# om-ai-lab/OmChat

Measured on AMD Instinct MI355X. Metric: images/sec prefill + decode tokens/sec, OmChat-13B TP=1/8; p50 TTFT, higher is better.
Workload: dtype bf16

## Files before the change

include/omchat_hip.h:

```cpp
#ifndef OMCHAT_HIP_H
#define OMCHAT_HIP_H
#include <stddef.h>
#include <stdint.h>

#ifdef __cplusplus
extern "C" {
#endif

#define OMCHAT_F16 0
#define OMCHAT_BF16 1
#define OMCHAT_F32 2
#define OMCHAT_PAD_ROW INT32_MIN

typedef struct omchat_ctx omchat_ctx;

typedef struct {
  int v_hidden;
  int v_heads;
  int v_qk_channels;
  int v_mlp;
  int v_layers;
  int v_patch;
  int v_image;
  float v_eps;
  int t_hidden;
  int t_layers;
  int t_heads;
  int t_kv_heads;
  int t_mlp;
  int t_vocab;
  int t_vocab_total;
  float t_eps;
  float rope_theta;
  int max_seq;
  int max_batch;
  int max_tiles;
  int max_prefill_rows;
  int dtype;
  int v_head_dim;
  int v_norm_type;
  int v_no_qk_norm;
} omchat_config;

const char* omchat_last_error(void);
const char* omchat_version(void);

int omchat_ctx_create(const omchat_config* cfg, int tp_rank, int tp_size, void* rccl_comm, omchat_ctx** out);
void omchat_ctx_destroy(omchat_ctx* ctx);
int omchat_load_tensor(omchat_ctx* ctx, const char* name, const void* data, const int64_t* shape, int ndim, int src_dtype);
int omchat_fill_synthetic(omchat_ctx* ctx, uint64_t seed);
int omchat_weights_missing(omchat_ctx* ctx);
size_t omchat_device_bytes(omchat_ctx* ctx);

int omchat_vit_forward(omchat_ctx* ctx, const void* pixels, int n_tiles, int select_layer, int keep_cls, void* out, void* stream);
int omchat_projector_forward(omchat_ctx* ctx, const void* in, int rows, void* out, void* stream);
int omchat_encode_images(omchat_ctx* ctx, const void* pixels, int n_tiles, int select_layer, void* out, void* stream);

int omchat_splice_plan(const int64_t* ids, const uint8_t* mask, int b, int T, int n_tok, int n_tiles_avail,
                       int padding_side, int max_length, int32_t* src_index, int32_t* lengths, int* S_out, int vocab);
int omchat_splice_gather(omchat_ctx* ctx, const int32_t* src_index, const void* feats, void* embeds, int rows, void* stream);

int omchat_prefill(omchat_ctx* ctx, const void* embeds, int b, int S, const int32_t* lengths, float* logits_last,
                   void* hidden_out, void* stream);
int omchat_prefill_left(omchat_ctx* ctx, const void* embeds, int b, int S, const int32_t* lengths, float* logits_last,
                        void* hidden_out, void* stream);
int omchat_decode_step(omchat_ctx* ctx, const int32_t* tokens, int b, float* logits, int32_t* next_tokens, void* stream);
int omchat_decode_step_masked(omchat_ctx* ctx, const int32_t* tokens, int b, const int32_t* positions, const uint8_t* key_mask, int mask_ld,
                              float* logits, int32_t* next_tokens, void* stream);
int omchat_masked_decode_begin(omchat_ctx* ctx, int b, const int32_t* positions, const uint8_t* key_mask, int mask_ld, int mask_cols, void* stream);
int omchat_decode_step_masked_next(omchat_ctx* ctx, const int32_t* tokens, int b, float* logits, int32_t* next_tokens, void* stream);
int omchat_fused_status(omchat_ctx* ctx, long* launches, unsigned* timeout_bits);
int omchat_has_experiments(void);
int omchat_lm_head(omchat_ctx* ctx, const void* hidden, int n, float* logits, void* stream);
int omchat_greedy(omchat_ctx* ctx, const float* logits, int b, int32_t* next_tokens, void* stream);
int omchat_set_sampling(omchat_ctx* ctx, int b, uint64_t seed, float temperature, int top_k, double top_p, float rep_penalty,
                        const int32_t* seen_ids, const int32_t* n_seen_per_row, void* stream);
int omchat_set_sampling_filters(omchat_ctx* ctx, double min_p, double typical_p, double epsilon_cutoff, double eta_cutoff, void* stream);
int omchat_sample(omchat_ctx* ctx, const float* logits, int b, int32_t* next_tokens, void* stream);
#define OMCHAT_CON_MAX_NGRAM 64
#define OMCHAT_CON_MAX_EOS 16
#define OMCHAT_CON_MAX_SUPPRESS 1024
#define OMCHAT_CON_MAX_BAD_WORDS 1024
#define OMCHAT_CON_MAX_BAD_WORD_IDS 8192
int omchat_set_constraints(omchat_ctx* ctx, int b, int no_repeat_ngram_size, int min_new_tokens, int min_length, const int32_t* eos_ids, int n_eos,
                           const int32_t* suppress_ids, int n_suppress, const int32_t* begin_suppress_ids, int n_begin_suppress,
                           const int32_t* bad_word_ids, const int32_t* bad_word_offsets, int n_bad_words, const int32_t* prompt_ids,
                           const int32_t* prompt_len, int max_new, void* stream);
int omchat_set_logprobs(omchat_ctx* ctx, int b, int max_new, void* stream);
int omchat_read_logprobs(omchat_ctx* ctx, int b, float* raw, float* processed, int32_t* counts, int max_len);
int omchat_read_sampling_state(omchat_ctx* ctx, int row, int* step, uint32_t* seen_words);
int omchat_kv_lengths(omchat_ctx* ctx, int32_t* out, int b);
int omchat_kv_rewind(omchat_ctx* ctx, int b, int n, void* stream);

int omchat_beam_begin(omchat_ctx* ctx, int b, int num_beams, float length_penalty, int early_stopping, const int32_t* eos_ids, int n_eos,
                      int max_new, int prompt_tok_len, void* stream);
int omchat_beam_step(omchat_ctx* ctx, const float* logits, int rows, int32_t* next_tokens, int32_t* done_word, void* stream);
int omchat_beam_result(omchat_ctx* ctx, int num_return, int32_t* tokens, int32_t* lengths, float* scores, int max_len);

#define OMCHAT_VERIFY_KEEP_ALL 1
#define OMCHAT_VERIFY_SAMPLE 2
int omchat_decode_verify(omchat_ctx* ctx, const int32_t* tokens, int T, float* logits, int32_t* picks,
                         int* n_accept, int flags, void* stream);

int omchat_prefill_extend(omchat_ctx* ctx, const void* embeds, int S_new, int keep, float* logits_last, void* hidden_out, void* stream);
int omchat_extend_attn_form(int S_new, int keep, int Hkv);
int omchat_kv_read(omchat_ctx* ctx, int layer, int which, int pos0, int n, void* out, void* stream);

int omchat_enable_decode_graph(omchat_ctx* ctx, int on);
int omchat_decode_graph_stats(omchat_ctx* ctx, long* steps, long* replays, long* captures);

int omchat_enable_fp8_decode(omchat_ctx* ctx, int on);

int omchat_enable_mxfp4_decode(omchat_ctx* ctx, int mode);

int omchat_enable_fp8_kv(omchat_ctx* ctx, int on);
int omchat_enable_fp8_prefill(omchat_ctx* ctx, int on);

#define OMCHAT_PROF_DECODE_GATEUP 0
#define OMCHAT_PROF_PREFILL_GATEUP 1
#define OMCHAT_PROF_VIT_FC1 2
#define OMCHAT_PROF_CATS 3
int omchat_prof_enable(omchat_ctx* ctx, int on);
int omchat_prof_read(omchat_ctx* ctx, int cat, double* total_ms, long* launches, int reset);

int omchat_mha_fwd(const void* qkv, int B, int S, int H, float softmax_scale, int causal, void* out, int dtype, void* stream);
int omchat_mha_fwd_varlen(const void* qkv, int B, int S, int H, int D, const int32_t* seqlens, float softmax_scale, int causal,
                          void* out, int dtype, void* stream);

int omchat_op_gemm(int dtype, const void* A, int lda, const void* W, int ldw, void* C, int ldc, int M, int N, int K,
                   const void* bias, const void* ls, const void* resid, int ldr, int epi, int force_tile, void* stream);
int omchat_op_gemm_fused(int dtype, const void* A, int lda, const void* W, int ldw, void* C, int ldc, int M, int N, int K,
                         const void* bias, const void* ls, const void* resid, int ldr, int epi, int force_tile, const float* row_scale,
                         const float* rs_stats, int rs_ld, int rs_nslots, int rs_dim, float rs_eps,
                         float* stats, int stats_ld, int* nslots, void* stream);
int omchat_op_stats_finish(const float* stats, int ld, int slot0, int nslots, int ngroups, int rows, int dim, float eps, float* out, void* stream);
int omchat_op_row_sumsq(int dtype, const void* x, int ldx, int rows, int H, float* stats, void* stream);
int omchat_op_fold_cols(int dtype, const void* W, const void* n, void* out, int rows, int cols, void* stream);
int omchat_op_vit_knorm_slots(int dtype, void* k, int ld, const void* wk, int rows, int C, int C_total, float eps, const float* stats, int stats_ld,
                              int nslots, float* sumsq_q, void* stream);
int omchat_op_mha_qnorm(int dtype, const void* qkv, int B, int Sq, int H, const float* sumsq, int stride, int dim, const void* wq,
                        float eps, float q_scale, void* out, void* stream);
int omchat_op_gemv_norm(int dtype, const void* X, const void* W, int ldw, void* Y, int N, int K, const void* norm_w, float eps,
                        const void* bias, int epi, int out_f32, void* stream);
int omchat_op_set_tuning(int key, int value);
int omchat_gemm_tune_load(const char* path);
int omchat_gemm_tune_dump(const char* path);
long omchat_gemm_tune_runs(void);
size_t omchat_op_gemm_sk_ws(void);
int omchat_op_gemm_sk(int dtype, const void* A, int lda, const void* W, int ldw, void* C, int ldc, int M, int N, int K,
                      const void* bias, const void* ls, const void* resid, int ldr, int epi, int force_tile, void* ws,
                      size_t ws_bytes, int stream_k, void* stream);
int omchat_op_gemv(int dtype, const void* X, int ldx, const void* W, int ldw, void* Y, int ldy, int b, int N, int K,
                   const void* bias, const void* resid, int ldr, int epi, int out_f32, void* stream);
int omchat_op_gemv_packed(int dtype, const void* X, int ldx, const void* W, int ldw, void* Y, int ldy, int b, int N, int K,
                          const void* bias, int epi, int out_f32, int ksplit, int w_packed, int y_packed, void* stream);
int omchat_op_pack_x(int dtype, const void* X, int ldx, int b, int K, void* out, void* stream);
int omchat_op_gemm_fp8(int dtype, const void* A8, const float* a_scale, const void* W8, const float* w_scale, void* C, int ldc, int M, int N,
                       int K, const void* bias, const void* resid, int ldr, int epi, void* stream);
int omchat_op_quant_rows_fp8(int dtype, const void* x, const void* norm_w, float eps, void* y8, float* scale, int rows, int H, void* stream);
int omchat_op_quant_fp8(int dtype, const void* W, int N, int K, void* W8, float* scale, void* stream);
int omchat_op_gemv_fp8(int dtype, const void* X, const void* W8, const float* scale, void* Y, int N, int K, const void* bias,
                       const void* resid, int epi, int out_f32, int ksplit, void* stream);
int omchat_op_quant_mxfp4(int dtype, const void* W, int N, int K, void* W4, void* S, void* stream);
int omchat_op_gemv_mxfp4(int dtype, const void* X, const void* W4, const void* S, void* Y, int N, int K, const void* bias,
                         const void* resid, int epi, int out_f32, int ksplit, void* stream);
int omchat_op_gemv_mxfp4_norm(int dtype, const void* X, const void* W4, const void* S, void* Y, int N, int K, const void* norm_w, float eps,
                              const void* bias, int epi, int out_f32, void* stream);
int omchat_op_gemv_mxfp4_rows(int dtype, const void* X, int ldx, const void* W4, const void* S, void* Y, int ldy, int b, int N, int K,
                              const void* bias, int epi, int out_f32, int ksplit, void* stream);
int omchat_op_gemv_mxfp4_packed(int dtype, const void* X, int ldx, const void* W4, const void* S, void* Y, int ldy, int b, int N, int K,
                                const void* bias, int epi, int out_f32, int ksplit, int y_packed, void* stream);
int omchat_op_pack_w(int dtype, const void* W, int ldw, int N, int K, void* out, void* stream);
int omchat_op_pack_w4(const void* W4, const void* S, int N, int K, void* W4P, void* SP, void* stream);
int omchat_op_gemv_prepacked(int dtype, const void* XP, const void* WP, const void* SP, void* Y, int ldy, int b, int N, int K, const void* bias,
                             int epi, int out_f32, int ksplit, int y_packed, void* stream);
int omchat_op_rmsnorm(int dtype, const void* x, const void* w, void* y, int rows, int H, float eps, void* stream);
int omchat_op_resid_rmsnorm(int dtype, void* x, int ldx, const float* part, int ks, const void* w, void* xn, int ldn, int rows, int H,
                            float eps, int pack_nb, void* stream);
int omchat_op_vit_qknorm(int dtype, void* qkv, int ld, const void* wq, const void* wk, int rows, int C, int C_total,
                         float eps, float q_scale, void* stream);
int omchat_op_attn_prefill(int dtype, const void* q, const void* k, const void* v, void* out, int b, int Sq, int Skv,
                           int Hq, int Hkv, const int32_t* kv_len, int causal, int q_pos0, float scale, void* stream);
int omchat_op_attn_prefill_d(int dtype, const void* q, const void* k, const void* v, void* out, int b, int Sq, int Skv,
                             int Hq, int Hkv, int D, const int32_t* kv_len, int causal, int q_pos0, float scale, void* stream);
int omchat_op_layernorm(int dtype, const void* x, const void* w, const void* b, void* y, int rows, int H, float eps, void* stream);
size_t omchat_op_attn_decode_ws(int b, int Hq, int L);
int omchat_op_attn_decode(int dtype, const void* q, const void* k, const void* v, void* out, int b, int Hq, int Hkv,
                          int cap, int L, const int32_t* kv_len, float scale, void* ws, size_t ws_bytes, void* stream);
int omchat_op_attn_verify(int dtype, const void* q, void* k, void* v, void* out, int T, int Hq, int Hkv, int cap, int L, float scale,
                          void* ws, size_t ws_bytes, void* stream);
int omchat_op_attn_verify_tpw(int keys, int Hkv);
size_t omchat_op_attn_extend_ws(int Sq, int Hq, int Hkv, int L);
int omchat_op_attn_extend(int dtype, const void* q, const void* k, const void* v, void* out, int Sq, int Hq, int Hkv, int cap, int L,
                          float scale, void* ws, size_t ws_bytes, void* stream);
int omchat_op_attn_verify_append(int dtype, const void* qkv, float theta, void* k, void* v, void* out, int T, int Hq, int Hkv, int cap,
                                 int L, float scale, void* ws, size_t ws_bytes, void* stream);
// ... 95 lines not shown
```

omchat_amd/_lib.py:

```python
import ctypes as C
import os

HERE = os.path.dirname(os.path.abspath(__file__))
LIB_PATH = os.environ.get("OMCHAT_LIB") or os.path.join(HERE, "lib", "libomchat_hip.so")
_lib = None

F16, BF16, F32 = 0, 1, 2
EPI_NONE, EPI_GELU, EPI_LS_RESID, EPI_RESID, EPI_SWIGLU = 0, 1, 2, 3, 4
EPI_F32OUT = 6
EPI_LS_RESID_STATS, EPI_NONE_STATS = 7, 8
PAD_ROW = -(2 ** 31)
PROF_DECODE_GATEUP, PROF_PREFILL_GATEUP, PROF_VIT_FC1 = 0, 1, 2


class OmchatConfig(C.Structure):
    _fields_ = [
        ("v_hidden", C.c_int), ("v_heads", C.c_int), ("v_qk_channels", C.c_int), ("v_mlp", C.c_int), ("v_layers", C.c_int),
        ("v_patch", C.c_int), ("v_image", C.c_int), ("v_eps", C.c_float),
        ("t_hidden", C.c_int), ("t_layers", C.c_int), ("t_heads", C.c_int), ("t_kv_heads", C.c_int), ("t_mlp", C.c_int),
        ("t_vocab", C.c_int), ("t_vocab_total", C.c_int), ("t_eps", C.c_float), ("rope_theta", C.c_float),
        ("max_seq", C.c_int), ("max_batch", C.c_int), ("max_tiles", C.c_int), ("max_prefill_rows", C.c_int), ("dtype", C.c_int),
        ("v_head_dim", C.c_int), ("v_norm_type", C.c_int), ("v_no_qk_norm", C.c_int),
    ]

# ... 52 lines not shown
    "omchat_op_row_sumsq": (_i, [_i, _vp, _i, _i, _i, _vp, _vp]),
    "omchat_op_fold_cols": (_i, [_i, _vp, _vp, _vp, _i, _i, _vp]),
    "omchat_op_vit_knorm_slots": (_i, [_i, _vp, _i, _vp, _i, _i, _i, _f, _vp, _i, _i, _vp, _vp]),
    "omchat_op_mha_qnorm": (_i, [_i, _vp, _i, _i, _i, _vp, _i, _i, _vp, _f, _f, _vp, _vp]),
    "omchat_ctx_sp_stats": (_i, [_vp, C.POINTER(C.c_long), C.POINTER(C.c_long)]),
    "omchat_op_set_tuning": (_i, [_i, _i]),
    "omchat_gemm_tune_load": (_i, [C.c_char_p]),
    "omchat_gemm_tune_dump": (_i, [C.c_char_p]),
    "omchat_gemm_tune_runs": (C.c_long, []),
    "omchat_op_gemm_sk_ws": (_sz, []),
    "omchat_op_gemm_sk": (_i, [_i, _vp, _i, _vp, _i, _vp, _i, _i, _i, _i, _vp, _vp, _vp, _i, _i, _i, _vp, _sz, _i, _vp]),
    "omchat_op_gemv": (_i, [_i, _vp, _i, _vp, _i, _vp, _i, _i, _i, _i, _vp, _vp, _i, _i, _i, _vp]),
    "omchat_op_gemv_packed": (_i, [_i, _vp, _i, _vp, _i, _vp, _i, _i, _i, _i, _vp, _i, _i, _i, _i, _i, _vp]),
    "omchat_op_pack_x": (_i, [_i, _vp, _i, _i, _i, _vp, _vp]),
    "omchat_op_gemm_fp8": (_i, [_i, _vp, _vp, _vp, _vp, _vp, _i, _i, _i, _i, _vp, _vp, _i, _i, _vp]),
    "omchat_op_quant_rows_fp8": (_i, [_i, _vp, _vp, _f, _vp, _vp, _i, _i, _vp]),
    "omchat_enable_fp8_decode": (_i, [_vp, _i]),
    "omchat_enable_fp8_kv": (_i, [_vp, _i]),
    "omchat_enable_fp8_prefill": (_i, [_vp, _i]),
    "omchat_enable_decode_graph": (_i, [_vp, _i]),
    "omchat_decode_graph_stats": (_i, [_vp, C.POINTER(C.c_long), C.POINTER(C.c_long), C.POINTER(C.c_long)]),
    "omchat_op_quant_fp8": (_i, [_i, _vp, _i, _i, _vp, _vp, _vp]),
    "omchat_op_gemv_fp8": (_i, [_i, _vp, _vp, _vp, _vp, _i, _i, _vp, _vp, _i, _i, _i, _vp]),
    "omchat_enable_mxfp4_decode": (_i, [_vp, _i]),
    "omchat_op_quant_mxfp4": (_i, [_i, _vp, _i, _i, _vp, _vp, _vp]),
    "omchat_op_gemv_mxfp4": (_i, [_i, _vp, _vp, _vp, _vp, _i, _i, _vp, _vp, _i, _i, _i, _vp]),
    "omchat_op_gemv_mxfp4_rows": (_i, [_i, _vp, _i, _vp, _vp, _vp, _i, _i, _i, _i, _vp, _i, _i, _i, _vp]),
    "omchat_op_gemv_mxfp4_packed": (_i, [_i, _vp, _i, _vp, _vp, _vp, _i, _i, _i, _i, _vp, _i, _i, _i, _i, _vp]),
    "omchat_op_pack_w": (_i, [_i, _vp, _i, _i, _i, _vp, _vp]),
    "omchat_op_pack_w4": (_i, [_vp, _vp, _i, _i, _vp, _vp, _vp]),
    "omchat_op_gemv_prepacked": (_i, [_i, _vp, _vp, _vp, _vp, _i, _i, _i, _i, _vp, _i, _i, _i, _i, _vp]),
    "omchat_op_gemv_mxfp4_norm": (_i, [_i, _vp, _vp, _vp, _vp, _i, _i, _vp, _f, _vp, _i, _i, _vp]),
    "omchat_op_rmsnorm": (_i, [_i, _vp, _vp, _vp, _i, _i, _f, _vp]),
    "omchat_op_resid_rmsnorm": (_i, [_i, _vp, _i, _vp, _i, _vp, _vp, _i, _i, _i, _f, _i, _vp]),
    "omchat_op_vit_qknorm": (_i, [_i, _vp, _i, _vp, _vp, _i, _i, _i, _f, _f, _vp]),
    "omchat_op_attn_prefill": (_i, [_i, _vp, _vp, _vp, _vp, _i, _i, _i, _i, _i, _vp, _i, _i, _f, _vp]),
    "omchat_op_attn_prefill_d": (_i, [_i, _vp, _vp, _vp, _vp, _i, _i, _i, _i, _i, _i, _vp, _i, _i, _f, _vp]),
    "omchat_op_layernorm": (_i, [_i, _vp, _vp, _vp, _vp, _i, _i, _f, _vp]),
    "omchat_op_attn_decode_ws": (_sz, [_i, _i, _i]),
    "omchat_op_attn_decode": (_i, [_i, _vp, _vp, _vp, _vp, _i, _i, _i, _i, _i, _vp, _f, _vp, _sz, _vp]),
    "omchat_op_attn_verify_tpw": (_i, [_i, _i]),
    "omchat_op_attn_verify": (_i, [_i, _vp, _vp, _vp, _vp, _i, _i, _i, _i, _i, _f, _vp, _sz, _vp]),
    "omchat_op_attn_extend_ws": (_sz, [_i, _i, _i, _i]),
    "omchat_op_attn_extend": (_i, [_i, _vp, _vp, _vp, _vp, _i, _i, _i, _i, _i, _f, _vp, _sz, _vp]),
    "omchat_prefill_extend": (_i, [_vp, _vp, _i, _i, _vp, _vp, _vp]),
    "omchat_extend_attn_form": (_i, [_i, _i, _i]),
    "omchat_kv_read": (_i, [_vp, _i, _i, _i, _i, _vp, _vp]),
    "omchat_op_attn_verify_append": (_i, [_i, _vp, _f, _vp, _vp, _vp, _i, _i, _i, _i, _i, _f, _vp, _sz, _vp]),
    "omchat_op_attn_decode_kv8": (_i, [_i, _vp, _vp, _vp, _vp, _vp, _vp, _i, _i, _i, _i, _i, _vp, _f, _vp, _sz, _vp]),
    "omchat_op_attn_decode_kv8_append": (_i, [_i, _vp, _f, _vp, _vp, _vp, _vp, _vp, _vp, _vp, _i, _i, _i, _i, _i, _vp, _vp, _f, _vp, _sz, _vp]),
    "omchat_op_rope_kv": (_i, [_i, _vp, _i, _i, _i, _i, _i, _f, _vp, _vp, _i, _vp]),
    "omchat_op_rope_kv_q8": (_i, [_i, _vp, _i, _i, _i, _i, _i, _f, _vp, _vp, _i, _vp, _vp, _vp, _vp, _vp]),
    "omchat_op_argmax": (_i, [_vp, _i, _i, _vp, _vp]),
    "omchat_op_attn_prefill_left": (_i, [_i, _vp, _vp, _vp, _vp, _i, _i, _i, _i, _i, _vp, _vp, _i, _i, _f, _i, _vp]),
    "omchat_op_rope_kv_pos": (_i, [_i, _vp, _i, _i, _i, _i, _vp, _i, _i, _i, _f, _vp, _vp, _i, _vp]),
    "omchat_op_argmax_ld": (_i, [_vp, _i, _i, _i, _vp, _vp, _vp, _vp]),
    "omchat_op_im2col": (_i, [_i, _vp, _vp, _i, _i, _i, _i, _vp]),
    "omchat_op_vit_assemble": (_i, [_i, _vp, _vp, _vp, _vp, _i, _i, _i, _vp]),
    "omchat_op_gather_rows": (_i, [_i, _vp, _vp, _vp, _vp, _i, _i, _vp]),
    "omchat_op_copy_rows": (_i, [_i, _vp, _i64, _vp, _i64, _i, _i, _i, _i, _vp]),
    "omchat_op_tp_finish": (_i, [_i, _vp, _vp, _vp, _vp, _vp, _i, _i, _i, _vp]),
    "omchat_op_resid16_norm": (_i, [_i, _vp, _i, _vp, _i, _vp, _vp, _vp, _i, _i, _i, _f, _vp]),
    "omchat_op_cast_f32": (_i, [_i, _vp, _vp, _i64, _vp]),
    "omchat_op_rmsnorm_ld": (_i, [_i, _vp, _i, _vp, _vp, _i, _i, _i, _f, _i, _vp]),
    "omchat_op_layernorm_ld": (_i, [_i, _vp, _i, _vp, _vp, _vp, _i, _i, _i, _f, _vp]),
    "omchat_op_sample": (_i, [_vp, _i, _i, _u64, _f, _i, C.c_double, _f, _vp, _vp, _i, _vp, _vp, _vp]),
    "omchat_op_token_logprob": (_i, [_vp, _i, _i, _i, _vp, _vp, _f, _f, _vp, _vp, _vp, _vp, _vp, _vp, _vp]),
    "omchat_op_sample_filtered": (_i, [_vp, _i, _i, _u64, _f, _i, C.c_double, _f, C.c_double, C.c_double, C.c_double, C.c_double, _vp, _vp, _i,
                                       _vp, _vp, _vp, _vp]),
    "omchat_op_sample_verify": (_i, [_vp, _i, _i, _i, _vp, _u64, _i, _f, _i, C.c_double, _f, C.c_double, C.c_double, C.c_double, C.c_double, _vp,
                                     _i, _i, _i, _vp, _vp, _vp, _vp]),
    "omchat_read_sampling_state": (_i, [_vp, _i, _vp, _vp]),
    "omchat_op_token_logprob_interval": (_i, [_vp, _i, _i, _i, _vp, _vp, _f, _f, _vp, _vp, _vp, _vp, _vp, _vp, _vp, _vp]),
    "omchat_op_constrain": (_i, [_vp, _vp, _vp, _i, _i, _i, _i, _i, _i, _i, _i, _vp, _i, _vp, _i, _vp, _i, _vp, _vp, _i, _vp, _vp]),
    "omchat_beam_state_words": (_sz, [_i, _i, _i]),
    "omchat_op_beam_select": (_i, [_vp, _i, _i, _i, _i, _i, _i, _f, _i, _vp, _i, _vp, _vp, _vp, _vp, _vp]),
    "omchat_op_kv_gather": (_i, [_i, _vp, _vp, _vp, _vp, _vp, _vp, _i, _i, _i, _i, _vp, _i, _i, _i, _i, _i, _vp]),
    "omchat_op_fill_uniform": (_i, [_i, _vp, _i64, _u64, _f, _f, _vp]),
    "omchat_preproc_plan": (_i, [_i, _i, _vp, _i, _i, C.POINTER(_i), C.POINTER(_i), C.POINTER(_i)]),
    "omchat_preproc_anyres": (_i, [_i, _vp, _i, _i, _i, _i, _i, _i, _vp, _vp, _vp, _vp]),
    "omchat_preproc_dynamic": (_i, [_i, _vp, _i, _i, _i, _i, _i, _i, _i, _vp, _vp, _vp, _vp]),
    "omchat_resample_coeffs": (_i, [_i, _i, C.POINTER(_i), _vp, _vp, _i]),
    "omchat_normalize_lut": (_i, [_vp, _vp, _vp]),
    "omchat_comm_unique_id": (_i, [C.c_char_p]),
    "omchat_comm_init": (_i, [C.c_char_p, _i, _i, C.POINTER(_vp)]),
    "omchat_comm_allreduce": (_i, [_vp, _vp, _sz, _i, _vp]),
    "omchat_comm_destroy": (None, [_vp]),
    "omchat_comm_count": (_i, [_vp, C.POINTER(_i)]),
    "omchat_peer_create": (_i, [_i, _i, _sz, C.POINTER(_vp), C.c_char_p]),
    "omchat_peer_connect": (_i, [_vp, C.c_char_p]),
    "omchat_peer_base": (_vp, [_vp]),
    "omchat_peer_connect_local": (_i, [_vp, C.POINTER(_vp)]),
    "omchat_peer_set_mode": (_i, [_vp, _i, _sz, _i]),
    "omchat_peer_capacity": (_sz, [_vp]),
    "omchat_peer_allreduce": (_i, [_vp, _vp, _sz, _i, _vp]),
    "omchat_peer_reduce_scatter": (_i, [_vp, _vp, _sz, _i, _vp]),
    "omchat_peer_all_gather": (_i, [_vp, _vp, _sz, _i, _vp]),
    "omchat_peer_resid_rmsnorm": (_i, [_vp, _i, _vp, _i, _vp, _i, _vp, _vp, _i, _i, _i, _f, _i, _vp]),
    "omchat_peer_error": (_i, [_vp, C.POINTER(_i)]),
    "omchat_peer_destroy": (None, [_vp]),
    "omchat_ctx_set_peer": (_i, [_vp, _vp, _sz, _i]),
    "omchat_ctx_allreduce": (_i, [_vp, _vp, _sz, _i, _vp]),
    "omchat_ctx_comm_stats": (_i, [_vp, C.POINTER(C.c_long), C.POINTER(C.c_long)]),
}
EXPORTS = sorted(_SIGS)

# ... 50 lines not shown
```

omchat_amd/csrc/capi.hip:

```cpp
#include "kernels.h"
#include <stdlib.h>
#include "../../include/omchat_hip.h"
#include <math.h>
#include <vector>

#define S(x) ((hipStream_t)(x))
#if OMCHAT_EXPERIMENTS
int g_launch_any_order = 0;
#endif

extern "C" int omchat_op_gemm(int dtype, const void* A, int lda, const void* W, int ldw, void* C, int ldc, int M, int N, int K,
                              const void* bias, const void* ls, const void* resid, int ldr, int epi, int force_tile, void* stream) {
  GemmArgs g{A, lda, W, ldw, C, ldc, M, N, K, bias, ls, resid, ldr, epi, force_tile, nullptr, 0, -1};
  return launch_gemm(dtype, g, S(stream));
}

extern "C" int omchat_op_gemm_fused(int dtype, const void* A, int lda, const void* W, int ldw, void* C, int ldc, int M, int N, int K,
                                    const void* bias, const void* ls, const void* resid, int ldr, int epi, int force_tile, const float* row_scale,
                                    const float* rs_stats, int rs_ld, int rs_nslots, int rs_dim, float rs_eps,
                                    float* stats, int stats_ld, int* nslots, void* stream) {
  GemmArgs g{A, lda, W, ldw, C, ldc, M, N, K, bias, ls, resid, ldr, epi, force_tile, nullptr, 0, -1};
  g.row_scale = row_scale; g.stats = stats; g.stats_ld = stats_ld; g.stats_nslots = nslots;
  g.rs_stats = rs_stats; g.rs_ld = rs_ld; g.rs_nslots = rs_nslots; g.rs_dim = rs_dim; g.rs_eps = rs_eps;
  return launch_gemm(dtype, g, S(stream));
// ... 22 lines not shown
  a.O = out; a.o_sb = (int64_t)Sq * H * 128; a.o_sh = 128; a.o_sr = (int64_t)H * 128;
  a.batch = B; a.q_heads = H; a.kv_heads = H; a.Sq = Sq; a.Skv = Sq; a.kv_len = nullptr; a.causal = 0; a.q_pos0 = 0;
  a.scale = 1.0f;
  a.qn_sumsq = sumsq; a.qn_stride = stride; a.qn_dim = dim; a.qn_w = wq; a.qn_eps = eps; a.qn_scale = q_scale;
  return launch_attn_prefill(dtype, a, S(stream));
}

extern "C" int omchat_op_set_tuning(int key, int value) {
  const char* allow = getenv("OMCHAT_ALLOW_TUNING");
  if (!allow || allow[0] != '1') {
    omchat_set_error("omchat_op_set_tuning: process-global test / measurement hook; set OMCHAT_ALLOW_TUNING=1 to use it (see include/omchat_hip.h)");
    return 1;
  }
  if (key == 0) { gemm_set_skew(value); return 0; }
  if (key == 1) { gemv_set_force_mfma(value); return 0; }
  if (key == 5) { gemm_set_autotune(value); return 0; }
  if (key == 4) { model_set_ar_min_rows(value); return 0; }
  if (key == 6) { model_set_pack_replica(value); return 0; }
  if (key == 8) { attn_set_v2(value); return 0; }
  if (key == 9) { model_set_fuse_peer_norm(value); return 0; }
  if (key == 10) { attn_set_tpw(value); return 0; }
  if (key == 11) { gemv_set_no_xs(value); return 0; }
  if (key == 12) { attn_set_klds(value); return 0; }
  if (key == 25) { attn_set_dma(value); return 0; }
  if (key == 26) { attn_set_dma_slots(value); return 0; }
  if (key == 27) { attn_set_dma_rot(value); return 0; }
  if (key == 28) { gemv_set_skew(value); return 0; }
  if (key == 29) { model_set_tp_f32(value); return 0; }
  if (key == 30) { attn_set_hsplit(value); return 0; }
  if (key == 33) { attn_set_mha_xcd(value); return 0; }
  if (key == 16) { gemv_set_norm_loop(value); return 0; }
  if (key == 17) { gemv_set_rows_balance(value); return 0; }
  if (key == 19) { attn_set_merge_mid_min(value); return 0; }
  if (key == 21) { attn_set_merge_dg(value); return 0; }
  if (key == 13) { gemm_set_persist(value); return 0; }
  if (key == 14) { model_set_norm_in_gemv(value); return 0; }
  if (key == 22) { model_set_fuse_attn_oproj(value); return 0; }
  if (key == 23) { model_set_decode_layer(value); return 0; }
  if (key == 24) { gemv_set_dyn(value); return 0; }
  if (key == 34) { gemv_set_shard_shapes(value); return 0; }
  if (key == 35) { model_set_shard_as_tp1(value); return 0; }
  if (key == 36) { attn_set_kg(value); return 0; }
  if (key == 37) { gemm_set_wide_store(value); return 0; }
  if (key == 43) { gemm_set_skip_dead(value); return 0; }
  if (key == 44) { model_set_vit_fused(value); return 0; }
  if (key == 45) { model_set_tp_sp(value); return 0; }
  if (key == 46) { attn_set_peel(value); return 0; }
  if (key == 47) { attn_set_kv8_tpw(value); return 0; }
  if (key == 48) { attn_set_kv8_fuse(value); return 0; }
  if (key == 49) { model_set_extend_attn(value); return 0; }
  if (key == 38) { gemv_set_gu_rr(value); return 0; }
  if (key == 39) { gemv_set_longk_direct(value); return 0; }
  if (key == 40) { norm_set_wave(value); return 0; }
#if OMCHAT_EXPERIMENTS
  if (key == 41) { g_launch_any_order = value; return 0; }
  if (key == 42) { model_set_ao_oproj(value); return 0; }
#endif
  omchat_set_error("omchat_op_set_tuning: unknown key");
  return 1;
}

extern "C" int omchat_allreduce_noop(void*, void*, size_t, int, void*) { return 0; }

extern "C" int omchat_gemm_tune_load(const char* path) { OM_CHECK(path, "null path"); return gemm_tune_load(path); }
extern "C" int omchat_gemm_tune_dump(const char* path) { OM_CHECK(path, "null path"); return gemm_tune_dump(path); }
extern "C" long omchat_gemm_tune_runs(void) { return gemm_tune_runs(); }

extern "C" size_t omchat_op_gemm_sk_ws(void) { return gemm_sk_ws_bytes(); }

extern "C" int omchat_op_gemm_sk(int dtype, const void* A, int lda, const void* W, int ldw, void* C, int ldc, int M, int N, int K,
                                 const void* bias, const void* ls, const void* resid, int ldr, int epi, int force_tile, void* ws,
                                 size_t ws_bytes, int stream_k, void* stream) {
  GemmArgs g{A, lda, W, ldw, C, ldc, M, N, K, bias, ls, resid, ldr, epi, force_tile, ws, ws_bytes, stream_k};
  return launch_gemm(dtype, g, S(stream));
}

extern "C" int omchat_op_gemv(int dtype, const void* X, int ldx, const void* W, int ldw, void* Y, int ldy, int b, int N, int K,
                              const void* bias, const void* resid, int ldr, int epi, int out_f32, void* stream) {
  GemvArgs g{X, ldx, W, ldw, Y, ldy, b, N, K, bias, resid, ldr, epi, out_f32};
  return launch_gemv(dtype, g, S(stream));
}

extern "C" int omchat_op_gemv_norm(int dtype, const void* X, const void* W, int ldw, void* Y, int N, int K, const void* norm_w, float eps,
                                   const void* bias, int epi, int out_f32, void* stream) {
  OM_CHECK(X && W && Y && norm_w, "null argument");
  GemvArgs g{X, K, W, ldw, Y, N, 1, N, K, bias, nullptr, 0, epi, out_f32};
  g.norm_w = norm_w; g.norm_eps = eps;
  return launch_gemv(dtype, g, S(stream));
}

extern "C" int omchat_op_gemv_packed(int dtype, const void* X, int ldx, const void* W, int ldw, void* Y, int ldy, int b, int N, int K,
                                     const void* bias, int epi, int out_f32, int ksplit, int w_packed, int y_packed, void* stream) {
  OM_CHECK(b >= 1 && b <= 32 && K % 64 == 0, "1 <= b <= 32, K % 64 == 0");
  const int NB = b > 16 ? 2 : 1;
  void *xp = nullptr, *wp = nullptr;
  OM_HIP(hipMalloc(&xp, (size_t)NB * 16 * K * 2));
  int rc = launch_pack_x(dtype, X, ldx, b, K, xp, S(stream));
  if (rc == 0 && w_packed) {
    if (hipMalloc(&wp, (size_t)N * K * 2) != hipSuccess) { hipFree(xp); omchat_set_error("hipMalloc failed"); return 2; }
    rc = launch_pack_w(dtype, W, ldw, N, K, wp, S(stream));
  }
  if (rc == 0) {
    GemvArgs g{xp, K, w_packed ? wp : W, ldw, Y, ldy, b, N, K, bias, nullptr, 0, epi, out_f32, ksplit, 0, nullptr, 1, w_packed, y_packed};
    rc = launch_gemv(dtype, g, S(stream));
  }
  hipStreamSynchronize(S(stream));
  hipFree(xp); if (wp) hipFree(wp);
  return rc;
}
extern "C" int omchat_op_pack_x(int dtype, const void* X, int ldx, int b, int K, void* out, void* stream) { return launch_pack_x(dtype, X, ldx, b, K, out, S(stream)); }

extern "C" int omchat_op_gemm_fp8(int dtype, const void* A8, const float* a_scale, const void* W8, const float* w_scale, void* C, int ldc, int M,
                                  int N, int K, const void* bias, const void* resid, int ldr, int epi, void* stream) {
  GemmArgs g{A8, K, W8, K, C, ldc, M, N, K, bias, nullptr, resid, ldr, epi, 0, nullptr, 0, -1, 1, a_scale, w_scale};
  return launch_gemm(dtype, g, S(stream));
}
extern "C" int omchat_op_quant_rows_fp8(int dtype, const void* x, const void* norm_w, float eps, void* y8, float* scale, int rows, int H, void* stream) {
  if (norm_w) return launch_rmsnorm_q8(dtype, x, H, norm_w, y8, H, scale, rows, H, eps, S(stream));
  return launch_quant_rows_q8(dtype, x, H, y8, H, scale, rows, H, S(stream));
}

extern "C" int omchat_op_resid_rmsnorm(int dtype, void* x, int ldx, const float* part, int ks, const void* w, void* xn, int ldn, int rows, int H,
                                       float eps, int pack_nb, void* stream) {
  OM_CHECK(x && part, "null argument");
  return launch_resid_rmsnorm(dtype, x, ldx, part, ks, w, xn, ldn, rows, H, eps, S(stream), pack_nb);
}
extern "C" int omchat_op_rmsnorm(int dtype, const void* x, const void* w, void* y, int rows, int H, float eps, void* stream) {
  return launch_rmsnorm(dtype, x, H, w, y, H, rows, H, eps, S(stream));
}

extern "C" int omchat_op_vit_qknorm(int dtype, void* qkv, int ld, const void* wq, const void* wk, int rows, int C, int C_total, float eps,
                                    float q_scale, void* stream) {
  return launch_vit_qknorm(dtype, qkv, ld, wq, wk, rows, C, C_total, eps, q_scale, nullptr, S(stream));
}

extern "C" int omchat_op_attn_prefill(int dtype, const void* q, const void* k, const void* v, void* out, int b, int Sq, int Skv, int Hq,
                                      int Hkv, const int32_t* kv_len, int causal, int q_pos0, float scale, void* stream) {
  AttnArgs a{};
  a.Q = q; a.q_sb = (int64_t)Sq * Hq * 128; a.q_sh = 128; a.q_sr = (int64_t)Hq * 128;
  a.K = k; a.k_sb = (int64_t)Hkv * Skv * 128; a.k_sh = (int64_t)Skv * 128; a.k_sr = 128;
// ... 673 lines not shown
```

omchat_amd/csrc/ctx.h:

```cpp
#pragma once
#include "kernels.h"
#include "../../include/omchat_hip.h"
#include <rccl/rccl.h>
#include <string>
#include <unordered_map>
#include <vector>

#define TRY(x) do { int rc_ = (x); if (rc_) return rc_; } while (0)

extern int g_fuse_peer_norm;

enum RouteKind { R_PLAIN = 0, R_GATE = 1, R_UP = 2, R_PATCH = 3 };
struct Route {
  void* dst = nullptr;
  int64_t rows = 0, cols = 0;
  int64_t dst_ld = 0;
  int kind = R_PLAIN;
  bool loaded = false;
  float synth_std = 0.02f, synth_off = 0.f;
};

struct Grown {
  void* p = nullptr; size_t cap = 0;
  void release() { if (p) (void)hipFree(p); p = nullptr; cap = 0; }
};

struct PickState {
  void* arg_scratch = nullptr;
  float* tp_table = nullptr;
  struct Sampling { bool on = false; uint64_t seed = 0; float temperature = 1.f; int top_k = 0; double top_p = 1.0; float penalty = 1.f; };
  Sampling smp;
  SampleFilters smp_f, smp_f_graph;
  void* smp_ws = nullptr;
  uint32_t* smp_bm = nullptr; int smp_bmw = 0;
  int *smp_last = nullptr, *smp_step = nullptr;
  uint32_t* smp_vseen = nullptr;
  int* smp_vlast = nullptr;
  int smp_vcommit = 0;
  struct Constraints {
    bool on = false; int b = 0, ngram = 0, min_new = 0, min_len = 0, n_eos = 0, n_sup = 0, n_bsup = 0, n_bw = 0;
    bool operator==(const Constraints& o) const {
      return on == o.on && b == o.b && ngram == o.ngram && min_new == o.min_new && min_len == o.min_len && n_eos == o.n_eos && n_sup == o.n_sup &&
             n_bsup == o.n_bsup && n_bw == o.n_bw;
    }
  };
  Constraints con;
  int con_ld = 0, con_fed = 0, con_room = 0;
  int *con_len = nullptr, *con_plen = nullptr;
  int32_t* con_lists = nullptr;
  uint32_t* con_ban = nullptr; int con_bmw = 0;
  float* con_logits = nullptr;
  struct Logprobs { bool on = false; int b = 0, max_new = 0; };
  Logprobs lp;
  int lp_picks = 0;
  int lp_cap = 0;
  int* lp_cnt = nullptr;
  void* lp_ws = nullptr;
  float* lp_table = nullptr;
  Grown con_hist;
  Grown lp_rec;
  bool sampling_on() const { return smp.on; }
  bool constraints_on() const { return con.on; }
  bool logprobs_on() const { return lp.on; }
  void release() { con_hist.release(); lp_rec.release(); }
};

struct BeamState {
  struct Search { bool on = false; int b = 0, N = 0, KB = 0, max_new = 0, P = 0, es = 0, ns = 1, t = 0; float lp = 1.f; std::vector<int> eos; };
  Search cur;
  Grown state, table, dn, parents, stash;
  bool stash8 = false;
  std::vector<int> hpos, hlen;
  bool on() const { return cur.on; }
  void end() { cur.on = false; }
  void release() { for (Grown* g : {&state, &table, &dn, &parents, &stash}) g->release(); }
};

struct omchat_ctx {
  omchat_config c;
  int dt = OMCHAT_BF16;
  int tp_rank = 0, tp_size = 1;
// ... 14 lines not shown
  void* t_lmP = nullptr;
  bool pk_ready = false, pk_unavailable = false;
  void* t_lm8 = nullptr; float* t_lm8_s = nullptr;
  bool fp8_decode = false, fp8_stale = false;
  struct DecLayer4 { void *wqkv = nullptr, *wo = nullptr, *wgu = nullptr, *wd = nullptr; unsigned char *sqkv = nullptr, *so = nullptr, *sgu = nullptr, *sd = nullptr; };
  std::vector<DecLayer4> dl4;
  void* t_lm4 = nullptr; unsigned char* t_lm4_s = nullptr;
  bool mxfp4_decode = false, mxfp4_stale = false;
  std::vector<DecLayer4> dl4p;
  void* t_lm4P = nullptr; unsigned char* t_lm4P_s = nullptr;
  bool mxfp4_batched = false, mxfp4p_stale = false;
  bool mx4_rows_ok(int b) const { return !(mxfp4_decode && mxfp4_batched && b > 32); }
  bool mx4_step(int b) const { return mxfp4_decode && (b == 1 || (mxfp4_batched && b >= 2 && b <= 32)); }
  void *k8cache = nullptr, *v8cache = nullptr;
  float *ks8 = nullptr, *vs8 = nullptr;
  bool fp8_kv = false, kv8_valid = false, fp8_prefill = false;
  void* tw_q8 = nullptr; float* tw_q8s = nullptr;
  int64_t scale_layer_stride() const { return (int64_t)c.max_batch * c.t_kv_heads * c.max_seq; }
  struct DecodeGraph { hipGraph_t graph = nullptr; hipGraphExec_t exec = nullptr; int cap_len = 0; };
  std::unordered_map<int, DecodeGraph> graphs;
  bool graph_on = false;
  hipStream_t graph_stream = nullptr;
  hipEvent_t graph_ev_in = nullptr, graph_ev_out = nullptr;
  int32_t *d_tok_in = nullptr, *d_tok_out = nullptr;
  long graph_steps = 0, graph_replays = 0, graph_captures = 0;
  void *v_cls = nullptr, *v_pos = nullptr, *v_wpatch = nullptr, *v_bpatch = nullptr;
  std::vector<VitLayer> vl;
  void *p_w0 = nullptr, *p_b0 = nullptr, *p_w2 = nullptr, *p_b2 = nullptr;
  void *t_embed = nullptr, *t_norm = nullptr, *t_lm = nullptr;
  std::vector<DecLayer> dl;
  float* rope = nullptr;

  void *vw_cols = nullptr, *vw_pe = nullptr, *vw_x = nullptr, *vw_x2 = nullptr, *vw_xn = nullptr, *vw_qkv = nullptr, *vw_ao = nullptr,
       *vw_h = nullptr, *vw_feat = nullptr, *vw_proj = nullptr;
  float* vw_sumsq = nullptr;
  float *vw_stats_x = nullptr, *vw_stats_qk = nullptr, *vw_rstd = nullptr;
  int vw_stats_x_ld = 0, vw_stats_qk_ld = 0, vw_stats_x_ld_used = 1;
  struct VitFold { void *wqkv = nullptr, *w1 = nullptr; };
  std::vector<VitFold> vfold;
  bool vfold_stale = true;
  void *tw_x = nullptr, *tw_x2 = nullptr, *tw_xn = nullptr, *tw_qkv = nullptr, *tw_ao = nullptr, *tw_act = nullptr, *tw_last = nullptr;
  float* tw_logits = nullptr;
  void* sk_ws = nullptr; size_t sk_ws_bytes = 0;
  float* tp_f32_ws = nullptr; size_t tp_f32_bytes = 0;
  float* tw_part = nullptr;
  float* tw_attn_ws = nullptr;
  size_t tw_attn_ws_bytes = 0;
  void* fd_ws = nullptr;
  unsigned* fd_err = nullptr;
  unsigned fd_epoch = 0;
  long n_fused_launches = 0;
  void* dl_ws = nullptr;
  long n_layer_launches = 0;
  unsigned long long* dbg_stamps = nullptr;
  unsigned* dyn_ctr = nullptr;
  int *d_pos = nullptr, *d_len = nullptr, *d_idx = nullptr, *d_start = nullptr;
  int* d_verify_n = nullptr;
  PickState pick;
  BeamState beam;
  Grown ext_ws;
  int grow(Grown& g, size_t n) {
    if (n <= g.cap) return 0;
    if (g.p) { hipFree(g.p); bytes -= g.cap; g.p = nullptr; g.cap = 0; }
    hipError_t e = hipMalloc(&g.p, n);
    if (e != hipSuccess) { omchat_set_error(std::string("hipMalloc failed: ") + hipGetErrorString(e)); return 2; }
    g.cap = n; bytes += n;
    return 0;
  }
  bool left_padded = false;
  int pre_S = 0, pre_b = 0, masked_steps = 0, dec_mode = 0;
  unsigned char* d_mask = nullptr; int64_t mask_sb = 0;
  bool mask_on_device = false;
  void *kcache = nullptr, *vcache = nullptr;
  std::vector<int> h_len;
  struct Prof { std::vector<hipEvent_t> ev; size_t used = 0; double ms = 0; long count = 0; };
  bool prof_on = false;
  Prof prof[OMCHAT_PROF_CATS];
  void prof_mark(int cat, hipStream_t s) {
    if (!prof_on) return;
    Prof& p = prof[cat];
    if (p.used == p.ev.size()) { hipEvent_t e; hipEventCreate(&e); p.ev.push_back(e); }
    hipEventRecord(p.ev[p.used++], s);
  }
  void* stage_f32 = nullptr; size_t stage_f32_bytes = 0;
  void* stage_t = nullptr; size_t stage_t_bytes = 0;

  int alloc(void** p, size_t n) {
    if (n == 0) n = 16;
    hipError_t e = hipMalloc(p, n);
    if (e != hipSuccess) { omchat_set_error(std::string("hipMalloc failed: ") + hipGetErrorString(e)); return 2; }
    allocs.push_back(*p);
    bytes += n;
    return 0;
  }
  int alloc_group(const std::vector<void**>& slots, const std::vector<size_t>& sizes) {
    std::vector<void*> got;
    size_t total = 0;
    for (size_t i = 0; i < slots.size(); ++i) {
      const size_t n = sizes[i] ? sizes[i] : 16;
      const hipError_t e = hipMalloc(slots[i], n);
      if (e != hipSuccess) {
        (void)hipGetLastError();
        for (void* p : got) (void)hipFree(p);
        for (void** s : slots) *s = nullptr;
        omchat_set_error(std::string("hipMalloc failed: ") + hipGetErrorString(e));
        return 2;
// ... 104 lines not shown
```

omchat_amd/csrc/elementwise.hip:

```cpp
#include "kernels.h"
#include <limits.h>

namespace {

constexpr int NORM_THREADS = 256;
constexpr int NORM_MAXC = 8;

__device__ __forceinline__ float block_sum(float v, float* red) {
  v = wave_sum(v);
  const int lane = threadIdx.x & 63, wave = threadIdx.x >> 6;
  if (lane == 0) red[wave] = v;
  __syncthreads();
  float t = 0.f;
#pragma unroll
  for (int w = 0; w < NORM_THREADS / 64; ++w) t += red[w];
  __syncthreads();
  return t;
}

template <typename T>
__global__ __launch_bounds__(NORM_THREADS) void rmsnorm_kernel(const T* x, int ldx, const T* w, T* y, int ldy, int H, float eps, int pack_nb) {
  typedef typename V8<T>::type v8;
  __shared__ float red[NORM_THREADS / 64];
  const int row = blockIdx.x;
// ... 602 lines not shown
__global__ void vit_assemble_kernel(const T* pe, const T* cls, const T* pos, T* x, int B, int np, int C) {
  typedef typename V8<T>::type v8;
  const int cc = C >> 3;
  const long n = (long)B * (np + 1) * cc;
  for (long i = (long)blockIdx.x * blockDim.x + threadIdx.x; i < n; i += (long)gridDim.x * blockDim.x) {
    const int c = (int)(i % cc);
    const long rt = i / cc;
    const int t = (int)(rt % (np + 1)), b = (int)(rt / (np + 1));
    const v8 a = t == 0 ? ld8<T>(cls + c * 8) : ld8<T>(pe + ((size_t)b * np + (t - 1)) * C + c * 8);
    const v8 p = ld8<T>(pos + (size_t)t * C + c * 8);
    v8 o;
#pragma unroll
    for (int j = 0; j < 8; ++j) o[j] = fromf<T>(tof(a[j]) + tof(p[j]));
    st8<T>(x + ((size_t)b * (np + 1) + t) * C + c * 8, o);
  }
}

template <typename T>
__global__ void gather_rows_kernel(const int* idx, const T* table, const T* feats, T* out, int rows, int H) {
  typedef typename V8<T>::type v8;
  const int cc = H >> 3;
  const long n = (long)rows * cc;
  for (long i = (long)blockIdx.x * blockDim.x + threadIdx.x; i < n; i += (long)gridDim.x * blockDim.x) {
    const int c = (int)(i % cc);
    const int r = (int)(i / cc);
    const int id = idx[r];
    v8 v;
    if (id == INT_MIN) {
#pragma unroll
      for (int j = 0; j < 8; ++j) v[j] = (T)0.f;
    } else if (id >= 0) {
      v = ld8<T>(table + (size_t)id * H + c * 8);
    } else {
      v = ld8<T>(feats + (size_t)(-1 - id) * H + c * 8);
    }
    st8<T>(out + (size_t)r * H + c * 8, v);
  }
}

template <typename T>
__global__ void copy_rows_kernel(const T* src, int64_t src_ld, T* dst, int64_t dst_ld, int rows, int H, int group, int skip) {
  typedef typename V8<T>::type v8;
  const int cc = H >> 3;
  const long n = (long)rows * cc;
  for (long i = (long)blockIdx.x * blockDim.x + threadIdx.x; i < n; i += (long)gridDim.x * blockDim.x) {
    const int c = (int)(i % cc);
    const long r = i / cc;
    const long sr = (r / group) * (group + skip) + skip + r % group;
    st8<T>(dst + r * dst_ld + c * 8, ld8<T>(src + sr * src_ld + c * 8));
  }
}

constexpr int ARG_CHUNKS = 64;
__device__ __forceinline__ void arg_better(float& best, int& besti, float v, int i) {
  if (v > best || (v == best && i < besti)) { best = v; besti = i; }
}
__global__ __launch_bounds__(256) void argmax_stage1_kernel(const float* logits, int ld, int V, float* pv, int* pi) {
  __shared__ float bv[4];
  __shared__ int bi[4];
  const float* row = logits + (size_t)blockIdx.y * ld;
  const int per = (V + ARG_CHUNKS - 1) / ARG_CHUNKS;
  const int lo = blockIdx.x * per, hi = lo + per < V ? lo + per : V;
  float best = -INFINITY;
  int besti = INT_MAX;
  for (int i = lo + threadIdx.x; i < hi; i += 256) arg_better(best, besti, row[i], i);
#pragma unroll
  for (int o = 32; o > 0; o >>= 1) arg_better(best, besti, __shfl_xor(best, o, 64), __shfl_xor(besti, o, 64));
  if ((threadIdx.x & 63) == 0) { bv[threadIdx.x >> 6] = best; bi[threadIdx.x >> 6] = besti; }
  __syncthreads();
  if (threadIdx.x == 0) {
    for (int w = 1; w < 4; ++w) arg_better(best, besti, bv[w], bi[w]);
    pv[blockIdx.y * ARG_CHUNKS + blockIdx.x] = best;
    pi[blockIdx.y * ARG_CHUNKS + blockIdx.x] = besti;
  }
}
__global__ __launch_bounds__(64) void argmax_stage2_kernel(const float* pv, const int* pi, int* out, int* adv_pos, int* adv_len) {
  if (threadIdx.x == 0) {
    if (adv_pos) adv_pos[blockIdx.x] += 1;
    if (adv_len) adv_len[blockIdx.x] += 1;
  }
  float best = pv[blockIdx.x * ARG_CHUNKS + threadIdx.x];
  int besti = pi[blockIdx.x * ARG_CHUNKS + threadIdx.x];
#pragma unroll
  for (int o = 32; o > 0; o >>= 1) arg_better(best, besti, __shfl_xor(best, o, 64), __shfl_xor(besti, o, 64));
  if (threadIdx.x == 0) out[blockIdx.x] = besti == INT_MAX ? 0 : besti;
}

__device__ __forceinline__ uint64_t splitmix64(uint64_t x) {
  x += 0x9E3779B97F4A7C15ull;
  x = (x ^ (x >> 30)) * 0xBF58476D1CE4E5B9ull;
  x = (x ^ (x >> 27)) * 0x94D049BB133111EBull;
  return x ^ (x >> 31);
}
template <typename T>
__global__ void fill_uniform_kernel(T* dst, int64_t n, uint64_t key, float mul, float offset) {
  for (int64_t i = (int64_t)blockIdx.x * blockDim.x + threadIdx.x; i < n; i += (int64_t)gridDim.x * blockDim.x) {
    const uint64_t h = splitmix64(key + (uint64_t)i * 0x9E3779B97F4A7C15ull);
    const int iv = (int)(h >> 40) - (1 << 23);
    float v = __fmul_rn((float)iv, mul);
    if (offset != 0.f) v = __fadd_rn(v, offset);
    uint32_t u = __float_as_uint(v);
    u = ((u + 0x7FFFu + ((u >> 16) & 1u)) >> 16) << 16;
    float f = __uint_as_float(u);
    if ((float)((f16)f) != f) f = 0.f;
    dst[i] = (T)f;
  }
}

template <typename T>
__global__ void cast_f32_kernel(const T* src, float* dst, int64_t n) {
  for (int64_t i = (int64_t)blockIdx.x * blockDim.x + threadIdx.x; i < n; i += (int64_t)gridDim.x * blockDim.x) dst[i] = tof(src[i]);
}

inline int grid_for(long n, int threads) {
  long g = (n + threads - 1) / threads;
  return (int)(g < 1 ? 1 : (g > 8192 ? 8192 : g));
}

}

#define DISPATCH(dtype, CALL)                                        \
  if ((dtype) == OMCHAT_F16) { typedef f16 T; CALL; }                \
  else if ((dtype) == OMCHAT_BF16) { typedef bf16 T; CALL; }         \
  else { omchat_set_error("bad dtype"); return 1; }

static int g_norm_wave = 0;
[[maybe_unused]] constexpr int NORM_WAVE_ROWS = 256;
void norm_set_wave(int v) { g_norm_wave = v; }

int launch_layernorm(int dtype, const void* x, int ldx, const void* w, const void* b, void* y, int ldy, int rows, int H, float eps, hipStream_t s) {
  OM_CHECK(H % 8 == 0 && H <= NORM_THREADS * NORM_MAXC * 8 && ldx % 8 == 0 && ldy % 8 == 0, "H must be a multiple of 8 and <= 16384");
  OM_CHECK(w && b, "LayerNorm needs weight and bias");
  if (rows == 0) return 0;
  DISPATCH(dtype, hipLaunchKernelGGL(layernorm_kernel<T>, dim3(rows), dim3(NORM_THREADS), 0, s, (const T*)x, ldx, (const T*)w, (const T*)b, (T*)y, ldy, H, eps));
  OM_LAUNCH_CHECK();
  return 0;
}

// ... 137 lines not shown
template <typename T>
__global__ __launch_bounds__(256) void tp_finish_kernel(const float* __restrict__ sum, const T* __restrict__ bias, const T* __restrict__ ls,
                                                        const T* resid, T* out, long total4, int N, int epi) {
#pragma clang fp contract(off)
  for (long i = (long)blockIdx.x * 256 + threadIdx.x; i < total4; i += (long)gridDim.x * 256) {
    const long e = i * 4;
    const int col = (int)(e % N);
    const f32x4 a = *reinterpret_cast<const f32x4*>(sum + e);
    typename V8<T>::half_type o;
#pragma unroll
    for (int j = 0; j < 4; ++j) {
      float v = a[j] + (bias ? tof(bias[col + j]) : 0.f);
      if (epi != EPI_NONE) v = rnd<T>(v);
      if (epi == EPI_LS_RESID) v = tof(resid[e + j]) + rnd<T>(v * tof(ls[col + j]));
      if (epi == EPI_RESID) v = tof(resid[e + j]) + v;
      o[j] = fromf<T>(v);
    }
    *reinterpret_cast<typename V8<T>::half_type*>(out + e) = o;
  }
}

int launch_tp_finish(int dtype, const float* sum, const void* bias, const void* ls, const void* resid, void* out, int M, int N, int epi, hipStream_t s) {
  OM_CHECK(sum && out && M > 0 && N > 0 && N % 4 == 0, "tp_finish: null argument or N % 4 != 0");
  OM_CHECK(epi == EPI_NONE || ((epi == EPI_RESID || epi == EPI_LS_RESID) && resid && (epi != EPI_LS_RESID || ls)), "tp_finish: epilogue NONE / RESID / LS_RESID with its operands");
  const long total4 = (long)M * N / 4;
  const int grid = (int)std::min<long>((total4 + 255) / 256, 4096);
  if (dtype == OMCHAT_F16) hipLaunchKernelGGL(tp_finish_kernel<f16>, dim3(grid), dim3(256), 0, s, sum, (const f16*)bias, (const f16*)ls, (const f16*)resid, (f16*)out, total4, N, epi);
  else if (dtype == OMCHAT_BF16) hipLaunchKernelGGL(tp_finish_kernel<bf16>, dim3(grid), dim3(256), 0, s, sum, (const bf16*)bias, (const bf16*)ls, (const bf16*)resid, (bf16*)out, total4, N, epi);
  else { omchat_set_error("tp_finish: bad dtype"); return 1; }
  OM_LAUNCH_CHECK();
  return 0;
}

int launch_gather_rows(int dtype, const int* idx, const void* table, const void* feats, void* out, int rows, int H, hipStream_t s) {
  OM_CHECK(H % 8 == 0, "H % 8");
  const long n = (long)rows * (H / 8);
  if (n == 0) return 0;
  DISPATCH(dtype, hipLaunchKernelGGL(gather_rows_kernel<T>, dim3(grid_for(n, 256)), dim3(256), 0, s, idx, (const T*)table, (const T*)feats, (T*)out, rows, H));
  OM_LAUNCH_CHECK();
  return 0;
}

int launch_copy_rows(int dtype, const void* src, int64_t src_ld, void* dst, int64_t dst_ld, int rows, int H, int group, int skip, hipStream_t s) {
  OM_CHECK(H % 8 == 0 && src_ld % 8 == 0 && dst_ld % 8 == 0 && group > 0, "H/ld % 8, group > 0");
  const long n = (long)rows * (H / 8);
  if (n == 0) return 0;
  DISPATCH(dtype, hipLaunchKernelGGL(copy_rows_kernel<T>, dim3(grid_for(n, 256)), dim3(256), 0, s, (const T*)src, src_ld, (T*)dst, dst_ld, rows, H, group, skip));
  OM_LAUNCH_CHECK();
  return 0;
}

size_t argmax_scratch_bytes(int b) { return (size_t)b * ARG_CHUNKS * 8; }

int launch_argmax(const float* logits, int ld, int b, int V, int* out, void* scratch, hipStream_t s, int* adv_pos, int* adv_len) {
  if (b == 0) return 0;
  OM_CHECK(scratch, "argmax scratch missing");
  float* pv = (float*)scratch;
  int* pi = (int*)((char*)scratch + (size_t)b * ARG_CHUNKS * 4);
  hipLaunchKernelGGL(argmax_stage1_kernel, dim3(ARG_CHUNKS, b), dim3(256), 0, s, logits, ld, V, pv, pi);
  hipLaunchKernelGGL(argmax_stage2_kernel, dim3(b), dim3(64), 0, s, pv, pi, out, adv_pos, adv_len);
  OM_LAUNCH_CHECK();
  return 0;
}

int launch_resid_rmsnorm(int dtype, void* x, int ldx, const float* part, int ks, const void* w, void* xn, int ldn, int rows, int H, float eps,
                         hipStream_t s, int pack_nb) {
  OM_CHECK(H % 8 == 0 && H <= NORM_THREADS * NORM_MAXC * 8 && ldx % 8 == 0 && ldn % 8 == 0 && ks >= 1, "H % 8, H <= 16384, ld % 8");
  OM_CHECK(pack_nb == 0 || (rows <= 16 * pack_nb && H % 64 == 0), "packed output: rows <= 16 * NB, H % 64 == 0");
  if (rows == 0) return 0;
  OM_CHECK(ks <= 8, "at most 8 K slices");
#define RR(KS_) case KS_: DISPATCH(dtype, hipLaunchKernelGGL((resid_rmsnorm_kernel<T, KS_>), dim3(rows), dim3(NORM_THREADS), 0, s, (T*)x, ldx, part, rows, (const T*)w, (T*)xn, ldn, H, eps, pack_nb)); break;
  switch (ks) { RR(1) RR(2) RR(3) RR(4) RR(5) RR(6) RR(7) RR(8) }
#undef RR
  OM_LAUNCH_CHECK();
  return 0;
}

int launch_fill_uniform(int dtype, void* dst, int64_t n, uint64_t key, float scale, float offset, hipStream_t s) {
  if (n == 0) return 0;
  const float mul = scale / 8388608.0f;
  DISPATCH(dtype, hipLaunchKernelGGL(fill_uniform_kernel<T>, dim3(grid_for(n, 256)), dim3(256), 0, s, (T*)dst, n, key, mul, offset));
  OM_LAUNCH_CHECK();
  return 0;
}

int launch_cast_f32(int dtype, const void* src, float* dst, int64_t n, hipStream_t s) {
  if (n == 0) return 0;
  DISPATCH(dtype, hipLaunchKernelGGL(cast_f32_kernel<T>, dim3(grid_for(n, 256)), dim3(256), 0, s, (const T*)src, dst, n));
  OM_LAUNCH_CHECK();
  return 0;
}
```

omchat_amd/csrc/gemv.hip:

```cpp
#include "kernels.h"
#include "rowdot.h"
#include <type_traits>

namespace {

struct GemvP {
  const void* X; const void* W; void* Y; const void* bias; const void* resid;
  int ldx, ldw, ldy, ldr, b, N, K, out_f32, ksplit;
  const float* w_scale;
  int y_packed;
  const void* norm_w; float norm_eps;
  unsigned* dyn;
  void* y_pack;
  unsigned long long* dbg;
  const unsigned char* mx_s;
#if OMCHAT_EXPERIMENTS
  int xskew;
#endif
};
constexpr int WF_16 = 0, WF_E4M3 = 1, WF_MX4 = 2;
#if OMCHAT_EXPERIMENTS
#define OM_DBG_MIN(slot, cond) do { if (p.dbg && (cond) && threadIdx.x == 0) atomicMax(p.dbg + (slot), ~wall_clock64()); } while (0)
#define OM_DBG_MAX(slot, cond) do { if (p.dbg && (cond) && threadIdx.x == 0) atomicMax(p.dbg + (slot), wall_clock64()); } while (0)
#else
#define OM_DBG_MIN(slot, cond) do { } while (0)
#define OM_DBG_MAX(slot, cond) do { } while (0)
#endif

template <typename T, int NTILE, int N, int WAVES, bool NTL, int NB>
__device__ __forceinline__ void gemv_group(f32x4 (&acc)[NTILE][NB], const T* const (&wrow)[NTILE], const T* const (&xrow)[NB], int k0,
                                           const bool (&xvalid)[NB]) {
  typedef typename V8<T>::type frag_t;
  frag_t wf[N][NTILE][2], xf[N][NB][2];
#pragma unroll
  for (int u = 0; u < N; ++u) {
    const int k = k0 + u * WAVES * 64;
#pragma unroll
    for (int t = 0; t < NTILE; ++t) {
      if constexpr (NTL) {
        wf[u][t][0] = __builtin_nontemporal_load(reinterpret_cast<const frag_t*>(wrow[t] + k));
        wf[u][t][1] = __builtin_nontemporal_load(reinterpret_cast<const frag_t*>(wrow[t] + k + 32));
      } else {
        wf[u][t][0] = ld8<T>(wrow[t] + k);
        wf[u][t][1] = ld8<T>(wrow[t] + k + 32);
      }
    }
#pragma unroll
    for (int nb = 0; nb < NB; ++nb) {
      xf[u][nb][0] = ld8<T>(xrow[nb] + k);
      xf[u][nb][1] = ld8<T>(xrow[nb] + k + 32);
    }
  }
  frag_t zero;
#pragma unroll
  for (int j = 0; j < 8; ++j) zero[j] = (T)0.f;
#pragma unroll
  for (int u = 0; u < N; ++u) {
#pragma unroll
    for (int nb = 0; nb < NB; ++nb) {
      if (!xvalid[nb]) { xf[u][nb][0] = zero; xf[u][nb][1] = zero; }
#pragma unroll
      for (int t = 0; t < NTILE; ++t) {
        acc[t][nb] = mfma16(wf[u][t][0], xf[u][nb][0], acc[t][nb]);
        acc[t][nb] = mfma16(wf[u][t][1], xf[u][nb][1], acc[t][nb]);
      }
    }
  }
}

template <typename T, int NTILE, int N, int WAVES, bool NTL, int NB>
__device__ __forceinline__ void gemv_tail(int rem, f32x4 (&acc)[NTILE][NB], const T* const (&wrow)[NTILE], const T* const (&xrow)[NB], int k0,
                                          const bool (&xvalid)[NB]) {
// ... 643 lines not shown

template <typename T, int R, int NCH>
__device__ __forceinline__ void rw_rows(const T* W, int ldw, const int (&rows)[R], int k0, int K, int lane, const rw_u32x4 (&xr)[RW_MAXC],
                                        float (&acc)[R], RwTail<T, R>& tail) {
  rw_u32x4 w[R][NCH];
#pragma unroll
  for (int r = 0; r < R; ++r)
#pragma unroll
    for (int c = 0; c < NCH; ++c) {
      int k = k0 + c * 512 + lane * 8;
      k = k < K ? k : k0;
      w[r][c] = __builtin_nontemporal_load(reinterpret_cast<const rw_u32x4*>(W + (size_t)rows[r] * ldw + k));
    }
  rw_tail_load<T, R>(tail);
#pragma unroll
  for (int r = 0; r < R; ++r) {
    float a = 0.f;
#pragma unroll
    for (int c = 0; c < NCH; ++c) a = rw_dot8<T>(w[r][c], xr[c], a);
#pragma unroll
    for (int o = 32; o > 0; o >>= 1) a += __shfl_xor(a, o, 64);
    acc[r] = a;
  }
}

template <typename T, int R, int N>
__device__ __forceinline__ void rw_dispatch(int nch, const T* W, int ldw, const int (&rows)[R], int k0, int K, int lane,
                                            const rw_u32x4 (&xr)[RW_MAXC], float (&acc)[R], RwTail<T, R>& tail) {
  if constexpr (N > 0) {
    if (nch == N) rw_rows<T, R, N>(W, ldw, rows, k0, K, lane, xr, acc, tail);
    else rw_dispatch<T, R, N - 1>(nch, W, ldw, rows, k0, K, lane, xr, acc, tail);
  }
}

template <typename T, int EPI, int RR, int WAVES, int F8>
__device__ __forceinline__ void gemv_rows_body(const GemvP& p) {
  constexpr int R = EPI == EPI_SWIGLU ? 2 * RR : RR;
  constexpr int OUT = RR;
  const int lane = threadIdx.x & 63, wave = threadIdx.x >> 6;
  const T* W = (const T*)p.W;
  if constexpr (EPI == EPI_RESID && WAVES == 7) OM_DBG_MIN(1, blockIdx.x < 8);
  const int nch_all = (p.K + 511) / 512;
  const int c_lo = (int)(((long)nch_all * blockIdx.y) / p.ksplit), c_hi = (int)(((long)nch_all * (blockIdx.y + 1)) / p.ksplit);
  const int nch = c_hi - c_lo, k0 = c_lo * 512;
  rw_u32x4 xr[RW_MAXC];
#pragma unroll
  for (int c = 0; c < RW_MAXC; ++c) {
    const int k = k0 + c * 512 + lane * 8;
    rw_u32x4 z = {0u, 0u, 0u, 0u};
    xr[c] = (c < nch && k < p.K) ? *reinterpret_cast<const rw_u32x4*>((const T*)p.X + k) : z;
  }
  const int n_out = EPI == EPI_SWIGLU ? p.N / 2 : p.N;
  const int ngroups = (n_out + OUT - 1) / OUT;
  for (int g = blockIdx.x * WAVES + wave; g < ngroups; g += gridDim.x * WAVES) {
    int rows[R];
#pragma unroll
    for (int r = 0; r < R; ++r) {
      if constexpr (EPI == EPI_SWIGLU) {
        int n = g * RR + (r % RR); n = n < n_out ? n : n_out - 1;
        rows[r] = 32 * (n >> 4) + (n & 15) + (r / RR) * 16;
      } else {
        const int n = g * R + r;
        rows[r] = n < p.N ? n : p.N - 1;
      }
    }
    float acc[R];
    RwTail<T, R> tail;
    {
      constexpr bool plain = EPI != EPI_SWIGLU && EPI != EPI_PARTIAL;
      const bool hb = plain && p.bias, hr = EPI == EPI_RESID && !p.out_f32;
      tail.p0 = hb ? (const T*)p.bias : (const T*)p.X;
      tail.p1 = hr ? (const T*)p.resid : (const T*)p.X;
#pragma unroll
      for (int r = 0; r < R; ++r) {
        const int n = g * OUT + r;
        tail.idx[r] = (hb || hr) ? (n < n_out ? n : n_out - 1) : 0;
      }
      if (!hb) tail.p0 = tail.p1;
      if (!hr) tail.p1 = tail.p0;
    }
    if constexpr (F8 != WF_16) rw_dispatch_q<T, R, RW_MAXC, F8>(nch, p, rows, k0, lane, xr, acc, tail);
    else rw_dispatch<T, R, RW_MAXC>(nch, W, p.ldw, rows, k0, p.K, lane, xr, acc, tail);
    if (lane == 0) {
#pragma unroll
      for (int r = 0; r < OUT; ++r) {
        const int n = g * OUT + r;
        if (n >= n_out) continue;
        if constexpr (EPI == EPI_SWIGLU) {
          const float gt = rnd<T>(acc[r]), up = rnd<T>(acc[r + RR]);
          ((T*)p.Y)[n] = fromf<T>(rnd<T>(silu(gt)) * up);
        } else if constexpr (EPI == EPI_PARTIAL) {
          ((float*)p.Y)[(size_t)blockIdx.y * p.ldy + n] = acc[r];
        } else {
          float y = acc[r] + (p.bias ? tail.v0[r] : 0.f);
          if (p.out_f32) ((float*)p.Y)[n] = y;
          else {
            y = rnd<T>(y);
            if constexpr (EPI == EPI_RESID) y = tail.v1[r] + y;
            ((T*)p.Y)[n] = fromf<T>(y);
          }
        }
      }
    }
  }
  if constexpr (EPI == EPI_RESID && WAVES == 7) OM_DBG_MAX(3, (blockIdx.x & 7) == 0);
}

template <typename T, int EPI, int RR = 4, int WAVES = 4, bool F8 = false>
__global__ __launch_bounds__(WAVES * 64) void gemv_rows_kernel(GemvP p) { gemv_rows_body<T, EPI, RR, WAVES, F8 ? WF_E4M3 : WF_16>(p); }
template <typename T, int EPI, int RR, int WAVES>
__global__ __launch_bounds__(WAVES * 64) void gemv_rows_mx4_kernel(GemvP p) { gemv_rows_body<T, EPI, RR, WAVES, WF_MX4>(p); }

template <typename T, int EPI, int RR, int NCH, int F8, int WAVES>
__device__ __forceinline__ void gemv_rows_norm_body(const GemvP& p) {
  typedef typename V8<T>::type v8;
  constexpr int R = EPI == EPI_SWIGLU ? 2 * RR : RR;
  __shared__ __attribute__((aligned(16))) T xs[NCH * 512];
  __shared__ float red[WAVES];
  const int lane = threadIdx.x & 63, wave = __builtin_amdgcn_readfirstlane(threadIdx.x >> 6);
  const int n_out = EPI == EPI_SWIGLU ? p.N / 2 : p.N;
  int g = blockIdx.x * WAVES + wave;
#if OMCHAT_EXPERIMENTS
  if constexpr (EPI == EPI_SWIGLU && RR == 1 && WAVES == 4) {
    if (p.xskew) {
      const int x = blockIdx.x & 7, j = blockIdx.x >> 3;
      const int base = ((n_out + 3) / 4) / 8;
      const int n_x = base + ((x & 1) ? -p.xskew : p.xskew);
      if (j >= n_x) return;
      g = (x * base + ((x & 1) ? p.xskew : 0) + j) * 4 + wave;
    }
  }
#endif
  if constexpr (EPI == EPI_SWIGLU) OM_DBG_MIN(4, blockIdx.x < 8);
  if constexpr (EPI == EPI_NONE) OM_DBG_MIN(8, blockIdx.x < 8);
  static_assert(WAVES >= 4 && NCH <= 8, "sum-of-squares order: four owner waves, up to two chunks each");
  constexpr int MC = (NCH + WAVES - 1) / WAVES;
  constexpr int SC = (NCH + 3) / 4;
  rw_u32x4 xq[MC], nq[MC], sq[SC];
#pragma unroll
  for (int i = 0; i < MC; ++i) {
    const int c = wave + WAVES * i, k = c * 512 + lane * 8;
    const rw_u32x4 z = {0u, 0u, 0u, 0u};
    const bool ok = c < NCH && k < p.K;
    xq[i] = ok ? *reinterpret_cast<const rw_u32x4*>((const T*)p.X + k) : z;
    nq[i] = ok ? *reinterpret_cast<const rw_u32x4*>((const T*)p.norm_w + k) : z;
  }
#pragma unroll
  for (int i = 0; i < SC; ++i) {
    if constexpr (WAVES == 4) {
      sq[i] = xq[i];
    } else {
      const int c = wave + 4 * i, k = c * 512 + lane * 8;
      const rw_u32x4 z = {0u, 0u, 0u, 0u};
      sq[i] = (wave < 4 && c < NCH && k < p.K) ? *reinterpret_cast<const rw_u32x4*>((const T*)p.X + k) : z;
    }
  }
  int rows[R];
#pragma unroll
  for (int r = 0; r < R; ++r) {
    if constexpr (EPI == EPI_SWIGLU) {
      int n = g * RR + (r % RR); n = n < n_out ? n : n_out - 1;
      rows[r] = 32 * (n >> 4) + (n & 15) + (r / RR) * 16;
    } else {
      const int n = g * R + r;
      rows[r] = n < p.N ? n : p.N - 1;
    }
  }
  typedef typename RwW<F8>::type wreg_t;
  wreg_t w[R][NCH];
#pragma unroll
  for (int r = 0; r < R; ++r)
#pragma unroll
    for (int c = 0; c < NCH; ++c) {
      int k = c * 512 + lane * 8;
      k = k < p.K ? k : 0;
      w[r][c] = rw_ldw<T, F8>(p, (size_t)rows[r], k);
    }
  float e_bias[RR], e_scale[R];
  {
    const T* bp = (EPI != EPI_SWIGLU && p.bias) ? (const T*)p.bias : (const T*)p.norm_w;
    const int nmax = (EPI != EPI_SWIGLU && p.bias) ? n_out - 1 : 0;
#pragma unroll
    for (int r = 0; r < RR; ++r) {
      const int n = g * RR + r;
      e_bias[r] = tof(bp[n < nmax ? n : nmax]);
    }
    if (!(EPI != EPI_SWIGLU && p.bias)) {
#pragma unroll
      for (int r = 0; r < RR; ++r) e_bias[r] = 0.f;
    }
#pragma unroll
    for (int r = 0; r < R; ++r) e_scale[r] = 1.f;
    if constexpr (F8 == WF_E4M3) {
#pragma unroll
      for (int r = 0; r < R; ++r) e_scale[r] = p.w_scale[rows[r]];
    }
  }
  __builtin_amdgcn_sched_barrier(0);
  float ss = 0.f;
#pragma unroll
  for (int i = 0; i < SC; ++i) {
    const v8 xv = __builtin_bit_cast(v8, sq[i]);
#pragma unroll
    for (int j = 0; j < 8; ++j) { const float v = tof(xv[j]); ss += v * v; }
  }
#pragma unroll
  for (int o = 32; o > 0; o >>= 1) ss += __shfl_xor(ss, o, 64);
  if (lane == 0 && wave < 4) red[wave] = ss;
  asm volatile("s_waitcnt lgkmcnt(0)" ::: "memory");
  __builtin_amdgcn_s_barrier();
  float tot = red[0];
#pragma unroll
  for (int w = 1; w < 4; ++w) tot += red[w];
  const float inv = rsqrtf(tot / (float)p.K + p.norm_eps);
#pragma unroll
  for (int i = 0; i < MC; ++i) {
    const int c = wave + WAVES * i;
    if (c < NCH) {
      const v8 xv = __builtin_bit_cast(v8, xq[i]), wv = __builtin_bit_cast(v8, nq[i]);
      v8 o;
#pragma unroll
      for (int j = 0; j < 8; ++j) o[j] = fromf<T>(tof(wv[j]) * rnd<T>(tof(xv[j]) * inv));
      *reinterpret_cast<v8*>(xs + c * 512 + lane * 8) = o;
    }
  }
  asm volatile("s_waitcnt lgkmcnt(0)" ::: "memory");
  __builtin_amdgcn_s_barrier();
  rw_u32x4 xr[NCH];
#pragma unroll
  for (int c = 0; c < NCH; ++c) xr[c] = *reinterpret_cast<const rw_u32x4*>(xs + c * 512 + lane * 8);
  __builtin_amdgcn_sched_barrier(0);
  float acc[R];
#pragma unroll
  for (int r = 0; r < R; ++r) {
    float a = 0.f;
#pragma unroll
    for (int c = 0; c < NCH; ++c) {
      a = rw_dotw<T, F8>(w[r][c], xr[c], a);
    }
#pragma unroll
    for (int o = 32; o > 0; o >>= 1) a += __shfl_xor(a, o, 64);
    if constexpr (F8 == WF_E4M3) a *= e_scale[r];
    acc[r] = a;
  }
  if (lane == 0) {
#pragma unroll
    for (int r = 0; r < RR; ++r) {
      const int n = g * RR + r;
      if (n >= n_out) continue;
      if constexpr (EPI == EPI_SWIGLU) {
        const float gt = rnd<T>(acc[r]), up = rnd<T>(acc[r + RR]);
        ((T*)p.Y)[n] = fromf<T>(rnd<T>(silu(gt)) * up);
      } else {
        const float y = acc[r] + e_bias[r];
        if (p.out_f32) ((float*)p.Y)[n] = y;
        else ((T*)p.Y)[n] = fromf<T>(y);
      }
    }
  }
  if constexpr (EPI == EPI_SWIGLU) { OM_DBG_MAX(5, blockIdx.x + 64 >= gridDim.x); OM_DBG_MAX(16 + (blockIdx.x & 7), blockIdx.x + 512 >= gridDim.x); }
  if constexpr (EPI == EPI_NONE) OM_DBG_MAX(9, (blockIdx.x & 7) == 0);
}

template <typename T, int EPI, int RR, int NCH, bool F8, int WAVES = 4>
__global__ __launch_bounds__(WAVES * 64) void gemv_rows_norm_kernel(GemvP p) { gemv_rows_norm_body<T, EPI, RR, NCH, F8 ? WF_E4M3 : WF_16, WAVES>(p); }
template <typename T, int EPI, int RR, int NCH, int WAVES = 4>
__global__ __launch_bounds__(WAVES * 64) void gemv_rows_norm_mx4_kernel(GemvP p) { gemv_rows_norm_body<T, EPI, RR, NCH, WF_MX4, WAVES>(p); }

template <typename T, int EPI, int NCH, int F8>
__device__ __forceinline__ void gemv_rows_norm_loop_body(const GemvP& p, int per_wg, unsigned skew) {
  typedef typename V8<T>::type v8;
  constexpr int R = EPI == EPI_SWIGLU ? 2 : 1;
  __shared__ __attribute__((aligned(16))) T xs[NCH * 512];
  __shared__ float red[4];
  const int lane = threadIdx.x & 63, wave = __builtin_amdgcn_readfirstlane(threadIdx.x >> 6);
  const int n_out = EPI == EPI_SWIGLU ? p.N / 2 : p.N;
  int o0 = blockIdx.x * per_wg, o1 = o0 + per_wg < n_out ? o0 + per_wg : n_out;
  if constexpr (EPI == EPI_SWIGLU) OM_DBG_MIN(4, blockIdx.x < 8);
  if (skew) {
    const int l = blockIdx.x & 7;
    int pre = 0;
    for (int i = 0; i < l; ++i) pre += per_wg + (int)((skew >> (4 * i)) & 15u) - 8;
    o0 = (blockIdx.x >> 3) * 8 * per_wg + pre;
    o1 = o0 + per_wg + (int)((skew >> (4 * l)) & 15u) - 8;
    o1 = o1 < n_out ? o1 : n_out;
  }
  typedef typename RwW<F8>::type wreg_t;
  auto row_of = [&](int n, int r) { return EPI == EPI_SWIGLU ? 32 * (n >> 4) + (n & 15) + r * 16 : n; };
  auto load_w = [&](wreg_t (&w)[R][NCH], int n) {
#pragma unroll
    for (int r = 0; r < R; ++r) {
      const size_t row = (size_t)row_of(n, r);
#pragma unroll
      for (int c = 0; c < NCH; ++c) {
        int k = c * 512 + lane * 8;
        k = k < p.K ? k : 0;
        w[r][c] = rw_ldw<T, F8>(p, row, k);
      }
    }
  };
  wreg_t wa[R][NCH], wb[R][NCH], wc[R][NCH];
  const int u0 = o0 + wave;
  if (u0 < o1) load_w(wa, u0);
  if (u0 + 4 < o1) load_w(wb, u0 + 4);
  if (u0 + 8 < o1) load_w(wc, u0 + 8);
  constexpr int MC = (NCH + 3) / 4;
  rw_u32x4 xq[MC], nq[MC];
#pragma unroll
  for (int i = 0; i < MC; ++i) {
// ... 326 lines not shown
    }
  };
  auto load_x = [&](rw_u32x4 (&x)[8], int pass) {
#pragma unroll
    for (int c = 0; c < 8; ++c) {
      const int k = (pass * 8 + c) * 512 + lane * 8;
      const rw_u32x4 z = {0u, 0u, 0u, 0u};
      x[c] = k < p.K ? *reinterpret_cast<const rw_u32x4*>((const T*)p.X + k) : z;
    }
  };
  float acc = 0.f;
  auto dots = [&](wreg_t (&w)[8], rw_u32x4 (&x)[8]) {
#pragma unroll
    for (int c = 0; c < 8; ++c) {
      acc = rw_dotw<T, F8>(w[c], x[c], acc);
    }
  };
  wreg_t wa[8], wb[8];
  rw_u32x4 xa[8], xb[8];
  load_w(wa, 0);
  load_x(xa, 0);
  if (npass > 1) { load_w(wb, 1); load_x(xb, 1); }
  const float e_bias_raw = tof(((const T*)(p.bias ? p.bias : p.X))[p.bias ? row : 0]);
  const float e_res_raw = tof(((const T*)(p.resid ? p.resid : p.X))[p.resid ? row : 0]);
  const float e_bias = p.bias ? e_bias_raw : 0.f, e_res = p.resid ? e_res_raw : 0.f;
  float e_scale = 1.f;
  if constexpr (F8 == WF_E4M3) e_scale = p.w_scale[row];
  for (int ps = 0; ps < npass; ps += 2) {
    dots(wa, xa);
    if (ps + 2 < npass) { load_w(wa, ps + 2); load_x(xa, ps + 2); }
    if (ps + 1 < npass) {
      dots(wb, xb);
      if (ps + 3 < npass) { load_w(wb, ps + 3); load_x(xb, ps + 3); }
    }
  }
  float a = acc;
#pragma unroll
  for (int o = 32; o > 0; o >>= 1) a += __shfl_xor(a, o, 64);
  if constexpr (F8 == WF_E4M3) a *= e_scale;
  if (lane == 0) {
    const float y = rnd<T>(a + e_bias);
    ((T*)p.Y)[n] = fromf<T>(e_res + y);
  }
}

template <typename T, bool F8>
__global__ __launch_bounds__(256) void gemv_rows_longk_direct_kernel(GemvP p) { gemv_rows_longk_direct_body<T, F8 ? WF_E4M3 : WF_16>(p); }
template <typename T>
__global__ __launch_bounds__(256) void gemv_rows_longk_direct_mx4_kernel(GemvP p) { gemv_rows_longk_direct_body<T, WF_MX4>(p); }

#endif
int g_gemv_longk_direct = 0;

template <typename T>
int launch_rows_longk(const GemvP& p, hipStream_t s) {
#if OMCHAT_EXPERIMENTS
  if (g_gemv_longk_direct > 0) {
    const int wpw = g_gemv_longk_direct > 4 ? 4 : g_gemv_longk_direct;
    if (p.mx_s) hipLaunchKernelGGL((gemv_rows_longk_direct_mx4_kernel<T>), dim3(cdiv(p.N, wpw)), dim3(64 * wpw), 0, s, p);
    else if (p.w_scale) hipLaunchKernelGGL((gemv_rows_longk_direct_kernel<T, true>), dim3(cdiv(p.N, wpw)), dim3(64 * wpw), 0, s, p);
    else hipLaunchKernelGGL((gemv_rows_longk_direct_kernel<T, false>), dim3(cdiv(p.N, wpw)), dim3(64 * wpw), 0, s, p);
    return 0;
  }
#endif
  const int n_cu = device_cus();
  int rpw = cdiv(p.N, 2 * n_cu);
  rpw = rpw < 1 ? 1 : (rpw > 8 ? 8 : rpw);
  const int grid = cdiv(p.N, rpw);
  const int npass = (cdiv(p.K, 512) + 7) / 8;
  const size_t lds = (size_t)npass * 8 * 512 * 2;
  if (p.mx_s) {
    static PerDeviceOnce set;
    auto k = gemv_rows_longk_mx4_kernel<T>;
    if (set.first()) OM_HIP(hipFuncSetAttribute((const void*)k, hipFuncAttributeMaxDynamicSharedMemorySize, 64 * 1024));
    hipLaunchKernelGGL(k, dim3(grid), dim3(64 * rpw), lds, s, p, rpw);
  } else if (p.w_scale) {
    auto k = gemv_rows_longk_kernel<T, true>;
    static PerDeviceOnce set;
    if (set.first()) OM_HIP(hipFuncSetAttribute((const void*)k, hipFuncAttributeMaxDynamicSharedMemorySize, 64 * 1024));
    hipLaunchKernelGGL(k, dim3(grid), dim3(64 * rpw), lds, s, p, rpw);
  } else {
    auto k = gemv_rows_longk_kernel<T, false>;
    static PerDeviceOnce set;
    if (set.first()) OM_HIP(hipFuncSetAttribute((const void*)k, hipFuncAttributeMaxDynamicSharedMemorySize, 64 * 1024));
    hipLaunchKernelGGL(k, dim3(grid), dim3(64 * rpw), lds, s, p, rpw);
  }
  return 0;
}

int g_gemv_rows_balance = 1;
unsigned g_gemv_skew = 0;
int g_gemv_dyn = 0;
int g_gemv_gu_rr = 1;
int g_gemv_gu_rr8 = 1;
int g_gemv_norm_loop = 0;

template <typename T, int EPI, int RR, int F8, int NCH>
void launch_rows_norm_n(const GemvP& p, hipStream_t s) {
  const int n_out = EPI == EPI_SWIGLU ? p.N / 2 : p.N;
  if constexpr (NCH >= 4) {
    const bool want = EPI == EPI_SWIGLU ? (g_gemv_norm_loop & (F8 != WF_16 ? 4 : 1)) : (p.N < 32768 ? (g_gemv_norm_loop & 2) : (g_gemv_norm_loop & 8));
    const int n_cu = device_cus();
#if OMCHAT_EXPERIMENTS
    if (want && p.dyn && g_gemv_dyn && n_out >= 8 * n_cu) {
      if constexpr (F8 == WF_MX4) hipLaunchKernelGGL((gemv_rows_norm_dyn_mx4_kernel<T, EPI, NCH>), dim3(2 * n_cu), dim3(256), 0, s, p);
      else hipLaunchKernelGGL((gemv_rows_norm_dyn_kernel<T, EPI, NCH, F8 == WF_E4M3>), dim3(2 * n_cu), dim3(256), 0, s, p);
      return;
    }
#endif
    if (want && n_out >= 8 * n_cu) {
      const int per = cdiv(n_out, 2 * n_cu);
      const unsigned skew = (g_gemv_skew >= 256u && n_out == per * 2 * n_cu && (2 * n_cu) % 8 == 0) ? g_gemv_skew : 0u;
      if constexpr (F8 == WF_MX4) hipLaunchKernelGGL((gemv_rows_norm_loop_mx4_kernel<T, EPI, NCH>), dim3(cdiv(n_out, per)), dim3(256), 0, s, p, per, skew);
      else hipLaunchKernelGGL((gemv_rows_norm_loop_kernel<T, EPI, NCH, F8 == WF_E4M3>), dim3(cdiv(n_out, per)), dim3(256), 0, s, p, per, skew);
      return;
    }
  }
  if constexpr (NCH >= 4 && EPI == EPI_NONE && RR <= 2) {
    const int n_cu = device_cus();
    if (g_gemv_rows_balance && n_out == 9 * 2 * n_cu) {
      if constexpr (F8 == WF_MX4) hipLaunchKernelGGL((gemv_rows_norm_mx4_kernel<T, EPI, 1, NCH, 9>), dim3(2 * n_cu), dim3(576), 0, s, p);
      else hipLaunchKernelGGL((gemv_rows_norm_kernel<T, EPI, 1, NCH, F8 == WF_E4M3, 9>), dim3(2 * n_cu), dim3(576), 0, s, p);
      return;
    }
  }
#if OMCHAT_EXPERIMENTS
  if constexpr (EPI == EPI_SWIGLU && RR == 1) {
    const int nwg = cdiv(n_out, 4), xs = (int)(g_gemv_skew < 256u ? g_gemv_skew : 0u);
    if (xs > 0 && nwg % 8 == 0 && n_out % 4 == 0 && xs < nwg / 8) {
      GemvP q = p; q.xskew = xs;
      if constexpr (F8 == WF_MX4) hipLaunchKernelGGL((gemv_rows_norm_mx4_kernel<T, EPI, RR, NCH>), dim3(8 * (nwg / 8 + xs)), dim3(256), 0, s, q);
      else hipLaunchKernelGGL((gemv_rows_norm_kernel<T, EPI, RR, NCH, F8 == WF_E4M3>), dim3(8 * (nwg / 8 + xs)), dim3(256), 0, s, q);
      return;
    }
  }
#endif
  if constexpr (F8 == WF_MX4) hipLaunchKernelGGL((gemv_rows_norm_mx4_kernel<T, EPI, RR, NCH>), dim3(cdiv(cdiv(n_out, RR), 4)), dim3(256), 0, s, p);
  else hipLaunchKernelGGL((gemv_rows_norm_kernel<T, EPI, RR, NCH, F8 == WF_E4M3>), dim3(cdiv(cdiv(n_out, RR), 4)), dim3(256), 0, s, p);
}
template <typename T, int EPI, int RR, int F8>
void launch_rows_norm(const GemvP& p, hipStream_t s) {
  switch (cdiv(p.K, 512)) {
    case 1: launch_rows_norm_n<T, EPI, RR, F8, 1>(p, s); break;
    case 2: launch_rows_norm_n<T, EPI, RR, F8, 2>(p, s); break;
    case 3: launch_rows_norm_n<T, EPI, RR, F8, 3>(p, s); break;
    case 4: launch_rows_norm_n<T, EPI, RR, F8, 4>(p, s); break;
    case 5: launch_rows_norm_n<T, EPI, RR, F8, 5>(p, s); break;
    case 6: launch_rows_norm_n<T, EPI, RR, F8, 6>(p, s); break;
    case 7: launch_rows_norm_n<T, EPI, RR, F8, 7>(p, s); break;
    default: launch_rows_norm_n<T, EPI, RR, F8, 8>(p, s); break;
  }
}

template <typename T, int EPI, int RR, int F8>
void launch_rows_r(const GemvP& p, hipStream_t s) {
  const int n_out = EPI == EPI_SWIGLU ? p.N / 2 : p.N;
  if constexpr (RR == 1 && EPI == EPI_RESID) {
    const int n_cu = device_cus();
    if (g_gemv_rows_balance && p.ksplit == 1 && n_out == 7 * 2 * n_cu) {
      if constexpr (F8 == WF_MX4) hipLaunchKernelGGL((gemv_rows_mx4_kernel<T, EPI, 1, 7>), dim3(2 * n_cu, 1), dim3(448), 0, s, p);
      else hipLaunchKernelGGL((gemv_rows_kernel<T, EPI, 1, 7, F8 == WF_E4M3>), dim3(2 * n_cu, 1), dim3(448), 0, s, p);
      return;
    }
  }
  int grid = cdiv(cdiv(n_out, RR), 4);
  grid = grid > 2048 ? 2048 : grid;
  if constexpr (F8 == WF_MX4) hipLaunchKernelGGL((gemv_rows_mx4_kernel<T, EPI, RR, 4>), dim3(grid, p.ksplit), dim3(256), 0, s, p);
  else hipLaunchKernelGGL((gemv_rows_kernel<T, EPI, RR, 4, F8 == WF_E4M3>), dim3(grid, p.ksplit), dim3(256), 0, s, p);
}
template <typename T, int EPI, int WF>
void launch_rows_q(const GemvP& p, hipStream_t s) {
  if constexpr (EPI == EPI_SWIGLU || EPI == EPI_NONE) {
    if (p.norm_w) {
      if (EPI == EPI_NONE && p.N < 32768) launch_rows_norm<T, EPI, 2, WF>(p, s);
      else if (EPI == EPI_SWIGLU && g_gemv_gu_rr8 == 2) launch_rows_norm<T, EPI, 2, WF>(p, s);
      else if (EPI == EPI_SWIGLU && g_gemv_gu_rr8 == 1) launch_rows_norm<T, EPI, 1, WF>(p, s);
      else launch_rows_norm<T, EPI, 4, WF>(p, s);
      return;
    }
  }
  if ((EPI == EPI_NONE || EPI == EPI_RESID) && p.N < 32768) launch_rows_r<T, EPI, 1, WF>(p, s);
  else if (EPI == EPI_NONE) launch_rows_r<T, EPI, 8, WF>(p, s);
  else launch_rows_r<T, EPI, 4, WF>(p, s);
}
template <typename T, int EPI>
void launch_rows(const GemvP& p, hipStream_t s) {
  if (p.mx_s) { launch_rows_q<T, EPI, WF_MX4>(p, s); return; }
  if (p.w_scale) { launch_rows_q<T, EPI, WF_E4M3>(p, s); return; }
  if constexpr (EPI == EPI_SWIGLU || EPI == EPI_NONE) {
    if (p.norm_w) {
      if (EPI == EPI_NONE && p.N < 32768) launch_rows_norm<T, EPI, 2, WF_16>(p, s);
      else if (EPI == EPI_SWIGLU && g_gemv_gu_rr == 2) launch_rows_norm<T, EPI, 2, WF_16>(p, s);
      else if (EPI == EPI_SWIGLU && g_gemv_gu_rr == 3) launch_rows_norm<T, EPI, 3, WF_16>(p, s);
      else if (EPI == EPI_SWIGLU) launch_rows_norm<T, EPI, 1, WF_16>(p, s);
      else launch_rows_norm<T, EPI, 4, WF_16>(p, s);
      return;
    }
  }
  if ((EPI == EPI_NONE || EPI == EPI_RESID) && p.N < 32768) launch_rows_r<T, EPI, 1, WF_16>(p, s);
  else if (EPI == EPI_SWIGLU && (g_gemv_shard & 4) && p.N / 2 < 16 * device_cus()) launch_rows_r<T, EPI, 1, WF_16>(p, s);
  else launch_rows_r<T, EPI, 4, WF_16>(p, s);
}

template <typename T>
int launch_t(const GemvArgs& a, hipStream_t s) {
  const int ks = a.ksplit > 1 ? a.ksplit : 1;
  GemvP p{a.X, a.W, a.Y, a.bias, a.resid, a.ldx, a.ldw, a.ldy, a.ldr, a.b, a.N, a.K, a.out_f32, ks, a.w_scale, a.y_packed, a.norm_w, a.norm_eps,
          (unsigned*)a.dyn_ctr, a.y_pack, a.dbg, a.mx_scale};
  if (a.norm_w && a.x_packed && !(a.w_packed && ks == 1 && (a.K >> 6) == 56 && a.epi == EPI_SWIGLU && a.N % 32 == 0 && !g_gemv_no_xs)) {
    omchat_set_error("launch_gemv: the in-register RMSNorm on packed x exists for the x-stationary gate|up form only (packed W, K = 3584, no split-K)");
    return 1;
  }
  if (a.epi == EPI_RESID && a.x_packed && !(a.w_packed && ks == 1 && (a.K >> 6) == 56 && a.N % 16 == 0 && a.N / 16 <= device_cus() && !g_gemv_no_xs)) {
    omchat_set_error("launch_gemv: the batched residual epilogue exists for the x-stationary form only (packed W, K = 3584, N / 16 <= CUs, no split-K)");
    return 1;
  }
  if (a.x_packed) {
#define OM_PK(NT_, EPI_, WV_, UN_)                                                                                                  \
  do {                                                                                                                              \
    const dim3 grid(cdiv(cdiv(a.N, 16), NT_), ks);                                                                                  \
    if (a.mx_scale) { if (a.b > 16) hipLaunchKernelGGL((gemv_pk_mx4_kernel<T, NT_, EPI_, WV_, UN_, 2>), grid, dim3(WV_ * 64), 0, s, p);     \
                      else hipLaunchKernelGGL((gemv_pk_mx4_kernel<T, NT_, EPI_, WV_, UN_, 1>), grid, dim3(WV_ * 64), 0, s, p); }             \
    else if (a.b > 16) { if (a.w_packed) hipLaunchKernelGGL((gemv_pk_kernel<T, NT_, EPI_, WV_, UN_, 2, true>), grid, dim3(WV_ * 64), 0, s, p);   \
                    else hipLaunchKernelGGL((gemv_pk_kernel<T, NT_, EPI_, WV_, UN_, 2, false>), grid, dim3(WV_ * 64), 0, s, p); }            \
    else { if (a.w_packed) hipLaunchKernelGGL((gemv_pk_kernel<T, NT_, EPI_, WV_, UN_, 1, true>), grid, dim3(WV_ * 64), 0, s, p);            \
           else hipLaunchKernelGGL((gemv_pk_kernel<T, NT_, EPI_, WV_, UN_, 1, false>), grid, dim3(WV_ * 64), 0, s, p); }                     \
  } while (0)
    const int n_cu = device_cus();
    if (a.mx_scale && (a.norm_w || a.epi == EPI_RESID)) {
      omchat_set_error("launch_gemv: the batched norm-in-GEMV / residual forms read 16-bit weights only (no MXFP4 instantiation)");
      return 1;
    }
#if !OMCHAT_EXPERIMENTS
    if (a.norm_w || a.epi == EPI_RESID) { omchat_set_error("launch_gemv: the batched norm-in-GEMV / residual forms need a -DOMCHAT_EXPERIMENTS=1 build"); return 1; }
#else
    if (a.w_packed && ks == 1 && !g_gemv_no_xs && (a.K >> 6) == 56 && a.epi == EPI_RESID) {
      const dim3 grid(a.N / 16);
      if (a.b > 16) hipLaunchKernelGGL((gemv_xs_kernel<T, EPI_RESID, 2, 7>), grid, dim3(512), 0, s, p);
      else hipLaunchKernelGGL((gemv_xs_kernel<T, EPI_RESID, 1, 7>), grid, dim3(512), 0, s, p);
      OM_LAUNCH_CHECK();
      return 0;
    }
#endif
    if (a.w_packed && ks == 1 && !g_gemv_no_xs && (a.K >> 6) == 56 && a.N % 32 == 0 && (a.epi == EPI_SWIGLU || a.epi == EPI_NONE) &&
        ((a.epi == EPI_SWIGLU ? a.N / 32 : a.N / 16) >= 4 * n_cu || (a.epi == EPI_NONE && a.N / 16 >= n_cu && a.N / 16 <= 2 * n_cu) ||
         ((g_gemv_shard & 1) && a.epi == EPI_NONE && a.N / 16 < n_cu) || ((g_gemv_shard & 8) && a.epi == EPI_SWIGLU && a.N / 32 <= n_cu))) {
      const dim3 grid((a.epi == EPI_SWIGLU ? a.N / 32 : a.N / 16) >= 4 * n_cu ? n_cu : (a.epi == EPI_SWIGLU ? a.N / 32 : a.N / 16 < n_cu ? a.N / 16 : a.N / 32));
#if OMCHAT_EXPERIMENTS
      if (a.epi == EPI_SWIGLU && a.norm_w) {
        if (a.b > 16) hipLaunchKernelGGL((gemv_xs_kernel<T, EPI_SWIGLU, 2, 7, true>), grid, dim3(512), 0, s, p);
        else hipLaunchKernelGGL((gemv_xs_kernel<T, EPI_SWIGLU, 1, 7, true>), grid, dim3(512), 0, s, p);
      } else
#endif
      if (a.mx_scale) {
        if (a.epi == EPI_SWIGLU) {
          if (a.b > 16) hipLaunchKernelGGL((gemv_xs_mx4_kernel<T, EPI_SWIGLU, 2, 7>), grid, dim3(512), 0, s, p);
          else hipLaunchKernelGGL((gemv_xs_mx4_kernel<T, EPI_SWIGLU, 1, 7>), grid, dim3(512), 0, s, p);
        } else {
          if (a.b > 16) hipLaunchKernelGGL((gemv_xs_mx4_kernel<T, EPI_NONE, 2, 7>), grid, dim3(512), 0, s, p);
          else hipLaunchKernelGGL((gemv_xs_mx4_kernel<T, EPI_NONE, 1, 7>), grid, dim3(512), 0, s, p);
        }
// ... 320 lines not shown
```

omchat_amd/csrc/kernels.h:

```cpp
#pragma once
#ifndef OMCHAT_EXPERIMENTS
#define OMCHAT_EXPERIMENTS 0
#endif
#include "common.h"
#if OMCHAT_EXPERIMENTS
#include <hip/hip_ext.h>
extern int g_launch_any_order;
#undef hipLaunchKernelGGL
#define hipLaunchKernelGGL(kernelName, numBlocks, numThreads, memPerBlock, streamId, ...)                                                      \
  do {                                                                                                                                         \
    if (g_launch_any_order)                                                                                                                    \
      hipExtLaunchKernelGGL((kernelName), dim3(numBlocks), dim3(numThreads), (memPerBlock), (streamId), nullptr, nullptr, hipExtAnyOrderLaunch, \
                            __VA_ARGS__);                                                                                                      \
    else                                                                                                                                       \
      hipLaunchKernelGGLInternal((kernelName), numBlocks, numThreads, memPerBlock, streamId, __VA_ARGS__);                                     \
  } while (0)
#endif

enum {
  EPI_NONE = 0,
  EPI_GELU = 1,
  EPI_LS_RESID = 2,
  EPI_RESID = 3,
  EPI_SWIGLU = 4,
  EPI_PARTIAL = 5,
  EPI_F32OUT = 6,
  EPI_LS_RESID_STATS = 7,
  EPI_NONE_STATS = 8,
};
struct GemmArgs {
  const void* A; int lda;
  const void* W; int ldw;
  void* C; int ldc;
  int M, N, K;
  const void* bias;
  const void* ls;
  const void* resid;
  int ldr;
  int epi;
  int force_tile;
  void* sk_ws; size_t sk_ws_bytes;
  int stream_k;
  int f8;
  const float* a_scale; const float* w_scale;
  const float* row_scale = nullptr;
  const float* rs_stats = nullptr; int rs_ld = 0, rs_nslots = 0, rs_dim = 0; float rs_eps = 0.f;
  float* stats = nullptr; int stats_ld = 0; int* stats_nslots = nullptr;
};
int launch_gemm(int dtype, const GemmArgs& a, hipStream_t stream);
int launch_stats_finish(const float* stats, int ld, int slot0, int nslots, int ngroups, int rows, int dim, float eps, float* out, hipStream_t s);
int launch_row_sumsq(int dtype, const void* x, int ldx, int rows, int H, float* stats, hipStream_t s);
size_t gemm_sk_ws_bytes();
void gemm_set_skew(int v);
void gemm_set_persist(int v);
void gemm_set_wide_store(int v);
void gemm_set_skip_dead(int v);

struct GemvArgs {
  const void* X; int ldx;
  const void* W; int ldw;
  void* Y; int ldy;
  int b, N, K;
  const void* bias;
  const void* resid; int ldr;
  int epi;
  int out_f32;
  int ksplit;
  int force_mfma;
  const float* w_scale;
  int x_packed;
  int w_packed;
  int y_packed;
  const void* norm_w; float norm_eps;
  void* dyn_ctr = nullptr;
  void* y_pack = nullptr;
  unsigned long long* dbg = nullptr;
  const unsigned char* mx_scale = nullptr;
};
int launch_pack_x(int dtype, const void* X, int ldx, int b, int K, void* out, hipStream_t s);
int launch_pack_w(int dtype, const void* W, int ldw, int N, int K, void* out, hipStream_t s);
int launch_pack_w4(const void* W4, const unsigned char* S, int N, int K, void* W4P, unsigned char* SP, hipStream_t s);
int launch_gemv(int dtype, const GemvArgs& a, hipStream_t stream);
int launch_gemv_wait(int dtype, const GemvArgs& a, const unsigned* flags, unsigned epoch, int nflags, unsigned* err, int mode, hipStream_t s);
int launch_quant_fp8_rows(int dtype, const void* W, int ldw, int N, int K, void* W8, int ld8, float* scale, hipStream_t stream);
int launch_quant_mxfp4_rows(int dtype, const void* W, int ldw, int N, int K, void* W4, int ld4, unsigned char* S, hipStream_t stream);
void gemv_set_force_mfma(int v);
int gemv_get_force_mfma();
void gemm_set_autotune(int v);
int gemm_tune_load(const char* path);
int gemm_tune_dump(const char* path);
long gemm_tune_runs();
void model_set_ar_min_rows(int v);
void model_set_tp_f32(int v);
void model_set_pack_replica(int v);
void model_set_norm_in_gemv(int v);
void model_set_vit_fused(int v);
void model_set_tp_sp(int v);
int launch_fold_cols(int dtype, const void* W, const void* n, void* out, int rows, int cols, hipStream_t s);

int launch_layernorm(int dtype, const void* x, int ldx, const void* w, const void* b, void* y, int ldy, int rows, int H, float eps, hipStream_t stream);
int launch_rmsnorm(int dtype, const void* x, int ldx, const void* w, void* y, int ldy, int rows, int H, float eps, hipStream_t s, int pack_nb = 0);
int launch_rmsnorm_q8(int dtype, const void* x, int ldx, const void* w, void* y8, int ldy, float* scale, int rows, int H, float eps, hipStream_t s);
int launch_quant_rows_q8(int dtype, const void* x, int ldx, void* y8, int ldy, float* scale, int rows, int H, hipStream_t s);
int launch_resid_rmsnorm(int dtype, void* x, int ldx, const float* part, int ks, const void* w, void* xn, int ldn, int rows, int H, float eps,
                         hipStream_t s, int pack_nb = 0);
int launch_resid16_norm(int dtype, void* x, int ldx, const void* y, int ldy, const void* w, const void* b, void* xn, int ldn, int rows, int H, float eps,
                        hipStream_t s);
int launch_vit_qknorm(int dtype, void* qkv, int ld, const void* wq, const void* wk, int rows, int C, int C_total,
                      float eps, float q_scale, const float* sumsq_in, hipStream_t s, int only_k = 0);
int launch_vit_qk_sumsq(int dtype, const void* qkv, int ld, int rows, int C, float* sumsq_out, hipStream_t s);
int launch_vit_knorm_slots(int dtype, void* k, int ld, const void* wk, int rows, int C, int C_total, float eps, const float* stats, int stats_ld, int nslots,
                           float* sumsq_q, hipStream_t s);
struct AttnArgs {
  const void* Q; int64_t q_sb, q_sh, q_sr;
  const void* K; int64_t k_sb, k_sh, k_sr;
  const void* V; int64_t v_sb, v_sh, v_sr;
  void* O; int64_t o_sb, o_sh, o_sr;
  int batch, q_heads, kv_heads;
  int Sq, Skv;
  const int* kv_len;
  const int* kv_start;
  int causal;
  int q_pos0;
  float scale;
  int head_dim;
  const float* qn_sumsq = nullptr; int qn_stride = 0, qn_dim = 0; const void* qn_w = nullptr; float qn_eps = 0.f, qn_scale = 1.f;
};
int launch_attn_prefill(int dtype, const AttnArgs& a, hipStream_t s);
int launch_attn_uniform_rows(int dtype, const AttnArgs& a, hipStream_t s);
void attn_set_v2(int v);
// ... 40 lines not shown
  const void* k_new; const void* v_new; int64_t new_sb;
  int o_pack_nb;
  const float* k_scale; const float* v_scale; int64_t scale_sb, scale_sh;
  void* k16_w = nullptr; void* v16_w = nullptr;
  const unsigned char* key_mask; int64_t mask_sb;
  unsigned* done_flags = nullptr; unsigned done_epoch = 0; int done_mode = 0;
  unsigned long long* done_dbg = nullptr;
};
int launch_kv_quant(int dtype, const void* kc, const void* vc, void* k8, void* v8, float* ks, float* vs, int b, int kv_heads, int64_t c_sb, int64_t c_sh,
                    int64_t s_sb, int64_t s_sh, const int* pos_lo, int pos0, const int* len, int max_rows, hipStream_t s);
size_t attn_decode_ws_bytes(int batch, int q_heads, int max_len);
int launch_attn_decode(int dtype, const AttnDecodeArgs& a, hipStream_t s);

struct AttnVerifyArgs {
  const void* Q; int64_t q_sb, q_sh;
  void* K; int64_t k_sh, k_sr;
  void* V; int64_t v_sh, v_sr;
  void* O; int64_t o_sb, o_sh;
  int T, q_heads, kv_heads, L;
  float scale;
  float* ws; size_t ws_bytes;
  const float* rope; int rope_max;
  const void* k_new; const void* v_new; int64_t new_sb;
  int o_pack_nb;
};
constexpr int VERIFY_MAX_T = 16;
int launch_attn_verify(int dtype, const AttnVerifyArgs& a, hipStream_t s);
int attn_verify_tpw(int keys, int kv_heads);

struct AttnExtendArgs {
  const void* Q; int64_t q_sb, q_sh;
  const void* K; int64_t k_sh, k_sr;
  const void* V; int64_t v_sh, v_sr;
  void* O; int64_t o_sb, o_sh;
  int Sq, q_heads, kv_heads, L;
  float scale;
  float* ws; size_t ws_bytes;
};
size_t attn_extend_ws_bytes(int Sq, int q_heads, int kv_heads, int L);
int launch_attn_extend(int dtype, const AttnExtendArgs& a, hipStream_t s);

struct FusedDecodeArgs {
  const void* Wo; int ldw;
  void* x; int H, qd;
  void* ws; unsigned epoch;
  unsigned* err; int timeout_ms;
  void* dbg = nullptr;
};
size_t fused_decode_ws_bytes(int q_heads);
bool attn_oproj_fused_ok(const AttnDecodeArgs& a, int H, int qd);
int launch_attn_oproj_fused(int dtype, const AttnDecodeArgs& a, const FusedDecodeArgs& f, hipStream_t s);
void model_set_fuse_attn_oproj(int v);
void model_set_decode_layer(int v);
void model_set_shard_as_tp1(int v);

struct DecodeLayerArgs {
  const void *ln1, *ln2, *wqkv, *bqkv, *wo, *wgu, *wd;
  void *kc, *vc; int64_t k_sh;
  void* x;
  int H, qd, kvd, It, q_heads, kv_heads, kv_len;
  const float* rope; int rope_max;
  float eps, scale;
  void* ws; unsigned epoch;
  unsigned* err; int timeout_ms;
  void* dbg = nullptr;
};
size_t decode_layer_ws_bytes(int q_heads, int H, int qd, int kvd, int It);
bool decode_layer_ok(const DecodeLayerArgs& a);
int launch_decode_layer(int dtype, const DecodeLayerArgs& a, hipStream_t s);

struct RopeArgs {
  void* qkv; int ld;
  int rows, S;
  int nq, nkv;
  const int* pos;
  int pos0;
  const float* cos_sin;
  int max_pos;
  void* kcache; void* vcache;
  int64_t c_sb, c_sh;
  void* k8 = nullptr; void* v8 = nullptr; float* ks = nullptr; float* vs = nullptr; int64_t s_sb = 0, s_sh = 0;
  int slot0 = -1;
};
int launch_rope_kv(int dtype, const RopeArgs& a, hipStream_t s);

int launch_im2col(int dtype, const void* pixels, void* cols, int B, int HW, int patch, int Kpad, hipStream_t s);
int launch_vit_assemble(int dtype, const void* pe, const void* cls, const void* pos, void* x, int B, int np, int C, hipStream_t s);
int launch_tp_finish(int dtype, const float* sum, const void* bias, const void* ls, const void* resid, void* out, int M, int N, int epi, hipStream_t s);
int launch_gather_rows(int dtype, const int* idx, const void* table, const void* feats, void* out, int rows, int H, hipStream_t s);
int launch_copy_rows(int dtype, const void* src, int64_t src_ld, void* dst, int64_t dst_ld, int rows, int H,
                     int group, int skip, hipStream_t s);
size_t argmax_scratch_bytes(int b);
int launch_argmax(const float* logits, int ld, int b, int V, int* out, void* scratch, hipStream_t s, int* adv_pos = nullptr, int* adv_len = nullptr);
struct SampleFilters {
  double min_p = -1.0, typical_p = 1.0, epsilon = 1.0, eta = 1.0;
  bool min_p_on() const { return min_p >= 0.0; }
  bool typical_on() const { return typical_p < 1.0; }
  bool epsilon_on() const { return epsilon < 1.0; }
  bool eta_on() const { return eta < 1.0; }
  bool any() const { return min_p_on() || typical_on() || epsilon_on() || eta_on(); }
  bool operator==(const SampleFilters& o) const { return min_p == o.min_p && typical_p == o.typical_p && epsilon == o.epsilon && eta == o.eta; }
};
struct SampleArgs {
  const float* logits = nullptr; int ld = 0, b = 0, V = 0, V_total = 0;
  int rank = 0, tp = 1;
  uint64_t seed = 0; float temperature = 1.f; int top_k = 0; double top_p = 1.0; float penalty = 1.f;
  SampleFilters f;
  uint32_t* bitmap = nullptr; int bm_words = 0;
  int* last_set = nullptr;
  int* step = nullptr;
  int* adv_pos = nullptr; int* adv_len = nullptr;
  int* out = nullptr; uint32_t* thr_out = nullptr;
  uint32_t* hi_out = nullptr;
  void* ws = nullptr;
  float* table = nullptr;
  const int32_t* vtokens = nullptr;
  uint32_t* vseen = nullptr;
  int (*xchg)(void* user, float* buf, size_t count, hipStream_t s) = nullptr;
  void* xchg_user = nullptr;
};
constexpr int SMP_VERIFY_ROWS = VERIFY_MAX_T;
size_t sample_ws_bytes(int b);
int launch_sample(const SampleArgs& a, hipStream_t s);
int launch_sample_rewind(uint32_t* bitmap, int bm_words, int* last_set, int* step, int b, int n, hipStream_t s);
int launch_sample_rewind_verify(uint32_t* bitmap, int* vlast, int* step, int cnt, int r, hipStream_t s);
const uint32_t* sample_thr_words(const void* ws, int b, int V_total, int top_k, double top_p, const SampleFilters& f, int* stride,
                                 const uint32_t** hi);
struct LogprobArgs {
  const float* raw = nullptr; int raw_ld = 0;
  const float* proc = nullptr; int proc_ld = 0;
  int b = 0, V = 0, rank = 0, tp = 1;
  const int* ids = nullptr;
  const uint32_t* ban = nullptr;
  const uint32_t* seen = nullptr; int bm_words = 0; const int* last_set = nullptr;
  float temperature = 1.f, penalty = 1.f;
  const uint32_t* thr = nullptr; const uint32_t* thr_hi = nullptr; int thr_stride = 1; int top1 = 0;
  void* ws = nullptr;
  float* table = nullptr;
  int (*xchg)(void* user, float* buf, size_t count, hipStream_t s) = nullptr;
  void* xchg_user = nullptr;
  float* rec = nullptr; int* cnt = nullptr; int max_new = 0, rec_ld = 0;
};
size_t logprob_ws_bytes(int b);
size_t logprob_table_bytes(int b, int tp);
int launch_logprob(const LogprobArgs& a, hipStream_t s);
// ... 51 lines not shown
```

omchat_amd/csrc/model.hip:

```cpp
#include "ctx.h"
#include <limits.h>
#include <math.h>
#include <string.h>
#include <algorithm>
#include <functional>
#include <string>
#include <unordered_map>
#include <vector>

static thread_local std::string g_err;
void omchat_set_error(const std::string& s) { g_err = s; }
extern "C" const char* omchat_last_error(void) { return g_err.c_str(); }
extern "C" const char* omchat_version(void) { return "omchat_hip 0.1 (gfx950)"; }

namespace {

__global__ void cast_from_f32_f16(const float* s, f16* d, int64_t n) {
  for (int64_t i = (int64_t)blockIdx.x * blockDim.x + threadIdx.x; i < n; i += (int64_t)gridDim.x * blockDim.x) d[i] = (f16)s[i];
}
__global__ void cast_from_f32_bf16(const float* s, bf16* d, int64_t n) {
  for (int64_t i = (int64_t)blockIdx.x * blockDim.x + threadIdx.x; i < n; i += (int64_t)gridDim.x * blockDim.x) d[i] = (bf16)s[i];
}
__global__ void add_positions_kernel(int* pos, int b, int d) {
  const int i = threadIdx.x;
// ... 9 lines not shown
  while (n < T - 1 && tokens[n + 1] == picks[n]) ++n;
  const int kept = keep_all ? T : n + 1;
  pos[0] = L + kept; len[0] = L + kept + 1;
  n_out[0] = n;
}
__global__ void verify_accept_sample_kernel(const int32_t* tokens, const int32_t* picks, int T, int L, int* pos, int* len, int* n_out,
                                            uint32_t* bm, int gbase, int V, int* vlast, int* last, int* step) {
  if (threadIdx.x != 0) return;
  int n = 0;
  while (n < T - 1 && tokens[n + 1] == picks[n]) ++n;
  for (int i = 0; i < VERIFY_MAX_T; ++i) {
    int set = -1;
    if (bm && i <= n) {
      const int id = picks[i];
      const int li = id >= gbase ? id - gbase : -1;
      if (id >= 0 && li >= 0 && li < V) {
        const uint32_t bit = 1u << (li & 31);
        if (!(bm[li >> 5] & bit)) { bm[li >> 5] |= bit; set = li; }
      }
    }
    vlast[i] = set;
  }
  last[0] = -1;
  step[0] += n + 1;
  pos[0] = L + n + 1; len[0] = L + n + 2;
  n_out[0] = n;
}
__global__ void last_row_index_kernel(const int* len, int S, int b, int* idx, int keep) {
  const int i = threadIdx.x;
  if (i < b) idx[i] = i * S + len[i] - keep - 1;
}

constexpr int DEC_KS_MAX = 8;

}

#if !OMCHAT_EXPERIMENTS
size_t fused_decode_ws_bytes(int) { return 0; }
bool attn_oproj_fused_ok(const AttnDecodeArgs&, int, int) { return false; }
int launch_attn_oproj_fused(int, const AttnDecodeArgs&, const FusedDecodeArgs&, hipStream_t) { omchat_set_error("fused decode launch: build with -DOMCHAT_EXPERIMENTS=1"); return 1; }
size_t decode_layer_ws_bytes(int, int, int, int, int) { return 0; }
bool decode_layer_ok(const DecodeLayerArgs&) { return false; }
int launch_decode_layer(int, const DecodeLayerArgs&, hipStream_t) { omchat_set_error("one-launch decode layer: build with -DOMCHAT_EXPERIMENTS=1"); return 1; }
#endif
extern "C" int omchat_has_experiments(void) { return OMCHAT_EXPERIMENTS; }
int g_shard_as_tp1 = 0;
void model_set_shard_as_tp1(int v) { g_shard_as_tp1 = v; }
int g_decode_layer = 0;
void model_set_decode_layer(int v) { g_decode_layer = v; }
int g_fuse_attn_oproj = 0;
void model_set_fuse_attn_oproj(int v) { g_fuse_attn_oproj = v; }
int g_ao_oproj = 0;
void model_set_ao_oproj(int v) { g_ao_oproj = v; }
int g_fuse_peer_norm = 1;
void model_set_fuse_peer_norm(int v) { g_fuse_peer_norm = v; }

namespace {

int add_route(omchat_ctx* ctx, const std::string& name, void** slot, int64_t rows, int64_t cols, float std_, float off,
              int kind = R_PLAIN, void* dst_override = nullptr, int64_t dst_ld = -1) {
  Route r;
  r.rows = rows; r.cols = cols; r.kind = kind; r.synth_std = std_; r.synth_off = off;
  if (dst_override) {
    r.dst = dst_override;
  } else {
    TRY(ctx->alloc(&r.dst, (size_t)rows * cols * 2));
    if (slot) *slot = r.dst;
  }
  r.dst_ld = dst_ld < 0 ? cols : dst_ld;
  ctx->routes[name] = r;
  return 0;
}

int build(omchat_ctx* ctx) {
  const omchat_config& c = ctx->c;
  const int C = c.v_hidden, I = c.v_mlp;
  ctx->v_np = (c.v_image / c.v_patch) * (c.v_image / c.v_patch);
  ctx->v_ntok = ctx->v_np + 1;
  ctx->v_hd = c.v_head_dim ? c.v_head_dim : 128;
  ctx->v_Cq = c.v_heads * ctx->v_hd;
  const int K = 3 * c.v_patch * c.v_patch;
  ctx->v_kpad = cdiv(K, 64) * 64;
  const std::string TW = "model.vision_tower.vision_tower.";

  if (c.v_layers > 0) {
    TRY(add_route(ctx, TW + "embeddings.class_embedding", &ctx->v_cls, 1, C, 0.02f, 0.f));
    TRY(add_route(ctx, TW + "embeddings.position_embedding", &ctx->v_pos, ctx->v_ntok, C, 0.02f, 0.f));
    TRY(ctx->alloc(&ctx->v_wpatch, (size_t)C * ctx->v_kpad * 2));
    OM_HIP(hipMemset(ctx->v_wpatch, 0, (size_t)C * ctx->v_kpad * 2));
    TRY(add_route(ctx, TW + "embeddings.patch_embedding.weight", nullptr, C, K, 0.02f, 0.f, R_PATCH, ctx->v_wpatch, ctx->v_kpad));
    TRY(add_route(ctx, TW + "embeddings.patch_embedding.bias", &ctx->v_bpatch, 1, C, 0.02f, 0.f));
    ctx->vl.resize(c.v_layers);
    for (int j = 0; j < c.v_layers; ++j) {
      const std::string P = TW + "encoder.layers." + std::to_string(j) + ".";
      auto& L = ctx->vl[j];
      TRY(add_route(ctx, P + "ls1", &L.ls1, 1, C, 0.02f, 0.1f));
      TRY(add_route(ctx, P + "ls2", &L.ls2, 1, C, 0.02f, 0.1f));
      TRY(add_route(ctx, P + "norm1.weight", &L.n1, 1, C, 0.05f, 1.f));
      TRY(add_route(ctx, P + "norm2.weight", &L.n2, 1, C, 0.05f, 1.f));
      L.n1b = L.n2b = L.qn = L.kn = nullptr;
      if (c.v_norm_type == 1) {
        TRY(add_route(ctx, P + "norm1.bias", &L.n1b, 1, C, 0.02f, 0.f));
        TRY(add_route(ctx, P + "norm2.bias", &L.n2b, 1, C, 0.02f, 0.f));
      }
      TRY(add_route(ctx, P + "attn.qkv.weight", &L.wqkv, 3 * ctx->v_Cq, C, 0.02f, 0.f));
      if (!c.v_no_qk_norm) {
// ... 1049 lines not shown
static int ensure_packed(omchat_ctx* ctx) {
  if (!g_pack_replica || ctx->pk_ready || ctx->pk_unavailable) return 0;
  const omchat_config& c = ctx->c;
  const int H = c.t_hidden, It = c.t_mlp, qkvd = ctx->t_qkvdim, qd = ctx->t_qdim;
  if (qkvd % 16 || H % 16 || c.t_vocab % 16) return 0;
  if (ctx->dlp.empty()) {
    std::vector<omchat_ctx::DecLayerP> fresh(c.t_layers);
    std::vector<void*> got;
    void* lmP = nullptr;
    auto grab = [&](void** p, size_t n) -> bool {
      if (hipMalloc(p, n) != hipSuccess) { (void)hipGetLastError(); *p = nullptr; return false; }
      got.push_back(*p);
      return true;
    };
    bool ok = true;
    for (auto& P : fresh) {
      ok = ok && grab(&P.wqkv, (size_t)qkvd * H * 2) && grab(&P.wo, (size_t)H * qd * 2) && grab(&P.wgu, (size_t)2 * It * H * 2) &&
           grab(&P.wd, (size_t)H * It * 2);
      if (!ok) break;
    }
    ok = ok && grab(&lmP, (size_t)c.t_vocab * H * 2);
    if (!ok) {
      for (void* p : got) (void)hipFree(p);
      ctx->pk_unavailable = true;
      return 0;
    }
    for (void* p : got) ctx->allocs.push_back(p);
    ctx->bytes += (size_t)c.t_layers * ((size_t)qkvd * H + (size_t)H * qd + (size_t)2 * It * H + (size_t)H * It) * 2 + (size_t)c.t_vocab * H * 2;
    ctx->dlp.swap(fresh);
    ctx->t_lmP = lmP;
  }
  for (int i = 0; i < c.t_layers; ++i) {
    auto& L = ctx->dl[i]; auto& P = ctx->dlp[i];
    TRY(launch_pack_w(ctx->dt, L.wqkv, H, qkvd, H, P.wqkv, nullptr));
    TRY(launch_pack_w(ctx->dt, L.wo, qd, H, qd, P.wo, nullptr));
    TRY(launch_pack_w(ctx->dt, L.wgu, H, 2 * It, H, P.wgu, nullptr));
    TRY(launch_pack_w(ctx->dt, L.wd, It, H, It, P.wd, nullptr));
  }
  TRY(launch_pack_w(ctx->dt, ctx->t_lm, H, c.t_vocab, H, ctx->t_lmP, nullptr));
  OM_HIP(hipDeviceSynchronize());
  ctx->pk_ready = true;
  return 0;
}

static const char* const MX4_ROWS_MSG = "MXFP4 decode mode 2 streams steps of at most 32 rows (omchat_enable_mxfp4_decode(ctx, 0 or 1) first)";

static int decode_body(omchat_ctx* ctx, const int32_t* tokens, int b, int Lmax, float* logits, int32_t* next_tokens, hipStream_t s, bool allow_prof,
                       bool exact_len = false, bool masked = false, int vL = -1, bool vsample = false) {
  const omchat_config& c = ctx->c;
  const int H = c.t_hidden, It = c.t_mlp, qkvd = ctx->t_qkvdim, qd = ctx->t_qdim;
  const bool lead = ctx->tp_rank == 0;
  void* x = ctx->tw_x;
  void* y = ctx->tw_x2;
  TRY(launch_gather_rows(ctx->dt, tokens, ctx->t_embed, nullptr, x, b, H, s));
  const bool f8 = ctx->fp8_decode && b == 1;
  const bool mx4 = ctx->mx4_step(b);
  const bool wq = f8 || mx4;
  const int pk = (b > 1 && b <= 32 && H % 64 == 0 && qd % 64 == 0 && It % 64 == 0) ? (b > 16 ? 2 : 1) : 0;
  const bool wpk = pk && ctx->pk_ready;
  const bool mpk = pk && mx4;
  OM_CHECK(!mx4 || b == 1 || mpk, "MXFP4 decode mode 2: geometry outside the packed path");
  static const omchat_ctx::DecLayerP noneP{};
  auto gemv_args = [&](const void* X, int ldx, const void* W, int K, void* Y, int ldy, int R, int N, const void* bias, const void* resid, int epi,
                       int ks, const void* W8, const float* sc, const void* WP, bool ypk, const void* W4 = nullptr, const unsigned char* s4 = nullptr) {
    GemvArgs g{X, ldx, W, K, Y, ldy, R, N, K, bias, resid, H, epi, 0, ks};
    if (f8 && W8) { g.W = W8; g.w_scale = sc; }
    if (mx4 && W4) { g.W = W4; g.ldw = K / 2; g.mx_scale = s4; }
    if (pk) {
      g.x_packed = 1; g.y_packed = ypk && epi == EPI_SWIGLU;
      if (mpk) g.w_packed = 1;
      else if (wpk && WP) { g.W = WP; g.w_packed = 1; }
    }
    return g;
  };
  auto gemv = [&](const void* X, int ldx, const void* W, int K, void* Y, int ldy, int N, const void* bias, const void* resid, int epi,
                  const void* W8 = nullptr, const float* sc = nullptr, const void* WP = nullptr, bool ypk = false, const void* W4 = nullptr,
                  const unsigned char* s4 = nullptr) -> int {
    for (int r0 = 0; r0 < b; r0 += 32) {
      const int R = std::min(32, b - r0);
      const GemvArgs g = gemv_args((const char*)X + (size_t)r0 * ldx * 2, ldx, W, K, (char*)Y + (size_t)r0 * ldy * 2, ldy, R, N, bias,
                                   resid ? (const char*)resid + (size_t)r0 * H * 2 : nullptr, epi, 0, W8, sc, WP, ypk, W4, s4);
      TRY(launch_gemv(ctx->dt, g, s));
    }
    return 0;
  };
  auto gemv_partial = [&](const void* X, int ldx, const void* W, int K, int ks, const void* W8 = nullptr, const float* sc = nullptr,
                          const void* WP = nullptr, const void* W4 = nullptr, const unsigned char* s4 = nullptr) -> int {
    OM_CHECK(b <= 32, "split-K decode path handles b <= 32");
    const GemvArgs g = gemv_args(X, ldx, W, K, ctx->tw_part, H, b, H, nullptr, nullptr, EPI_PARTIAL, ks, W8, sc, WP, false, W4, s4);
    TRY(launch_gemv(ctx->dt, g, s));
    return 0;
  };
  const bool fused = b <= 32;
  auto ks_rows = [&](int K) { const int nch = cdiv(K, 512); return nch >= 16 ? std::min(DEC_KS_MAX, nch) : std::max(1, std::min(3, nch)); };
  auto ks_short = [&](int K) { return std::max(1, std::min(DEC_KS_MAX, (K / 64) / 16)); };
  const bool shard_ks = (gemv_get_shard_shapes() & 2) != 0;
  const int ks_o = b == 1 ? ks_rows(qd) : ((wpk || mpk) && qd == 3584 ? 2 : (shard_ks && qd / 64 <= 64) ? ks_short(qd) :
                                           std::max(1, std::min(DEC_KS_MAX, std::min(qd / 64, cdiv(512, cdiv(H, 16))))));
  const int ks_d = b == 1 ? ks_rows(It) : (shard_ks && It / 64 <= 64) ? ks_short(It) :
                                          std::max(1, std::min(DEC_KS_MAX, std::min(It / 64, 3 * cdiv(512, cdiv(H, 16)))));
  const bool tp1_like = ctx->tp_size == 1 || (OMCHAT_EXPERIMENTS && g_shard_as_tp1 && ctx->hook == omchat_allreduce_noop);
  const bool n2 = (g_norm_in_gemv & 1) && fused && b == 1 && tp1_like && qd <= 4096 && H <= 4096 && !gemv_get_force_mfma();
  const bool n1 = n2 && (g_norm_in_gemv & 2) && It <= 32768 && It % 8 == 0;
  const bool nb2 = OMCHAT_EXPERIMENTS && (g_norm_in_gemv & 4) && fused && wpk && ctx->tp_size == 1 && !wq && (qd >> 6) == 56 && (H >> 6) == 56 && qd % 64 == 0 &&
                   H / 16 <= device_cus() && (2 * It) / 32 >= 4 * device_cus();
  if (fused && !n1) TRY(launch_rmsnorm(ctx->dt, x, H, ctx->dl[0].ln1, ctx->tw_xn, H, b, H, c.t_eps, s, pk));
#if OMCHAT_EXPERIMENTS
  if ((g_ao_oproj & 16) && ctx->dbg_stamps) OM_HIP(hipMemsetAsync(ctx->dbg_stamps, 0, (size_t)c.t_layers * 256, s));
#endif
  for (int i = 0; i < c.t_layers; ++i) {
    auto& L = ctx->dl[i];
    static const omchat_ctx::DecLayer8 none8{};
    const omchat_ctx::DecLayer8& Q = f8 ? ctx->dl8[i] : none8;
    static const omchat_ctx::DecLayer4 none4{};
    const omchat_ctx::DecLayer4& M = mx4 ? (mpk ? ctx->dl4p[i] : ctx->dl4[i]) : none4;
    const omchat_ctx::DecLayerP& P = wpk ? ctx->dlp[i] : noneP;
    char* kc = (char*)ctx->kcache + (size_t)i * ctx->cache_layer_stride() * 2;
    char* vc = (char*)ctx->vcache + (size_t)i * ctx->cache_layer_stride() * 2;
    if (!fused) TRY(launch_rmsnorm(ctx->dt, x, H, L.ln1, ctx->tw_xn, H, b, H, c.t_eps, s));
    if (g_decode_layer && n1 && exact_len && !masked && !wq && !(ctx->fp8_kv && ctx->kv8_valid) && ctx->dl_ws) {
      DecodeLayerArgs d{L.ln1, L.ln2, L.wqkv, L.bqkv, L.wo, L.wgu, L.wd, kc, vc, ctx->cache_sh(), x, H, qd, ctx->t_kvdim, It, c.t_heads, c.t_kv_heads, Lmax,
                        ctx->rope, c.max_seq, c.t_eps, 0.08838834764831845f, ctx->dl_ws, ++ctx->fd_epoch, ctx->fd_err, 2000};
      if (decode_layer_ok(d)) {
        const bool mark_l = allow_prof && i == c.t_layers / 2;
        if (mark_l) ctx->prof_mark(OMCHAT_PROF_DECODE_GATEUP, s);
        TRY(launch_decode_layer(ctx->dt, d, s));
        if (mark_l) ctx->prof_mark(OMCHAT_PROF_DECODE_GATEUP, s);
        ++ctx->n_layer_launches;
        continue;
      }
      --ctx->fd_epoch;
    }
    if (n1) {
      GemvArgs g = gemv_args(x, H, L.wqkv, H, ctx->tw_qkv, qkvd, 1, qkvd, L.bqkv, nullptr, EPI_NONE, 0, Q.wqkv, Q.sqkv, nullptr, false, M.wqkv, M.sqkv);
      g.norm_w = L.ln1; g.norm_eps = c.t_eps;
      if (OMCHAT_EXPERIMENTS && (g_ao_oproj & 16) && ctx->dbg_stamps) g.dbg = ctx->dbg_stamps + (size_t)i * 32;
      TRY(launch_gemv(ctx->dt, g, s));
    } else {
      TRY(gemv(ctx->tw_xn, H, L.wqkv, H, ctx->tw_qkv, qkvd, qkvd, L.bqkv, nullptr, EPI_NONE, Q.wqkv, Q.sqkv, P.wqkv, false, M.wqkv, M.sqkv));
    }
    AttnDecodeArgs a{};
    a.Q = ctx->tw_qkv; a.q_sb = qkvd; a.q_sh = 128;
    a.K = kc; a.k_sb = ctx->cache_sb(); a.k_sh = ctx->cache_sh(); a.k_sr = 128;
    a.V = vc; a.v_sb = a.k_sb; a.v_sh = a.k_sh; a.v_sr = 128;
    a.O = ctx->tw_ao; a.o_sb = qd; a.o_sh = 128;
    a.batch = b; a.q_heads = c.t_heads; a.kv_heads = c.t_kv_heads; a.L = Lmax; a.kv_len = ctx->d_len; a.scale = 0.08838834764831845f;
    a.ws = ctx->tw_attn_ws; a.ws_bytes = ctx->tw_attn_ws_bytes;
    a.rope = ctx->rope; a.rope_max = c.max_seq; a.pos = ctx->d_pos;
    a.k_new = (const char*)ctx->tw_qkv + (size_t)qd * 2; a.v_new = (const char*)ctx->tw_qkv + (size_t)(qd + ctx->t_kvdim) * 2; a.new_sb = qkvd;
    if (exact_len) a.kv_len = nullptr;
    if (masked) { a.key_mask = ctx->d_mask; a.mask_sb = ctx->mask_sb; }
    if (ctx->fp8_kv && ctx->kv8_valid) {
      const size_t off = (size_t)i * ctx->cache_layer_stride(), so = (size_t)i * ctx->scale_layer_stride();
      RopeArgs r{ctx->tw_qkv, qkvd, b, 1, c.t_heads, c.t_kv_heads, ctx->d_pos, 0, ctx->rope, c.max_seq, kc, vc, ctx->cache_sb(), ctx->cache_sh()};
      r.k8 = (char*)ctx->k8cache + off; r.v8 = (char*)ctx->v8cache + off; r.ks = ctx->ks8 + so; r.vs = ctx->vs8 + so;
      r.s_sb = (int64_t)c.t_kv_heads * c.max_seq; r.s_sh = c.max_seq;
      if (masked) r.slot0 = Lmax - 1;
      else if (exact_len) { r.pos = nullptr; r.pos0 = Lmax - 1; }
      if (attn_decode_kv8_fuses_rope(b, c.t_kv_heads, Lmax, masked)) { a.k16_w = kc; a.v16_w = vc; a.pos = nullptr; }
      else {
        TRY(launch_rope_kv(ctx->dt, r, s));
        a.rope = nullptr; a.pos = nullptr; a.k_new = nullptr; a.v_new = nullptr;
      }
      a.K = (char*)ctx->k8cache + off; a.V = (char*)ctx->v8cache + off;
      a.k_scale = ctx->ks8 + so; a.v_scale = ctx->vs8 + so; a.scale_sb = (int64_t)c.t_kv_heads * c.max_seq; a.scale_sh = c.max_seq;
    }
    a.o_pack_nb = fused ? pk : 0;
    bool ao_oproj = false;
    const bool fuse_ao = g_fuse_attn_oproj && n2 && exact_len && !wq && a.rope && ctx->fd_ws && attn_oproj_fused_ok(a, H, qd);
    if (vL >= 0) {
      AttnVerifyArgs va{};
      va.Q = ctx->tw_qkv; va.q_sb = qkvd; va.q_sh = 128;
      va.K = kc; va.k_sh = ctx->cache_sh(); va.k_sr = 128;
      va.V = vc; va.v_sh = ctx->cache_sh(); va.v_sr = 128;
      va.O = ctx->tw_ao; va.o_sb = qd; va.o_sh = 128;
      va.T = b; va.q_heads = c.t_heads; va.kv_heads = c.t_kv_heads; va.L = vL; va.scale = a.scale;
      va.ws = ctx->tw_attn_ws; va.ws_bytes = ctx->tw_attn_ws_bytes;
      va.rope = ctx->rope; va.rope_max = c.max_seq; va.k_new = a.k_new; va.v_new = a.v_new; va.new_sb = qkvd;
      va.o_pack_nb = a.o_pack_nb;
      TRY(launch_attn_verify(ctx->dt, va, s));
    } else if (fuse_ao) {
      FusedDecodeArgs fa{L.wo, qd, x, H, qd, ctx->fd_ws, ++ctx->fd_epoch, ctx->fd_err, 2000};
      TRY(launch_attn_oproj_fused(ctx->dt, a, fa, s));
      ++ctx->n_fused_launches;
    } else {
#if OMCHAT_EXPERIMENTS
      ao_oproj = (g_ao_oproj & 1) && n2 && !wq && !masked && ctx->fd_ws && Lmax <= 4096 && H == 3584 && qd == 3584 && c.t_heads <= 64 && !ctx->graph_on;
      if (ao_oproj) { a.done_flags = (unsigned*)ctx->fd_ws; a.done_epoch = ++ctx->fd_epoch; a.done_mode = g_ao_oproj; }
      if ((g_ao_oproj & 16) && n2 && ctx->dbg_stamps) a.done_dbg = ctx->dbg_stamps + (size_t)i * 32;
#endif
      TRY(launch_attn_decode(ctx->dt, a, s));
    }
    if (fuse_ao) {
    } else if (ao_oproj) {
      GemvArgs g = gemv_args(ctx->tw_ao, qd, L.wo, qd, x, H, 1, H, nullptr, x, EPI_RESID, 0, nullptr, nullptr, nullptr, false);
      if ((g_ao_oproj & 16) && ctx->dbg_stamps) g.dbg = ctx->dbg_stamps + (size_t)i * 32;
      TRY(launch_gemv_wait(ctx->dt, g, (const unsigned*)ctx->fd_ws, ctx->fd_epoch, c.t_heads, ctx->fd_err, g_ao_oproj, s));
    } else if (n2 && OMCHAT_EXPERIMENTS && (g_ao_oproj & 16) && ctx->dbg_stamps && !wq) {
      GemvArgs g = gemv_args(ctx->tw_ao, qd, L.wo, qd, x, H, 1, H, nullptr, x, EPI_RESID, 0, nullptr, nullptr, nullptr, false);
      g.dbg = ctx->dbg_stamps + (size_t)i * 32;
      TRY(launch_gemv(ctx->dt, g, s));
    } else if (n2) {
      TRY(gemv(ctx->tw_ao, qd, L.wo, qd, x, H, H, nullptr, x, EPI_RESID, Q.wo, Q.so, nullptr, false, M.wo, M.so));
    } else if (nb2) {
      GemvArgs g = gemv_args(ctx->tw_ao, qd, L.wo, qd, x, H, b, H, nullptr, x, EPI_RESID, 0, nullptr, nullptr, P.wo, false);
      g.y_pack = ctx->tw_xn;
      TRY(launch_gemv(ctx->dt, g, s));
    } else if (fused) {
      TRY(gemv_partial(ctx->tw_ao, qd, L.wo, qd, ks_o, Q.wo, Q.so, P.wo, M.wo, M.so));
      TRY(ctx->reduce_resid_rmsnorm(x, H, ctx->tw_part, ks_o, L.ln2, ctx->tw_xn, H, b, H, c.t_eps, pk, s));
    } else if (ctx->tp_size == 1) {
      TRY(gemv(ctx->tw_ao, qd, L.wo, qd, x, H, H, nullptr, x, EPI_RESID));
    } else {
      TRY(gemv(ctx->tw_ao, qd, L.wo, qd, y, H, H, nullptr, lead ? x : nullptr, lead ? EPI_RESID : EPI_NONE));
      TRY(ctx->allreduce(y, (size_t)b * H, s));
      std::swap(x, y);
    }
    if (!fused) TRY(launch_rmsnorm(ctx->dt, x, H, L.ln2, ctx->tw_xn, H, b, H, c.t_eps, s));
    const bool mark = allow_prof && i == c.t_layers / 2;
    if (mark) ctx->prof_mark(OMCHAT_PROF_DECODE_GATEUP, s);
    if (n2) {
      GemvArgs g = gemv_args(x, H, L.wgu, H, ctx->tw_act, It, 1, 2 * It, nullptr, nullptr, EPI_SWIGLU, 0, Q.wgu, Q.sgu, nullptr, false, M.wgu, M.sgu);
      g.norm_w = L.ln2; g.norm_eps = c.t_eps;
      if (ctx->dyn_ctr && !ctx->graph_on) g.dyn_ctr = ctx->dyn_ctr + (size_t)i * 65 * 64;
      if (OMCHAT_EXPERIMENTS && (g_ao_oproj & 16) && ctx->dbg_stamps) g.dbg = ctx->dbg_stamps + (size_t)i * 32;
      TRY(launch_gemv(ctx->dt, g, s));
    } else if (nb2) {
      GemvArgs g = gemv_args(ctx->tw_xn, H, L.wgu, H, ctx->tw_act, It, b, 2 * It, nullptr, nullptr, EPI_SWIGLU, 0, nullptr, nullptr, P.wgu, true);
      g.norm_w = L.ln2; g.norm_eps = c.t_eps;
      TRY(launch_gemv(ctx->dt, g, s));
    } else {
      TRY(gemv(ctx->tw_xn, H, L.wgu, H, ctx->tw_act, It, 2 * It, nullptr, nullptr, EPI_SWIGLU, Q.wgu, Q.sgu, P.wgu, true, M.wgu, M.sgu));
    }
    if (mark) ctx->prof_mark(OMCHAT_PROF_DECODE_GATEUP, s);
    if (n1 && OMCHAT_EXPERIMENTS && (g_ao_oproj & 16) && ctx->dbg_stamps && !wq) {
      GemvArgs g = gemv_args(ctx->tw_act, It, L.wd, It, x, H, 1, H, nullptr, x, EPI_RESID, 0, nullptr, nullptr, nullptr, false);
      g.dbg = ctx->dbg_stamps + (size_t)i * 32;
      TRY(launch_gemv(ctx->dt, g, s));
    } else if (n1) {
      TRY(gemv(ctx->tw_act, It, L.wd, It, x, H, H, nullptr, x, EPI_RESID, Q.wd, Q.sd, nullptr, false, M.wd, M.sd));
    } else if (fused) {
      TRY(gemv_partial(ctx->tw_act, It, L.wd, It, ks_d, Q.wd, Q.sd, P.wd, M.wd, M.sd));
      const void* nw = i + 1 < c.t_layers ? ctx->dl[i + 1].ln1 : ctx->t_norm;
      TRY(ctx->reduce_resid_rmsnorm(x, H, ctx->tw_part, ks_d, nw, ctx->tw_xn, H, b, H, c.t_eps, pk, s));
    } else if (ctx->tp_size == 1) {
      TRY(gemv(ctx->tw_act, It, L.wd, It, x, H, H, nullptr, x, EPI_RESID));
    } else {
      TRY(gemv(ctx->tw_act, It, L.wd, It, y, H, H, nullptr, lead ? x : nullptr, lead ? EPI_RESID : EPI_NONE));
      TRY(ctx->allreduce(y, (size_t)b * H, s));
      std::swap(x, y);
    }
  }
  if (!fused)   TRY(launch_rmsnorm(ctx->dt, x, H, ctx->t_norm, ctx->tw_xn, H, b, H, c.t_eps, s));
  float* lg = logits ? logits : ctx->tw_logits;
  if (n1) {
    GemvArgs g{x, H, ctx->t_lm, H, lg, c.t_vocab, 1, c.t_vocab, H, nullptr, nullptr, 0, EPI_NONE, 1};
    if (f8) { g.W = ctx->t_lm8; g.w_scale = ctx->t_lm8_s; }
    if (mx4) { g.W = ctx->t_lm4; g.ldw = H / 2; g.mx_scale = ctx->t_lm4_s; }
    g.norm_w = ctx->t_norm; g.norm_eps = c.t_eps;
    TRY(launch_gemv(ctx->dt, g, s));
  } else {
    TRY(lm_head_rows(ctx, ctx->tw_xn, b, lg, s, f8, fused && pk, mx4));
  }
  if (vL >= 0) TRY(pick_verify(ctx, lg, b, tokens, next_tokens, s, vsample));
  else if (next_tokens) TRY(pick_run(ctx, lg, b, next_tokens, s, true, tokens));
  else {
    hipLaunchKernelGGL(advance_lens_kernel, dim3(1), dim3(64 > b ? 64 : b), 0, s, ctx->d_pos, ctx->d_len, b);
    TRY(pick_feed(ctx, tokens, b, s));
  }
  OM_LAUNCH_CHECK();
  return 0;
}

static void destroy_graph(omchat_ctx::DecodeGraph& g) {
  if (g.exec) (void)hipGraphExecDestroy(g.exec);
  if (g.graph) (void)hipGraphDestroy(g.graph);
  g = omchat_ctx::DecodeGraph{};
}

void drop_decode_graphs(omchat_ctx* ctx) {
  for (auto& kv : ctx->graphs) destroy_graph(kv.second);
  ctx->graphs.clear();
}


extern "C" int omchat_enable_decode_graph(omchat_ctx* ctx, int on) {
  OM_CHECK(ctx, "null ctx");
  OM_CHECK(ctx->c.t_layers > 0, "context has no decoder");
  if (on && !ctx->graph_stream) {
    OM_HIP(hipStreamCreateWithFlags(&ctx->graph_stream, hipStreamNonBlocking));
    OM_HIP(hipEventCreateWithFlags(&ctx->graph_ev_in, hipEventDisableTiming));
    OM_HIP(hipEventCreateWithFlags(&ctx->graph_ev_out, hipEventDisableTiming));
    TRY(ctx->alloc((void**)&ctx->d_tok_in, (size_t)ctx->c.max_batch * 4));
    TRY(ctx->alloc((void**)&ctx->d_tok_out, (size_t)ctx->c.max_batch * 4));
  }
  ctx->graph_on = on != 0;
  return 0;
}

extern "C" int omchat_decode_graph_stats(omchat_ctx* ctx, long* steps, long* replays, long* captures) {
  OM_CHECK(ctx, "null ctx");
  if (steps) *steps = ctx->graph_steps;
  if (replays) *replays = ctx->graph_replays;
  if (captures) *captures = ctx->graph_captures;
  return 0;
}

extern "C" int omchat_decode_step(omchat_ctx* ctx, const int32_t* tokens, int b, float* logits, int32_t* next_tokens, void* stream) {
  OM_CHECK(ctx && tokens, "null argument");
  const omchat_config& c = ctx->c;
  OM_CHECK(c.t_layers > 0, "context has no decoder");
  OM_CHECK(b >= 1 && b <= c.max_batch, "batch exceeds max_batch");
  OM_CHECK(ctx->mx4_rows_ok(b), MX4_ROWS_MSG);
  int Lmax = 0;
  OM_CHECK(!ctx->left_padded, "per-sequence decode after a left-padded prefill: use omchat_decode_step_masked (the reference positions such a "
                              "batch with sum(mask) - 1 and a per-row key mask, omchat_arch.py:61-70; DESIGN.md section 7)");
  OM_CHECK(ctx->dec_mode != 2, "omchat_decode_step after omchat_decode_step_masked on the same prefill: the two place the cache rows differently");
  bool same_len = true;
  for (int i = 0; i < b; ++i) {
    OM_CHECK(ctx->h_len[i] >= 1, "decode before prefill");
    Lmax = std::max(Lmax, ctx->h_len[i] + 1);
    same_len = same_len && ctx->h_len[i] == ctx->h_len[0];
  }
// ... 317 lines not shown
```

omchat_amd/csrc/pick.hip:

```cpp
#include "ctx.h"
#include <math.h>
#include <algorithm>

namespace {

__global__ void tp_argmax_scatter_kernel(const float* logits, int ld, const int* local_idx, int b, int rank, int v_local, float* table) {
  const int i = threadIdx.x;
  if (i < b) {
    table[((size_t)rank * b + i) * 2] = logits[(size_t)i * ld + local_idx[i]];
    table[((size_t)rank * b + i) * 2 + 1] = (float)(rank * v_local + local_idx[i]);
  }
}
__global__ void tp_argmax_pick_kernel(const float* table, int b, int size, int* out) {
  const int i = threadIdx.x;
  if (i < b) {
    float best = table[(size_t)i * 2]; int bi = (int)table[(size_t)i * 2 + 1];
    for (int r = 1; r < size; ++r) {
      const float v = table[((size_t)r * b + i) * 2];
      if (v > best) { best = v; bi = (int)table[((size_t)r * b + i) * 2 + 1]; }
    }
    out[i] = bi;
  }
}

// ... 8 lines not shown
  a.ngram = P.con.ngram; a.min_new = P.con.min_new; a.min_len = P.con.min_len;
  constrain_bind_lists(P.con_lists, a);
  a.n_eos = P.con.n_eos; a.n_sup = P.con.n_sup; a.n_bsup = P.con.n_bsup; a.n_bw = P.con.n_bw;
  a.ban = P.con_ban; a.bmw = P.con_bmw;
  return a;
}

int ban_stage(omchat_ctx* ctx, const float** lg, int b, const int32_t* fed, hipStream_t s) {
  const PickState& P = ctx->pick;
  if (!P.con.on) return 0;
  OM_CHECK(b <= P.con.b, "constraints are on for fewer rows than this pick has (omchat_set_constraints)");
  const omchat_config& c = ctx->c;
  TRY(launch_constrain_ban(con_args(ctx, b, fed), s));
  TRY(launch_constrain_apply(*lg, c.t_vocab, b, c.t_vocab, P.con_ban, P.con_bmw, P.con_logits, fed ? P.con_len : nullptr, P.con_ld, s));
  *lg = P.con_logits;
  return 0;
}

int logprob_stage(omchat_ctx* ctx, const float* raw, const float* proc, int b, const int32_t* ids, hipStream_t s) {
  const PickState& P = ctx->pick;
  if (!P.lp.on) return 0;
  const omchat_config& c = ctx->c;
  LogprobArgs a;
  a.raw = raw; a.raw_ld = c.t_vocab; a.proc = proc; a.proc_ld = c.t_vocab;
  a.b = std::min(b, P.lp.b); a.V = c.t_vocab; a.rank = ctx->tp_rank; a.tp = ctx->tp_size;
  a.ids = ids;
  if (P.smp.on) {
    a.temperature = P.smp.temperature; a.penalty = P.smp.penalty;
    if (P.smp.penalty != 1.f) { a.seen = P.smp_bm; a.bm_words = P.smp_bmw; a.last_set = P.smp_last; }
    a.top1 = P.smp.top_k == 1;
    a.thr = sample_thr_words(P.smp_ws, b, c.t_vocab_total, P.smp.top_k, P.smp.top_p, P.smp_f, &a.thr_stride, &a.thr_hi);
  }
  a.ws = P.lp_ws; a.table = P.lp_table; a.xchg = smp_xchg; a.xchg_user = ctx;
  a.rec = (float*)P.lp_rec.p; a.cnt = P.lp_cnt; a.max_new = P.lp_cap; a.rec_ld = c.max_batch;
  return launch_logprob(a, s);
}

int lp_room(omchat_ctx* ctx) {
  OM_CHECK(!ctx->pick.lp.on || ctx->pick.lp_picks < ctx->pick.lp.max_new, "logprobs: more picks than the max_new given to omchat_set_logprobs");
  return 0;
}

int con_count_step(omchat_ctx* ctx) {
  if (!ctx->pick.con.on) return 0;
  OM_CHECK(ctx->pick.con_fed + 1 < ctx->pick.con_room, "constraints: more decode steps than the max_new given to omchat_set_constraints");
  ctx->pick.con_fed += 1;
  return 0;
}

}

int pick_alloc(omchat_ctx* ctx, int rows) {
  TRY(ctx->alloc(&ctx->pick.arg_scratch, argmax_scratch_bytes(rows)));
  return ctx->alloc((void**)&ctx->pick.tp_table, (size_t)ctx->tp_size * rows * 2 * 4);
}

int pick_admit(omchat_ctx* ctx, bool picks, bool feeds) {
  if (!(ctx->pick.smp_f == ctx->pick.smp_f_graph)) {
    drop_decode_graphs(ctx);
    ctx->pick.smp_f_graph = ctx->pick.smp_f;
  }
  if (picks) TRY(lp_room(ctx));
  if (feeds) TRY(con_count_step(ctx));
  ctx->pick.smp_vcommit = 0;
  if (ctx->pick.lp.on && picks) ctx->pick.lp_picks += 1;
  return 0;
}

int greedy_pick(omchat_ctx* ctx, const float* lg, int b, int32_t* next_tokens, hipStream_t s, bool advance) {
  const omchat_config& c = ctx->c;
  float* table = ctx->pick.tp_table;
  TRY(launch_argmax(lg, c.t_vocab, b, c.t_vocab, next_tokens, ctx->pick.arg_scratch, s, advance ? ctx->d_pos : nullptr, advance ? ctx->d_len : nullptr));
  if (ctx->tp_size > 1) {
    const size_t n = (size_t)ctx->tp_size * b * 2;
    OM_HIP(hipMemsetAsync(table, 0, n * 4, s));
    hipLaunchKernelGGL(tp_argmax_scatter_kernel, dim3(1), dim3(64 > b ? 64 : b), 0, s, lg, c.t_vocab, next_tokens, b, ctx->tp_rank, c.t_vocab, table);
    TRY(ctx->allreduce_f32(table, n, s));
    hipLaunchKernelGGL(tp_argmax_pick_kernel, dim3(1), dim3(64 > b ? 64 : b), 0, s, table, b, ctx->tp_size, next_tokens);
  }
  return 0;
}

int pick_run(omchat_ctx* ctx, const float* lg, int b, int32_t* next_tokens, hipStream_t s, bool advance, const int32_t* fed, bool force_greedy) {
  const PickState& P = ctx->pick;
  const float* raw = lg;
  TRY(ban_stage(ctx, &lg, b, fed, s));
  if (force_greedy || !P.smp.on) {
    TRY(greedy_pick(ctx, lg, b, next_tokens, s, advance));
    return logprob_stage(ctx, raw, lg, b, next_tokens, s);
  }
  const omchat_config& c = ctx->c;
  SampleArgs a;
  a.logits = lg; a.ld = c.t_vocab; a.b = b; a.V = c.t_vocab; a.V_total = c.t_vocab_total;
  a.rank = ctx->tp_rank; a.tp = ctx->tp_size;
  a.seed = P.smp.seed; a.temperature = P.smp.temperature; a.top_k = P.smp.top_k; a.top_p = P.smp.top_p; a.penalty = P.smp.penalty;
  a.f = P.smp_f;
  if (P.smp.penalty != 1.f) { a.bitmap = P.smp_bm; a.bm_words = P.smp_bmw; }
  a.last_set = P.smp_last; a.step = P.smp_step;
  if (advance) { a.adv_pos = ctx->d_pos; a.adv_len = ctx->d_len; }
  a.out = next_tokens; a.ws = P.smp_ws; a.table = P.tp_table;
  a.xchg = smp_xchg; a.xchg_user = ctx;
  TRY(launch_sample(a, s));
  return logprob_stage(ctx, raw, lg, b, next_tokens, s);
}

const char* pick_verify_refusal(omchat_ctx* ctx, int flags) {
  const PickState& P = ctx->pick;
  if (!(flags & OMCHAT_VERIFY_SAMPLE)) {
    if (P.smp.on) return "sampling is on: prompt-lookup decoding is greedy only";
  } else {
    if (!P.smp.on) return "OMCHAT_VERIFY_SAMPLE: sampling is off (omchat_set_sampling first)";
    if (flags & OMCHAT_VERIFY_KEEP_ALL) return "OMCHAT_VERIFY_SAMPLE with OMCHAT_VERIFY_KEEP_ALL: the slots behind a rejected draw are not the sampled sequence's";
  }
  return nullptr;
}

int pick_verify_prepare(omchat_ctx* ctx) {
  PickState& P = ctx->pick;
  if (P.smp.penalty != 1.f && !P.smp_vseen) TRY(ctx->alloc((void**)&P.smp_vseen, (size_t)SMP_VERIFY_ROWS * P.smp_bmw * 4));
  return 0;
}

int pick_verify(omchat_ctx* ctx, const float* lg, int T, const int32_t* tokens, int32_t* picks, hipStream_t s, bool sample) {
  if (!sample) return greedy_pick(ctx, lg, T, picks, s);
// ... 264 lines not shown
```

omchat_amd/engine.py:

```python
import ctypes as C
import numpy as np

from . import _lib
from ._lib import OmchatConfig, check, ptr, cur_stream
from .config import OmChatConfig


def _torch():
    import torch
    return torch


class Engine:
    def __init__(self, cfg: OmChatConfig, dtype="bf16", max_seq=4096, max_batch=1, max_tiles=4, max_prefill_rows=None,
                 tp_rank=0, tp_size=1, comm=None, device=None, vision=True, text=True):
        torch = _torch()
        if not torch.cuda.is_available():
            raise _lib.OmchatError("omchat_amd.Engine needs a HIP device: the HIP path has no CPU fallback")
        self.lib = _lib.lib()
        self.cfg = cfg
        self.dtype_code = {"f16": _lib.F16, "fp16": _lib.F16, "bf16": _lib.BF16}[dtype] if isinstance(dtype, str) else _lib.dtype_code(dtype)
        self.torch_dtype = _lib.torch_dtype(self.dtype_code)
        self.device = torch.device(device if device is not None else f"cuda:{torch.cuda.current_device()}")
        self.tp_rank, self.tp_size = tp_rank, tp_size
# ... 308 lines not shown
        n = C.c_int(0)
        check(self.lib.omchat_decode_verify(self.h, ptr(tk), T, ptr(logits), ptr(picks), C.byref(n), (1 if keep_all else 0) | (2 if sample else 0),
                                            cur_stream()))
        st = self._lookup_st
        st["verify_steps"] += 1; st["drafted"] += T - 1; st["accepted"] += n.value
        return (picks, n.value, logits) if want_logits else (picks, n.value)

    def lookup_stats(self, reset=False):
        out = dict(self._lookup_st)
        if reset:
            for key in self._lookup_st:
                self._lookup_st[key] = 0
        return out

    def verify_max_tokens(self):
        return min(16, 128 // max(1, self.c.t_heads // max(1, self.c.t_kv_heads)))

    def decode_step_masked(self, tokens, position_ids, attention_mask, want_logits=False):
        torch = _torch()
        tk = tokens.to(device=self.device, dtype=torch.int32).contiguous().view(-1)
        b = tk.shape[0]
        pos = position_ids.detach().to("cpu", torch.int32).contiguous().view(-1)
        m = attention_mask.detach().to("cpu").ne(0).to(torch.uint8).contiguous()
        if pos.shape[0] != b or m.dim() != 2 or m.shape[0] != b:
            raise ValueError("decode_step_masked: position_ids [b], attention_mask [b, slots + 1]")
        logits = torch.empty(b, self.c.t_vocab, dtype=torch.float32, device=self.device) if want_logits else None
        nxt = torch.empty(b, dtype=torch.int32, device=self.device)
        check(self.lib.omchat_decode_step_masked(self.h, ptr(tk), b, ptr(pos), ptr(m), m.shape[1], ptr(logits), ptr(nxt), cur_stream()))
        return nxt, logits

    def masked_decode_begin(self, position_ids, attention_mask):
        torch = _torch()
        pos = position_ids.detach().to("cpu", torch.int32).contiguous().view(-1)
        m = attention_mask.detach().to("cpu").ne(0).to(torch.uint8).contiguous()
        if m.dim() != 2 or pos.shape[0] != m.shape[0]:
            raise ValueError("masked_decode_begin: position_ids [b], attention_mask [b, cols]")
        cols = min(m.shape[1], self.c.max_seq)
        check(self.lib.omchat_masked_decode_begin(self.h, m.shape[0], ptr(pos), ptr(m), m.shape[1], cols, cur_stream()))

    def decode_step_masked_next(self, tokens, want_logits=False):
        torch = _torch()
        tk = tokens.to(device=self.device, dtype=torch.int32).contiguous().view(-1)
        b = tk.shape[0]
        logits = torch.empty(b, self.c.t_vocab, dtype=torch.float32, device=self.device) if want_logits else None
        nxt = torch.empty(b, dtype=torch.int32, device=self.device)
        check(self.lib.omchat_decode_step_masked_next(self.h, ptr(tk), b, ptr(logits), ptr(nxt), cur_stream()))
        return nxt, logits

    def fused_status(self):
        n, bits = C.c_long(0), C.c_uint(0)
        check(self.lib.omchat_fused_status(self.h, C.byref(n), C.byref(bits)))
        return n.value, bits.value

    def lm_head(self, hidden):
        torch = _torch()
        h = hidden.to(device=self.device, dtype=self.torch_dtype).contiguous()
        n = h.numel() // h.shape[-1]
        out = torch.empty(*h.shape[:-1], self.c.t_vocab, dtype=torch.float32, device=self.device)
        check(self.lib.omchat_lm_head(self.h, ptr(h), n, ptr(out), cur_stream()))
        return out

    def full_logits(self, logits):
        if self.tp_size == 1 or logits is None:
            return logits
        torch = _torch()
        import torch.distributed as dist
        if not (dist.is_available() and dist.is_initialized()):
            raise _lib.OmchatError("tensor-parallel logits are vocabulary shards: initialise torch.distributed to gather them, or use Engine.argmax")
        cpu = dist.get_backend() == "gloo"
        mine = logits.float().cpu().contiguous() if cpu else logits.float().contiguous()
        parts = [torch.empty_like(mine) for _ in range(self.tp_size)]
        dist.all_gather(parts, mine)
        return torch.cat(parts, dim=-1).to(self.device)

    def kv_lengths(self, b):
        torch = _torch()
        out = torch.zeros(b, dtype=torch.int32)
        check(self.lib.omchat_kv_lengths(self.h, ptr(out), b))
        return [int(x) for x in out]

    def kv_rewind(self, b, n=1):
        check(self.lib.omchat_kv_rewind(self.h, b, n, cur_stream()))

    def argmax(self, logits):
        torch = _torch()
        out = torch.empty(logits.shape[0], dtype=torch.int32, device=self.device)
        check(self.lib.omchat_greedy(self.h, ptr(logits), logits.shape[0], ptr(out), cur_stream()))
        return out

    def set_sampling(self, b, seed=0, temperature=1.0, top_k=0, top_p=1.0, repetition_penalty=1.0, seen=None, min_p=None, typical_p=None,
                     epsilon_cutoff=None, eta_cutoff=None):
        torch = _torch()
        seen = seen if seen is not None else [[] for _ in range(max(b, 0))]
        n = torch.tensor([len(r) for r in seen] or [0], dtype=torch.int32)
        flat = torch.tensor([int(i) for r in seen for i in r] or [0], dtype=torch.int32)
        check(self.lib.omchat_set_sampling(self.h, int(b), int(seed) & 0xFFFFFFFFFFFFFFFF, float(temperature), int(top_k or 0),
                                           float(1.0 if top_p is None else top_p), float(repetition_penalty), ptr(flat), ptr(n), cur_stream()))
        if int(b) > 0:
            cut = lambda v: float(v) if v is not None and 0.0 < float(v) < 1.0 else 1.0
            check(self.lib.omchat_set_sampling_filters(self.h, -1.0 if min_p is None else float(min_p),
                                                       1.0 if typical_p is None or float(typical_p) >= 1.0 else float(typical_p),
                                                       cut(epsilon_cutoff), cut(eta_cutoff), cur_stream()))

    def sampling_off(self):
        check(self.lib.omchat_set_sampling(self.h, 0, 0, 1.0, 0, 1.0, 1.0, None, None, cur_stream()))

# ... 80 lines not shown
```

Baseline: 342.6.

## Fuse embedding gather into first decode GEMVs and argmax into LM-head GEMV

For batch-1 decode, the first layer's QKV GEMV now reads the token's embedding row directly via a row index, and the o-proj residual does the same, so the separate gather-rows launch is dropped. The LM-head norm GEMV also writes per-block argmax candidates into slots, and a single-block pick kernel reduces them, replacing the two-stage full-vocab argmax. This also turns the SwiGLU XCD-skew launch on by default (skew 24 on 8-XCD parts) outside the experiments build. The changes cut launches and re-reads of the logits in the decode tail, at the cost of extra branches and shared-memory reductions in the GEMV kernels.

```diff
diff --git a/include/omchat_hip.h b/include/omchat_hip.h
--- a/include/omchat_hip.h
+++ b/include/omchat_hip.h
@@ -70,6 +70,7 @@
 int omchat_masked_decode_begin(omchat_ctx* ctx, int b, const int32_t* positions, const uint8_t* key_mask, int mask_ld, int mask_cols, void* stream);
 int omchat_decode_step_masked_next(omchat_ctx* ctx, const int32_t* tokens, int b, float* logits, int32_t* next_tokens, void* stream);
 int omchat_fused_status(omchat_ctx* ctx, long* launches, unsigned* timeout_bits);
+int omchat_decode_tail_stats(omchat_ctx* ctx, long* row_steps, long* slot_picks);
 int omchat_has_experiments(void);
 int omchat_lm_head(omchat_ctx* ctx, const void* hidden, int n, float* logits, void* stream);
 int omchat_greedy(omchat_ctx* ctx, const float* logits, int b, int32_t* next_tokens, void* stream);
@@ -142,6 +143,11 @@
                         float eps, float q_scale, void* out, void* stream);
 int omchat_op_gemv_norm(int dtype, const void* X, const void* W, int ldw, void* Y, int N, int K, const void* norm_w, float eps,
                         const void* bias, int epi, int out_f32, void* stream);
+int omchat_op_gemv_norm_slots(int dtype, const void* X, const void* W, int ldw, float* Y, int N, int K, const void* norm_w, float eps,
+                              const void* bias, float* slot_v, int32_t* slot_i, int cap, int* nslots, void* stream);
+int omchat_op_argmax_slots(const float* slot_v, const int32_t* slot_i, int nslots, int32_t* out, int32_t* adv_pos, int32_t* adv_len, void* stream);
+int omchat_op_gemv_row(int dtype, const void* X, const void* W, int ldw, void* Y, int N, int K, const void* norm_w, float eps, const void* bias,
+                       int epi, int out_f32, const int32_t* row_idx, const void* table, int row_ld, void* stream);
 int omchat_op_set_tuning(int key, int value);
 int omchat_gemm_tune_load(const char* path);
 int omchat_gemm_tune_dump(const char* path);
diff --git a/omchat_amd/_lib.py b/omchat_amd/_lib.py
--- a/omchat_amd/_lib.py
+++ b/omchat_amd/_lib.py
@@ -128,6 +128,10 @@
     "omchat_op_rope_kv": (_i, [_i, _vp, _i, _i, _i, _i, _i, _f, _vp, _vp, _i, _vp]),
     "omchat_op_rope_kv_q8": (_i, [_i, _vp, _i, _i, _i, _i, _i, _f, _vp, _vp, _i, _vp, _vp, _vp, _vp, _vp]),
     "omchat_op_argmax": (_i, [_vp, _i, _i, _vp, _vp]),
+    "omchat_op_gemv_norm_slots": (_i, [_i, _vp, _vp, _i, _vp, _i, _i, _vp, _f, _vp, _vp, _vp, _i, C.POINTER(_i), _vp]),
+    "omchat_op_argmax_slots": (_i, [_vp, _vp, _i, _vp, _vp, _vp, _vp]),
+    "omchat_op_gemv_row": (_i, [_i, _vp, _vp, _i, _vp, _i, _i, _vp, _f, _vp, _i, _i, _vp, _vp, _i, _vp]),
+    "omchat_decode_tail_stats": (_i, [_vp, C.POINTER(C.c_long), C.POINTER(C.c_long)]),
     "omchat_op_attn_prefill_left": (_i, [_i, _vp, _vp, _vp, _vp, _i, _i, _i, _i, _i, _vp, _vp, _i, _i, _f, _i, _vp]),
     "omchat_op_rope_kv_pos": (_i, [_i, _vp, _i, _i, _i, _i, _vp, _i, _i, _i, _f, _vp, _vp, _i, _vp]),
     "omchat_op_argmax_ld": (_i, [_vp, _i, _i, _i, _vp, _vp, _vp, _vp]),
diff --git a/omchat_amd/csrc/capi.hip b/omchat_amd/csrc/capi.hip
--- a/omchat_amd/csrc/capi.hip
+++ b/omchat_amd/csrc/capi.hip
@@ -98,6 +98,7 @@
   if (key == 38) { gemv_set_gu_rr(value); return 0; }
   if (key == 39) { gemv_set_longk_direct(value); return 0; }
   if (key == 40) { norm_set_wave(value); return 0; }
+  if (key == 50) { model_set_decode_tail(value); return 0; }
 #if OMCHAT_EXPERIMENTS
   if (key == 41) { g_launch_any_order = value; return 0; }
   if (key == 42) { model_set_ao_oproj(value); return 0; }
@@ -132,6 +133,26 @@
   OM_CHECK(X && W && Y && norm_w, "null argument");
   GemvArgs g{X, K, W, ldw, Y, N, 1, N, K, bias, nullptr, 0, epi, out_f32};
   g.norm_w = norm_w; g.norm_eps = eps;
+  return launch_gemv(dtype, g, S(stream));
+}
+
+extern "C" int omchat_op_gemv_norm_slots(int dtype, const void* X, const void* W, int ldw, float* Y, int N, int K, const void* norm_w, float eps,
+                                         const void* bias, float* slot_v, int32_t* slot_i, int cap, int* nslots, void* stream) {
+  OM_CHECK(X && W && Y && norm_w && slot_v && slot_i && nslots, "null argument");
+  GemvArgs g{X, K, W, ldw, Y, N, 1, N, K, bias, nullptr, 0, EPI_NONE, 1};
+  g.norm_w = norm_w; g.norm_eps = eps;
+  g.arg_v = slot_v; g.arg_i = slot_i; g.arg_cap = cap; g.arg_n = nslots;
+  return launch_gemv(dtype, g, S(stream));
+}
+extern "C" int omchat_op_argmax_slots(const float* slot_v, const int32_t* slot_i, int nslots, int32_t* out, int32_t* adv_pos, int32_t* adv_len, void* stream) {
+  return launch_argmax_slots(slot_v, slot_i, nslots, out, S(stream), adv_pos, adv_len);
+}
+extern "C" int omchat_op_gemv_row(int dtype, const void* X, const void* W, int ldw, void* Y, int N, int K, const void* norm_w, float eps, const void* bias,
+                                  int epi, int out_f32, const int32_t* row_idx, const void* table, int row_ld, void* stream) {
+  OM_CHECK(W && Y && row_idx && table && (norm_w || X), "null argument");
+  GemvArgs g{norm_w ? table : X, K, W, ldw, Y, N, 1, N, K, bias, norm_w ? nullptr : table, N, epi, out_f32};
+  g.norm_w = norm_w; g.norm_eps = eps;
+  g.row_idx = row_idx; g.row_table = table; g.row_ld = row_ld;
   return launch_gemv(dtype, g, S(stream));
 }
 
diff --git a/omchat_amd/csrc/ctx.h b/omchat_amd/csrc/ctx.h
--- a/omchat_amd/csrc/ctx.h
+++ b/omchat_amd/csrc/ctx.h
@@ -27,6 +27,9 @@
 
 struct PickState {
   void* arg_scratch = nullptr;
+  float* slot_v = nullptr; int* slot_i = nullptr; int slot_cap = 0;
+  const float* slot_lg = nullptr; int slot_n = 0;
+  long n_slot_picks = 0;
   float* tp_table = nullptr;
   struct Sampling { bool on = false; uint64_t seed = 0; float temperature = 1.f; int top_k = 0; double top_p = 1.0; float penalty = 1.f; };
   Sampling smp;
@@ -147,6 +150,7 @@
   long n_fused_launches = 0;
   void* dl_ws = nullptr;
   long n_layer_launches = 0;
+  long n_row_steps = 0;
   unsigned long long* dbg_stamps = nullptr;
   unsigned* dyn_ctr = nullptr;
   int *d_pos = nullptr, *d_len = nullptr, *d_idx = nullptr, *d_start = nullptr;
diff --git a/omchat_amd/csrc/elementwise.hip b/omchat_amd/csrc/elementwise.hip
--- a/omchat_amd/csrc/elementwise.hip
+++ b/omchat_amd/csrc/elementwise.hip
@@ -678,9 +678,6 @@
 }
 
 constexpr int ARG_CHUNKS = 64;
-__device__ __forceinline__ void arg_better(float& best, int& besti, float v, int i) {
-  if (v > best || (v == best && i < besti)) { best = v; besti = i; }
-}
 __global__ __launch_bounds__(256) void argmax_stage1_kernel(const float* logits, int ld, int V, float* pv, int* pi) {
   __shared__ float bv[4];
   __shared__ int bi[4];
@@ -710,6 +707,38 @@
 #pragma unroll
   for (int o = 32; o > 0; o >>= 1) arg_better(best, besti, __shfl_xor(best, o, 64), __shfl_xor(besti, o, 64));
   if (threadIdx.x == 0) out[blockIdx.x] = besti == INT_MAX ? 0 : besti;
+}
+
+constexpr int ARG_PICK_THREADS = 1024, ARG_PICK_PER = 10;
+__global__ __launch_bounds__(ARG_PICK_THREADS) void argmax_pick_kernel(const float* pv, const int* pi, int n, int* out, int* adv_pos, int* adv_len) {
+  __shared__ float bv[ARG_PICK_THREADS / 64];
+  __shared__ int bi[ARG_PICK_THREADS / 64];
+  if (threadIdx.x == 0) {
+    if (adv_pos) adv_pos[0] += 1;
+    if (adv_len) adv_len[0] += 1;
+  }
+  float best = -INFINITY;
+  int besti = INT_MAX;
+  for (int i0 = 0; i0 < n; i0 += ARG_PICK_THREADS * ARG_PICK_PER) {
+    float v[ARG_PICK_PER];
+    int ix[ARG_PICK_PER];
+#pragma unroll
+    for (int j = 0; j < ARG_PICK_PER; ++j) {
+      const int i = i0 + j * ARG_PICK_THREADS + threadIdx.x;
+      v[j] = i < n ? pv[i] : -INFINITY;
+      ix[j] = i < n ? pi[i] : INT_MAX;
+    }
+#pragma unroll
+    for (int j = 0; j < ARG_PICK_PER; ++j) arg_better(best, besti, v[j], ix[j]);
+  }
+#pragma unroll
+  for (int o = 32; o > 0; o >>= 1) arg_better(best, besti, __shfl_xor(best, o, 64), __shfl_xor(besti, o, 64));
+  if ((threadIdx.x & 63) == 0) { bv[threadIdx.x >> 6] = best; bi[threadIdx.x >> 6] = besti; }
+  __syncthreads();
+  if (threadIdx.x == 0) {
+    for (int w = 1; w < ARG_PICK_THREADS / 64; ++w) arg_better(best, besti, bv[w], bi[w]);
+    out[0] = besti == INT_MAX ? 0 : besti;
+  }
 }
 
 __device__ __forceinline__ uint64_t splitmix64(uint64_t x) {
@@ -953,6 +982,13 @@
 
 size_t argmax_scratch_bytes(int b) { return (size_t)b * ARG_CHUNKS * 8; }
 
+int launch_argmax_slots(const float* pv, const int* pi, int nslots, int* out, hipStream_t s, int* adv_pos, int* adv_len) {
+  OM_CHECK(pv && pi && out && nslots >= 1, "argmax slots: bad argument");
+  hipLaunchKernelGGL(argmax_pick_kernel, dim3(1), dim3(ARG_PICK_THREADS), 0, s, pv, pi, nslots, out, adv_pos, adv_len);
+  OM_LAUNCH_CHECK();
+  return 0;
+}
+
 int launch_argmax(const float* logits, int ld, int b, int V, int* out, void* scratch, hipStream_t s, int* adv_pos, int* adv_len) {
   if (b == 0) return 0;
   OM_CHECK(scratch, "argmax scratch missing");
diff --git a/omchat_amd/csrc/gemv.hip b/omchat_amd/csrc/gemv.hip
--- a/omchat_amd/csrc/gemv.hip
+++ b/omchat_amd/csrc/gemv.hip
@@ -14,10 +14,19 @@
   void* y_pack;
   unsigned long long* dbg;
   const unsigned char* mx_s;
-#if OMCHAT_EXPERIMENTS
   int xskew;
-#endif
+  const int* row_idx; const void* row_tab; int row_ld;
+  float* arg_v; int* arg_i;
+  int arg_cap; int* arg_n;
 };
+template <typename T>
+__device__ __forceinline__ const T* gemv_row_of(const GemvP& p, const T* direct, bool& zero) {
+  zero = false;
+  if (!p.row_idx) return direct;
+  const int id = __builtin_amdgcn_readfirstlane(p.row_idx[0]);
+  zero = id < 0;
+  return (const T*)p.row_tab + (size_t)(id < 0 ? 0 : id) * p.row_ld;
+}
 constexpr int WF_16 = 0, WF_E4M3 = 1, WF_MX4 = 2;
 #if OMCHAT_EXPERIMENTS
 #define OM_DBG_MIN(slot, cond) do { if (p.dbg && (cond) && threadIdx.x == 0) atomicMax(p.dbg + (slot), ~wall_clock64()); } while (0)
@@ -767,6 +776,9 @@
   }
   const int n_out = EPI == EPI_SWIGLU ? p.N / 2 : p.N;
   const int ngroups = (n_out + OUT - 1) / OUT;
+  bool rzero = false;
+  const T* resid = (const T*)p.resid;
+  if constexpr (EPI == EPI_RESID) resid = gemv_row_of<T>(p, resid, rzero);
   for (int g = blockIdx.x * WAVES + wave; g < ngroups; g += gridDim.x * WAVES) {
     int rows[R];
 #pragma unroll
@@ -785,7 +797,7 @@
       constexpr bool plain = EPI != EPI_SWIGLU && EPI != EPI_PARTIAL;
       const bool hb = plain && p.bias, hr = EPI == EPI_RESID && !p.out_f32;
       tail.p0 = hb ? (const T*)p.bias : (const T*)p.X;
-      tail.p1 = hr ? (const T*)p.resid : (const T*)p.X;
+      tail.p1 = hr ? resid : (const T*)p.X;
 #pragma unroll
       for (int r = 0; r < R; ++r) {
         const int n = g * OUT + r;
@@ -811,7 +823,7 @@
           if (p.out_f32) ((float*)p.Y)[n] = y;
           else {
             y = rnd<T>(y);
-            if constexpr (EPI == EPI_RESID) y = tail.v1[r] + y;
+            if constexpr (EPI == EPI_RESID) y = (rzero ? 0.f : tail.v1[r]) + y;
             ((T*)p.Y)[n] = fromf<T>(y);
           }
         }
@@ -835,7 +847,6 @@
   const int lane = threadIdx.x & 63, wave = __builtin_amdgcn_readfirstlane(threadIdx.x >> 6);
   const int n_out = EPI == EPI_SWIGLU ? p.N / 2 : p.N;
   int g = blockIdx.x * WAVES + wave;
-#if OMCHAT_EXPERIMENTS
   if constexpr (EPI == EPI_SWIGLU && RR == 1 && WAVES == 4) {
     if (p.xskew) {
       const int x = blockIdx.x & 7, j = blockIdx.x >> 3;
@@ -845,19 +856,20 @@
       g = (x * base + ((x & 1) ? p.xskew : 0) + j) * 4 + wave;
     }
   }
-#endif
   if constexpr (EPI == EPI_SWIGLU) OM_DBG_MIN(4, blockIdx.x < 8);
   if constexpr (EPI == EPI_NONE) OM_DBG_MIN(8, blockIdx.x < 8);
   static_assert(WAVES >= 4 && NCH <= 8, "sum-of-squares order: four owner waves, up to two chunks each");
   constexpr int MC = (NCH + WAVES - 1) / WAVES;
   constexpr int SC = (NCH + 3) / 4;
   rw_u32x4 xq[MC], nq[MC], sq[SC];
+  bool xzero;
+  const T* const X = gemv_row_of<T>(p, (const T*)p.X, xzero);
 #pragma unroll
   for (int i = 0; i < MC; ++i) {
     const int c = wave + WAVES * i, k = c * 512 + lane * 8;
     const rw_u32x4 z = {0u, 0u, 0u, 0u};
-    const bool ok = c < NCH && k < p.K;
-    xq[i] = ok ? *reinterpret_cast<const rw_u32x4*>((const T*)p.X + k) : z;
+    const bool ok = c < NCH && k < p.K && !xzero;
+    xq[i] = ok ? *reinterpret_cast<const rw_u32x4*>(X + k) : z;
     nq[i] = ok ? *reinterpret_cast<const rw_u32x4*>((const T*)p.norm_w + k) : z;
   }
 #pragma unroll
@@ -867,7 +879,7 @@
     } else {
       const int c = wave + 4 * i, k = c * 512 + lane * 8;
       const rw_u32x4 z = {0u, 0u, 0u, 0u};
-      sq[i] = (wave < 4 && c < NCH && k < p.K) ? *reinterpret_cast<const rw_u32x4*>((const T*)p.X + k) : z;
+      sq[i] = (wave < 4 && c < NCH && k < p.K && !xzero) ? *reinterpret_cast<const rw_u32x4*>(X + k) : z;
     }
   }
   int rows[R];
@@ -970,6 +982,27 @@
         const float y = acc[r] + e_bias[r];
         if (p.out_f32) ((float*)p.Y)[n] = y;
         else ((T*)p.Y)[n] = fromf<T>(y);
+      }
+    }
+  }
+  if constexpr (EPI == EPI_NONE) {
+    if (p.arg_v) {
+      __shared__ float abv[WAVES];
+      __shared__ int abi[WAVES];
+      float best = -INFINITY;
+      int besti = INT_MAX;
+#pragma unroll
+      for (int r = 0; r < RR; ++r) {
+        const int n = g * RR + r;
+        if (n < n_out) arg_better(best, besti, acc[r] + e_bias[r], n);
+      }
+      if (lane == 0) { abv[wave] = best; abi[wave] = besti; }
+      __syncthreads();
+      if (threadIdx.x == 0) {
+#pragma unroll
+        for (int w = 1; w < WAVES; ++w) arg_better(best, besti, abv[w], abi[w]);
+        p.arg_v[blockIdx.x] = best;
+        p.arg_i[blockIdx.x] = besti;
       }
     }
   }
@@ -1402,6 +1435,8 @@
 #endif
 int g_gemv_longk_direct = 0;
 
+static bool device_xcds_8() { return device_cus() == 256; }
+
 template <typename T>
 int launch_rows_longk(const GemvP& p, hipStream_t s) {
 #if OMCHAT_EXPERIMENTS
@@ -1439,17 +1474,25 @@
 }
 
 int g_gemv_rows_balance = 1;
-unsigned g_gemv_skew = 0;
+unsigned g_gemv_skew = 24;
 int g_gemv_dyn = 0;
 int g_gemv_gu_rr = 1;
 int g_gemv_gu_rr8 = 1;
 int g_gemv_norm_loop = 0;
 
+inline GemvP with_arg_slots(const GemvP& p, int grid) {
+  GemvP q = p;
+  if (!q.arg_v) return q;
+  if (grid > q.arg_cap) { q.arg_v = nullptr; q.arg_i = nullptr; return q; }
+  if (q.arg_n) *q.arg_n = grid;
+  return q;
+}
+
 template <typename T, int EPI, int RR, int F8, int NCH>
 void launch_rows_norm_n(const GemvP& p, hipStream_t s) {
   const int n_out = EPI == EPI_SWIGLU ? p.N / 2 : p.N;
   if constexpr (NCH >= 4) {
-    const bool want = EPI == EPI_SWIGLU ? (g_gemv_norm_loop & (F8 != WF_16 ? 4 : 1)) : (p.N < 32768 ? (g_gemv_norm_loop & 2) : (g_gemv_norm_loop & 8));
+    const bool want = !p.row_idx && (EPI == EPI_SWIGLU ? (g_gemv_norm_loop & (F8 != WF_16 ? 4 : 1)) : (p.N < 32768 ? (g_gemv_norm_loop & 2) : (g_gemv_norm_loop & 8)));
     const int n_cu = device_cus();
 #if OMCHAT_EXPERIMENTS
     if (want && p.dyn && g_gemv_dyn && n_out >= 8 * n_cu) {
@@ -1469,24 +1512,25 @@
   if constexpr (NCH >= 4 && EPI == EPI_NONE && RR <= 2) {
     const int n_cu = device_cus();
     if (g_gemv_rows_balance && n_out == 9 * 2 * n_cu) {
-      if constexpr (F8 == WF_MX4) hipLaunchKernelGGL((gemv_rows_norm_mx4_kernel<T, EPI, 1, NCH, 9>), dim3(2 * n_cu), dim3(576), 0, s, p);
-      else hipLaunchKernelGGL((gemv_rows_norm_kernel<T, EPI, 1, NCH, F8 == WF_E4M3, 9>), dim3(2 * n_cu), dim3(576), 0, s, p);
+      const GemvP q = with_arg_slots(p, 2 * n_cu);
+      if constexpr (F8 == WF_MX4) hipLaunchKernelGGL((gemv_rows_norm_mx4_kernel<T, EPI, 1, NCH, 9>), dim3(2 * n_cu), dim3(576), 0, s, q);
+      else hipLaunchKernelGGL((gemv_rows_norm_kernel<T, EPI, 1, NCH, F8 == WF_E4M3, 9>), dim3(2 * n_cu), dim3(576), 0, s, q);
       return;
     }
   }
-#if OMCHAT_EXPERIMENTS
   if constexpr (EPI == EPI_SWIGLU && RR == 1) {
-    const int nwg = cdiv(n_out, 4), xs = (int)(g_gemv_skew < 256u ? g_gemv_skew : 0u);
-    if (xs > 0 && nwg % 8 == 0 && n_out % 4 == 0 && xs < nwg / 8) {
+    const int nwg = cdiv(n_out, 4), xs = (int)(F8 == WF_16 && g_gemv_skew < 256u ? g_gemv_skew : 0u);
+    if (xs > 0 && nwg % 8 == 0 && n_out % 4 == 0 && xs < nwg / 8 && device_xcds_8()) {
       GemvP q = p; q.xskew = xs;
       if constexpr (F8 == WF_MX4) hipLaunchKernelGGL((gemv_rows_norm_mx4_kernel<T, EPI, RR, NCH>), dim3(8 * (nwg / 8 + xs)), dim3(256), 0, s, q);
       else hipLaunchKernelGGL((gemv_rows_norm_kernel<T, EPI, RR, NCH, F8 == WF_E4M3>), dim3(8 * (nwg / 8 + xs)), dim3(256), 0, s, q);
       return;
     }
   }
-#endif
-  if constexpr (F8 == WF_MX4) hipLaunchKernelGGL((gemv_rows_norm_mx4_kernel<T, EPI, RR, NCH>), dim3(cdiv(cdiv(n_out, RR), 4)), dim3(256), 0, s, p);
-  else hipLaunchKernelGGL((gemv_rows_norm_kernel<T, EPI, RR, NCH, F8 == WF_E4M3>), dim3(cdiv(cdiv(n_out, RR), 4)), dim3(256), 0, s, p);
+  const int grid = cdiv(cdiv(n_out, RR), 4);
+  const GemvP q = with_arg_slots(p, grid);
+  if constexpr (F8 == WF_MX4) hipLaunchKernelGGL((gemv_rows_norm_mx4_kernel<T, EPI, RR, NCH>), dim3(grid), dim3(256), 0, s, q);
+  else hipLaunchKernelGGL((gemv_rows_norm_kernel<T, EPI, RR, NCH, F8 == WF_E4M3>), dim3(grid), dim3(256), 0, s, q);
 }
 template <typename T, int EPI, int RR, int F8>
 void launch_rows_norm(const GemvP& p, hipStream_t s) {
@@ -1557,6 +1601,22 @@
   const int ks = a.ksplit > 1 ? a.ksplit : 1;
   GemvP p{a.X, a.W, a.Y, a.bias, a.resid, a.ldx, a.ldw, a.ldy, a.ldr, a.b, a.N, a.K, a.out_f32, ks, a.w_scale, a.y_packed, a.norm_w, a.norm_eps,
           (unsigned*)a.dyn_ctr, a.y_pack, a.dbg, a.mx_scale};
+  if (a.arg_n) *a.arg_n = 0;
+  const bool rows_form = a.b == 1 && !a.x_packed && ks == 1 && cdiv(a.K, 512) <= RW_MAXC && (a.w_scale || a.mx_scale || (!a.force_mfma && !g_gemv_force_mfma));
+  if (a.row_idx) {
+    if (!(rows_form && a.row_table && (a.norm_w ? (a.epi == EPI_NONE || a.epi == EPI_SWIGLU) : (a.epi == EPI_RESID && !a.out_f32)))) {
+      omchat_set_error("launch_gemv: a row index needs the batch-1 whole-row form (K <= 4096, no split-K): X of the norm form or the residual of EPI_RESID");
+      return 1;
+    }
+    p.row_idx = a.row_idx; p.row_tab = a.row_table; p.row_ld = a.row_ld;
+  }
+  if (a.arg_v) {
+    if (!(rows_form && a.arg_i && a.norm_w && a.epi == EPI_NONE && a.out_f32)) {
+      omchat_set_error("launch_gemv: pick slots need the batch-1 norm form with fp32 outputs (epilogue NONE)");
+      return 1;
+    }
+    p.arg_v = a.arg_v; p.arg_i = a.arg_i; p.arg_cap = a.arg_cap; p.arg_n = a.arg_n;
+  }
   if (a.norm_w && a.x_packed && !(a.w_packed && ks == 1 && (a.K >> 6) == 56 && a.epi == EPI_SWIGLU && a.N % 32 == 0 && !g_gemv_no_xs)) {
     omchat_set_error("launch_gemv: the in-register RMSNorm on packed x exists for the x-stationary gate|up form only (packed W, K = 3584, no split-K)");
     return 1;
diff --git a/omchat_amd/csrc/kernels.h b/omchat_amd/csrc/kernels.h
--- a/omchat_amd/csrc/kernels.h
+++ b/omchat_amd/csrc/kernels.h
@@ -76,6 +76,8 @@
   void* y_pack = nullptr;
   unsigned long long* dbg = nullptr;
   const unsigned char* mx_scale = nullptr;
+  const int32_t* row_idx = nullptr; const void* row_table = nullptr; int row_ld = 0;
+  float* arg_v = nullptr; int* arg_i = nullptr; int arg_cap = 0; int* arg_n = nullptr;
 };
 int launch_pack_x(int dtype, const void* X, int ldx, int b, int K, void* out, hipStream_t s);
 int launch_pack_w(int dtype, const void* W, int ldw, int N, int K, void* out, hipStream_t s);
@@ -222,6 +224,7 @@
 int launch_attn_oproj_fused(int dtype, const AttnDecodeArgs& a, const FusedDecodeArgs& f, hipStream_t s);
 void model_set_fuse_attn_oproj(int v);
 void model_set_decode_layer(int v);
+void model_set_decode_tail(int v);
 void model_set_shard_as_tp1(int v);
 
 struct DecodeLayerArgs {
@@ -260,7 +263,11 @@
 int launch_gather_rows(int dtype, const int* idx, const void* table, const void* feats, void* out, int rows, int H, hipStream_t s);
 int launch_copy_rows(int dtype, const void* src, int64_t src_ld, void* dst, int64_t dst_ld, int rows, int H,
                      int group, int skip, hipStream_t s);
+__device__ __forceinline__ void arg_better(float& best, int& besti, float v, int i) {
+  if (v > best || (v == best && i < besti)) { best = v; besti = i; }
+}
 size_t argmax_scratch_bytes(int b);
+int launch_argmax_slots(const float* pv, const int* pi, int nslots, int* out, hipStream_t s, int* adv_pos = nullptr, int* adv_len = nullptr);
 int launch_argmax(const float* logits, int ld, int b, int V, int* out, void* scratch, hipStream_t s, int* adv_pos = nullptr, int* adv_len = nullptr);
 struct SampleFilters {
   double min_p = -1.0, typical_p = 1.0, epsilon = 1.0, eta = 1.0;
diff --git a/omchat_amd/csrc/model.hip b/omchat_amd/csrc/model.hip
--- a/omchat_amd/csrc/model.hip
+++ b/omchat_amd/csrc/model.hip
@@ -85,6 +85,8 @@
 void model_set_fuse_attn_oproj(int v) { g_fuse_attn_oproj = v; }
 int g_ao_oproj = 0;
 void model_set_ao_oproj(int v) { g_ao_oproj = v; }
+int g_decode_tail = 1;
+void model_set_decode_tail(int v) { g_decode_tail = v; }
 int g_fuse_peer_norm = 1;
 void model_set_fuse_peer_norm(int v) { g_fuse_peer_norm = v; }
 
@@ -1240,7 +1242,7 @@
   const bool lead = ctx->tp_rank == 0;
   void* x = ctx->tw_x;
   void* y = ctx->tw_x2;
-  TRY(launch_gather_rows(ctx->dt, tokens, ctx->t_embed, nullptr, x, b, H, s));
+  ctx->pick.slot_lg = nullptr;
   const bool f8 = ctx->fp8_decode && b == 1;
   const bool mx4 = ctx->mx4_step(b);
   const bool wq = f8 || mx4;
@@ -1292,6 +1294,9 @@
   const bool n1 = n2 && (g_norm_in_gemv & 2) && It <= 32768 && It % 8 == 0;
   const bool nb2 = OMCHAT_EXPERIMENTS && (g_norm_in_gemv & 4) && fused && wpk && ctx->tp_size == 1 && !wq && (qd >> 6) == 56 && (H >> 6) == 56 && qd % 64 == 0 &&
                    H / 16 <= device_cus() && (2 * It) / 32 >= 4 * device_cus();
+  const bool tail1 = g_decode_tail && n1 && !g_decode_layer && !g_fuse_attn_oproj && !g_ao_oproj;
+  if (!tail1) TRY(launch_gather_rows(ctx->dt, tokens, ctx->t_embed, nullptr, x, b, H, s));
+  else ++ctx->n_row_steps;
   if (fused && !n1) TRY(launch_rmsnorm(ctx->dt, x, H, ctx->dl[0].ln1, ctx->tw_xn, H, b, H, c.t_eps, s, pk));
 #if OMCHAT_EXPERIMENTS
   if ((g_ao_oproj & 16) && ctx->dbg_stamps) OM_HIP(hipMemsetAsync(ctx->dbg_stamps, 0, (size_t)c.t_layers * 256, s));
@@ -1322,6 +1327,7 @@
     if (n1) {
       GemvArgs g = gemv_args(x, H, L.wqkv, H, ctx->tw_qkv, qkvd, 1, qkvd, L.bqkv, nullptr, EPI_NONE, 0, Q.wqkv, Q.sqkv, nullptr, false, M.wqkv, M.sqkv);
       g.norm_w = L.ln1; g.norm_eps = c.t_eps;
+      if (tail1 && i == 0) { g.row_idx = tokens; g.row_table = ctx->t_embed; g.row_ld = H; }
       if (OMCHAT_EXPERIMENTS && (g_ao_oproj & 16) && ctx->dbg_stamps) g.dbg = ctx->dbg_stamps + (size_t)i * 32;
       TRY(launch_gemv(ctx->dt, g, s));
     } else {
@@ -1388,6 +1394,10 @@
       GemvArgs g = gemv_args(ctx->tw_ao, qd, L.wo, qd, x, H, 1, H, nullptr, x, EPI_RESID, 0, nullptr, nullptr, nullptr, false);
       g.dbg = ctx->dbg_stamps + (size_t)i * 32;
       TRY(launch_gemv(ctx->dt, g, s));
+    } else if (n2 && tail1 && i == 0) {
+      GemvArgs g = gemv_args(ctx->tw_ao, qd, L.wo, qd, x, H, 1, H, nullptr, x, EPI_RESID, 0, Q.wo, Q.so, nullptr, false, M.wo, M.so);
+      g.row_idx = tokens; g.row_table = ctx->t_embed; g.row_ld = H;
+      TRY(launch_gemv(ctx->dt, g, s));
     } else if (n2) {
       TRY(gemv(ctx->tw_ao, qd, L.wo, qd, x, H, H, nullptr, x, EPI_RESID, Q.wo, Q.so, nullptr, false, M.wo, M.so));
     } else if (nb2) {
@@ -1446,7 +1456,11 @@
     if (f8) { g.W = ctx->t_lm8; g.w_scale = ctx->t_lm8_s; }
     if (mx4) { g.W = ctx->t_lm4; g.ldw = H / 2; g.mx_scale = ctx->t_lm4_s; }
     g.norm_w = ctx->t_norm; g.norm_eps = c.t_eps;
+    int n_slots = 0;
+    PickState& K = ctx->pick;
+    if (g_decode_tail && next_tokens && vL < 0 && K.slot_v && !K.smp.on && !K.con.on) { g.arg_v = K.slot_v; g.arg_i = K.slot_i; g.arg_cap = K.slot_cap; g.arg_n = &n_slots; }
     TRY(launch_gemv(ctx->dt, g, s));
+    if (n_slots > 0) { K.slot_lg = lg; K.slot_n = n_slots; }
   } else {
     TRY(lm_head_rows(ctx, ctx->tw_xn, b, lg, s, f8, fused && pk, mx4));
   }
@@ -1456,7 +1470,15 @@
     hipLaunchKernelGGL(advance_lens_kernel, dim3(1), dim3(64 > b ? 64 : b), 0, s, ctx->d_pos, ctx->d_len, b);
     TRY(pick_feed(ctx, tokens, b, s));
   }
+  ctx->pick.slot_lg = nullptr;
   OM_LAUNCH_CHECK();
+  return 0;
+}
+
+extern "C" int omchat_decode_tail_stats(omchat_ctx* ctx, long* row_steps, long* slot_picks) {
+  OM_CHECK(ctx, "null ctx");
+  if (row_steps) *row_steps = ctx->n_row_steps;
+  if (slot_picks) *slot_picks = ctx->pick.n_slot_picks;
   return 0;
 }
 
diff --git a/omchat_amd/csrc/pick.hip b/omchat_amd/csrc/pick.hip
--- a/omchat_amd/csrc/pick.hip
+++ b/omchat_amd/csrc/pick.hip
@@ -84,6 +84,12 @@
 
 int pick_alloc(omchat_ctx* ctx, int rows) {
   TRY(ctx->alloc(&ctx->pick.arg_scratch, argmax_scratch_bytes(rows)));
+  const int cap = cdiv(ctx->c.t_vocab, 8);
+  if (cap > 0) {
+    TRY(ctx->alloc((void**)&ctx->pick.slot_v, (size_t)cap * 4));
+    TRY(ctx->alloc((void**)&ctx->pick.slot_i, (size_t)cap * 4));
+    ctx->pick.slot_cap = cap;
+  }
   return ctx->alloc((void**)&ctx->pick.tp_table, (size_t)ctx->tp_size * rows * 2 * 4);
 }
 
@@ -102,6 +108,12 @@
 int greedy_pick(omchat_ctx* ctx, const float* lg, int b, int32_t* next_tokens, hipStream_t s, bool advance) {
   const omchat_config& c = ctx->c;
   float* table = ctx->pick.tp_table;
+  PickState& P = ctx->pick;
+  if (P.slot_lg && P.slot_lg == lg && P.slot_n > 0 && b == 1 && ctx->tp_size == 1) {
+    P.slot_lg = nullptr;
+    ++P.n_slot_picks;
+    return launch_argmax_slots(P.slot_v, P.slot_i, P.slot_n, next_tokens, s, advance ? ctx->d_pos : nullptr, advance ? ctx->d_len : nullptr);
+  }
   TRY(launch_argmax(lg, c.t_vocab, b, c.t_vocab, next_tokens, ctx->pick.arg_scratch, s, advance ? ctx->d_pos : nullptr, advance ? ctx->d_len : nullptr));
   if (ctx->tp_size > 1) {
     const size_t n = (size_t)ctx->tp_size * b * 2;
diff --git a/omchat_amd/engine.py b/omchat_amd/engine.py
--- a/omchat_amd/engine.py
+++ b/omchat_amd/engine.py
@@ -384,6 +384,11 @@
         check(self.lib.omchat_fused_status(self.h, C.byref(n), C.byref(bits)))
         return n.value, bits.value
 
+    def decode_tail_stats(self):
+        r, p = C.c_long(0), C.c_long(0)
+        check(self.lib.omchat_decode_tail_stats(self.h, C.byref(r), C.byref(p)))
+        return r.value, p.value
+
     def lm_head(self, hidden):
         torch = _torch()
         h = hidden.to(device=self.device, dtype=self.torch_dtype).contiguous()
```

Result: no change. 343.7, median of 6 (+0.3%).
